# PKU-MARL/HARL

Hardware: AMD Instinct MI355X
Metric: transitions/sec through HAPPO update (MPE spread, 3 agents) (higher is better)
Workload: dtype f32

## Files before the change

### harl_amd/_lib.py

```python
from __future__ import annotations

import ctypes as C
import os
from typing import Dict, Optional

import torch

from .traffic import algorithmic_bytes, algorithmic_flops

_HERE = os.path.dirname(os.path.abspath(__file__))
LIB_PATH = os.path.join(_HERE, "lib", "libharl_%s.so" % (os.environ.get("HARL_LIB") or "hip"))

PS_STRIDE = 48
DHEAD_LD = 32
SLAB = 32

_vp, _i, _l, _f, _d = C.c_void_p, C.c_int, C.c_long, C.c_float, C.c_double

SIGNATURES = {
    "harl_gae_returns": [_vp] * 8 + [_i, _i, _f, _f, _i, _i, _i, _vp],
    "harl_masked_moments": [_vp, _vp, _l, _vp, _vp, _vp],
    "harl_dist_rows": [_vp, _l, _i, _i, _vp, _f, _f, _vp, _vp, _vp, _i, _i, _vp, _vp, _vp, _vp, _vp, _vp],
    "harl_moments_mean": [_vp, _vp, _vp],
    "harl_clock_probe": [_vp, _l, _vp],
    "harl_build_seq": [_vp, _i, _i, _i, _l, _vp, _vp, _i, _vp, _vp, _vp, _vp, _vp],
    "harl_adv_normalize": [_vp, _vp, _vp, _l, _vp],
    "harl_factor_update": [_vp, _vp, _vp, _l, _i, _i, _vp],
    "harl_sum_sumsq": [_vp, _vp, _l, _vp, _vp],
    "harl_valuenorm_apply": [_vp, _vp, _d, _d, _vp],
    "harl_gradnorm_clip_adam": [_vp, _vp, _vp, _vp, _l, _vp, _i, _f, _d, _d, _d, _f, _f, _d, _d, _vp, _vp],
    "harl_fold_linear": [_vp] * 6 + [_i, _i, _vp],
    "harl_unfold_linear_grads": [_vp, _vp, _i, _vp, _vp, _vp, _vp, _vp, _vp, _vp, _i, _i, _i, _vp],
    "harl_mlp_fwd_input": [_vp, _l, _vp, _l, _i, _vp, _vp, _i, _i, _vp, _vp, _vp, _vp, _vp, _vp, _vp],
    "harl_mlp_x0n_wide": [_vp, _l, _vp, _l, _i, _i, _vp, _vp, _vp, _vp],
    "harl_mlp_fwd_wide": [_vp, _l, _i, _vp, _i, _vp, _i, _vp, _vp, _vp, _vp, _vp],
    "harl_mlp_linear_wide": [_vp, _l, _i, _vp, _i, _vp, _i, _vp, _vp, _vp],
    "harl_act_ln_fwd": [_vp, _l, _i, _i, _vp, _vp, _vp, _vp],
    "harl_act_bwd": [_vp, _vp, _vp, _vp, _l, _i, _i, _vp],
    "harl_act_ln_tangent": [_vp, _vp, _vp, _vp, _vp, _l, _i, _i, _vp, _vp],
    "harl_mlp_tangent_wide": [_vp, _l, _i, _vp, _i, _vp, _i, _vp, _vp, _vp, _vp, _vp, _vp],
    "harl_mlp_fwd_fused2x": [_vp, _l, _vp, _i, _vp, _vp, _vp, _i, _i, _vp, _vp, _vp, _vp, _vp, _vp, _vp],
    "harl_mlp_fwd_fused2": [_vp, _l, _vp, _l, _i, _vp, _vp, _i, _vp, _vp, _i, _i, _vp, _vp, _vp, _vp, _vp, _vp, _vp, _vp,
                            _vp, _vp],
    "harl_mlp_fwd_hidden": [_vp, _l, _i, _i, _vp, _vp, _vp, _vp, _vp, _vp],
    "harl_mlp_bwd_dx": [_vp, _vp, _vp, _vp, _l, _i, _i, _vp, _vp, _vp, _i, _vp, _i, _vp],
    "harl_mlp_bwd_dx_dw": [_vp, _vp, _vp, _vp, _l, _i, _i, _vp, _vp, _vp, _i, _vp, _vp, _i, _i, _vp],
    "harl_mlp_dw_partials": [_vp, _i, _i, _i, _vp, _i, _l, _vp, _vp, _vp, _i, _l, _vp, _i, _vp],
    "harl_mlp_dw_partials_multi": [_i, _vp, _vp, _vp, _i, _i, _l, _i, _vp],
    "harl_mlp_dw_partials_multi_v": [_i, _vp, _vp, _vp, _i, _vp, _vp, _vp, _l, _i, _vp],
    "harl_gru_dw6": [_vp, _vp, _vp, _vp, _vp, _vp, _vp, _l, _i, _vp],
    "harl_mlp_fwd_trunk": [_vp, _l, _i, _vp, _i, _vp, _i, _vp, _i, _vp, _vp, _vp, _vp, _vp, _vp, _vp, _vp, _vp, _vp],
    "harl_mlp_bwd_trunk": [_l, _i, _i, _vp, _vp, _vp, _vp, _vp, _vp, _vp, _vp, _vp, _vp, _vp],
    "harl_reduce_partials": [_vp, _i, _l, _vp, _vp],
    "harl_reduce_partials_multi": [_vp, _vp, _i, _i, _l, _vp, _vp],
    "harl_adam_fold": [_vp, _vp, _vp, _vp, _l, _vp, _vp, _i, _vp, _vp, _vp, _i, _vp, _i, _f, _i, _i, _vp, _i, _f, _d, _d,
                       _d, _f, _f, _d, _d, _vp, _vp],
    "harl_pack_scalars_hilo": [_vp, _vp, _vp],
    "harl_reduce_pack_scalars": [_vp, _i, _vp, _vp, _vp],
    "harl_randperm_replay": [_vp, _l, _l, _vp, _vp, _vp],
    "harl_rng_advance": [_vp, _l, _l, _vp],
    "harl_rng_jump": [_vp, _l, _l, _vp],
    "harl_actor_head_logp": [_vp, _l, _i, _vp, _vp, _vp, _f, _f, _i, _i, _vp, _vp, _vp, _vp, _vp, _i, _vp, _l, _l, _vp],
    "harl_actor_head_loss": [_vp, _vp, _vp, _l, _i, _vp, _vp, _vp, _f, _f, _i, _i, _vp, _vp, _vp, _vp, _vp, _vp,
                             _vp, _vp, _d, _f, _i, _i, _l, _l, _vp, _vp, _vp, _vp, _vp, _i, _vp],
    "harl_critic_head_values": [_vp, _l, _i, _vp, _vp, _vp, _vp],
    "harl_critic_head_loss": [_vp, _vp, _vp, _l, _i, _vp, _vp, _vp, _vp, _vp, _vp, _f, _i, _i, _f, _l, _l, _vp, _vp, _vp,
                              _vp, _i, _vp],
    "harl_gru_fwd": [_vp] * 7 + [_i, _i, _l] + [_vp] * 8 + [_i, _vp, _vp],
    "harl_gru_bwd": [_vp] * 9 + [_i, _i, _l] + [_vp] * 8 + [_vp],
    "harl_fold_linear_tangent": [_vp] * 9 + [_i, _i, _vp],
    "harl_fold_table": [_vp, _vp, _vp, _i, _i, _vp],
    "harl_unfold_table": [_vp, _vp, _vp, _vp, _i, _i, _vp],
    "harl_fold_tangent_table": [_vp, _vp, _vp, _vp, _i, _i, _vp],
    "harl_mlp_tangent_input": [_vp, _l, _vp, _l, _i, _vp, _vp, _i, _i, _vp, _vp, _vp, _vp, _vp],
    "harl_gru_gates": [_vp, _vp, _i, _l, _vp, _vp, _vp, _i, _vp],
    "harl_gru_tangent": [_vp] * 15 + [_i, _i, _l, _vp, _vp],
    "harl_mlp_tangent_hidden": [_vp, _vp, _l, _i, _i, _vp, _vp, _vp, _vp, _vp, _vp, _vp, _vp],
    "harl_mlp_tangent_hidden2": [_vp, _vp, _l, _i, _i, _vp, _vp, _vp, _vp, _vp, _vp, _vp, _vp, _vp],
    "harl_actor_head_fvp": [_vp, _vp, _vp, _vp, _l, _i, _vp, _vp, _vp, _vp, _vp, _f, _f, _i, _i, _vp, _l, _l, _vp, _vp, _vp],
    "harl_trpo_kl_sum": [_vp, _vp, _vp, _vp, _f, _f, _l, _i, _i, _vp, _vp],
    "harl_update_supported": [_i, _i, _i, _i],
    "harl_update_fwd_actor": [_vp, _l, _i, _i] + [_vp] * 7 + [_f, _f, _i, _i] + [_vp] * 7 + [_d, _f, _i, _i] + [_vp] * 4 + [_i] + [_vp] * 4,
    "harl_update_logp": [_vp, _l, _i, _i] + [_vp] * 7 + [_f, _f, _i, _i] + [_vp] * 5 + [_i, _vp, _vp],
    "harl_update_last_actor": [_vp, _l, _i] + [_vp] * 5 + [_f, _f, _i, _i] + [_vp] * 8 + [_d, _f, _i, _i] + [_vp] * 4 + [_i, _vp],
    "harl_update_last_critic": [_vp, _l, _i] + [_vp] * 8 + [_f, _i, _i, _f] + [_vp] * 3 + [_i, _vp],
    "harl_update_fwd_critic": [_vp, _l, _i, _i] + [_vp] * 9 + [_f, _i, _i, _f] + [_vp] * 3 + [_i] + [_vp] * 4,
    "harl_update_values": [_vp, _l, _i, _i] + [_vp] * 7 + [_vp],
    "harl_update_bwd": [_vp, _vp, _l, _i, _i] + [_vp] * 5 + [_i, _vp],
    "harl_head_blocks": [_l],
    "harl_trpo_fvp_finish": [_vp, _vp, _vp, _vp, _l, _f, _f, _l, _i, _f, _f, _vp],
    "harl_trpo_cg_step": [_vp, _vp, _vp, _vp, _l, _vp, _vp, _vp],
    "harl_mlp_panel_fwd": [_vp, _l, _i, _vp, _i, _vp, _i, _vp, _vp, _vp, _vp],
    "harl_mlp_panel_bwd": [_vp, _vp, _vp, _vp, _l, _i, _i, _vp, _vp, _vp],
    "harl_head_dw_rows256": [_vp, _l, _i, _vp, _vp, _i, _vp],
    "harl_mlp_panel_tangent": [_vp, _vp, _l, _i, _vp, _vp, _i, _vp, _vp, _vp, _vp, _vp, _vp],
    "harl_reduce_scalars": [_vp, _i, _vp, _vp],
    "harl_mlp_linear": [_vp, _l, _i, _i, _vp, _vp, _vp, _vp],
    "harl_mlp_linear3": [_vp, _vp, _vp, _l, _i, _i, _vp, _vp, _vp, _vp, _vp, _vp, _vp, _vp, _vp, _vp],
    "harl_gru_cell_init": [_vp, _vp, _i, _l, _vp, _vp],
    "harl_gru_cell_fwd": [_vp] * 8 + [_i, _l] + [_vp] * 7 + [_vp],
    "harl_gru_cell_bwd": [_vp] * 10 + [_i, _l] + [_vp] * 5 + [_vp],
    "harl_rownorm": [_vp, _l, _i, _vp, _vp, _vp],
    "harl_gru_cell_tangent": [_vp] * 19 + [_i, _l] + [_vp] * 3,
    "harl_md_head_logp": [_vp, _i, _vp, _i, _vp, _vp, _l, _vp, _vp, _vp, _i, _vp, _i, _vp, _l, _l, _vp],
    "harl_md_head_loss": [_vp, _vp, _i, _vp, _i, _vp, _vp, _l, _vp, _vp, _vp, _i, _vp, _vp, _vp, _vp, _vp, _d, _f, _i, _i,
                          _l, _l, _vp, _vp, _i, _vp],
    "harl_trpo_begin": [_vp, _vp, _l, _i, _vp, _vp, _vp, _vp, _l, _vp, _vp, _vp, _vp],
    "harl_trpo_step": [_vp, _vp, _vp, _vp, _vp, _vp, _l, _f, _vp, _vp, _vp],
    "harl_trpo_ls_candidate": [_vp, _vp, _vp, _vp, _l, _vp],
    "harl_trpo_ls_test": [_vp, _vp, _d, _d, _d, _d, _vp, _vp],
    "harl_reduce_scalars_set": [_vp, _i, _vp, _vp],
    "harl_zero_bytes": [_vp, _l, _vp],
    "harl_comm_create": [_i, _i, _l, _i, _vp, _vp],
    "harl_comm_connect": [_vp, _vp],
    "harl_comm_allreduce": [_vp, _vp, _l, _i, _vp],
    "harl_comm_set_timeout": [_vp, _d],
    "harl_comm_status": [_vp],
    "harl_comm_destroy": [_vp],
    "harl_version": [],
}


class HipLibraryMissing(RuntimeError):
    pass


_lib: Optional[C.CDLL] = None


def load() -> C.CDLL:
    global _lib
    if _lib is not None:
        return _lib
    if not os.path.exists(LIB_PATH):
        raise HipLibraryMissing(
            f"{LIB_PATH} not found: build it with `python -m harl_amd._build` (hipcc, gfx950). "
            "harl_amd has no CPU fallback.")
    lib = C.CDLL(LIB_PATH)
    for name, argtypes in SIGNATURES.items():
        fn = getattr(lib, name)
        fn.argtypes = argtypes
        fn.restype = C.c_int
    lib.harl_last_error.argtypes = []
    lib.harl_last_error.restype = C.c_char_p
    _lib = lib
    return lib


def ptr(t: Optional[torch.Tensor]) -> Optional[int]:
    if t is None:
        return None
    assert t.is_contiguous(), "harl_amd kernels need contiguous tensors"
    return t.data_ptr()


_raw_stream = getattr(torch._C, "_cuda_getCurrentRawStream", None)
_raw_device = getattr(torch._C, "_cuda_getDevice", None)


def stream() -> int:
    if _raw_stream is not None and _raw_device is not None:
        return _raw_stream(_raw_device())
    return torch.cuda.current_stream().cuda_stream


_timing_on = False
_timing_events: dict = {}


_timing_tags = None


_event_pool: list = []


def reserve_timing_events(n: int) -> None:
    while len(_event_pool) < n:
        _event_pool.append(torch.cuda.Event(enable_timing=True))


def enable_kernel_timing(on: bool, tags=None) -> None:
    global _timing_on, _timing_tags
    _timing_on = bool(on)
    _timing_tags = set(tags) if tags else None
    if on:
        _timing_events.clear()

# ... 57 lines not shown
```

### harl_amd/csrc/wide.hip

```cpp
#include <type_traits>
#include <stdlib.h>
#include "common.h"
#include "split_mfma.h"
#include "fwd_epilogue.h"
#include "../../include/harl_hip.h"

using namespace harl;

namespace {

int bad(const char *m) {
  set_error(m);
  return -2;
}

__device__ __forceinline__ float wave_sum_dpp(float v) {
  auto dpp = [](float x, auto ctrl) {
    return __builtin_bit_cast(float, __builtin_amdgcn_update_dpp(0, __builtin_bit_cast(int, x), decltype(ctrl)::value, 0xf, 0xf, true));
  };
  v += dpp(v, std::integral_constant<int, 0xB1>{});
  v += dpp(v, std::integral_constant<int, 0x4E>{});
  v += dpp(v, std::integral_constant<int, 0x141>{});
  v += dpp(v, std::integral_constant<int, 0x140>{});
  const float r0 = __builtin_bit_cast(float, __builtin_amdgcn_readlane(__builtin_bit_cast(int, v), 0));
  const float r1 = __builtin_bit_cast(float, __builtin_amdgcn_readlane(__builtin_bit_cast(int, v), 16));
  const float r2 = __builtin_bit_cast(float, __builtin_amdgcn_readlane(__builtin_bit_cast(int, v), 32));
  const float r3 = __builtin_bit_cast(float, __builtin_amdgcn_readlane(__builtin_bit_cast(int, v), 48));
  return (r0 + r1) + (r2 + r3);
}

constexpr int XT_LD = 36;

template <int NC>
__global__ __launch_bounds__(WG_THREADS, NC <= 3 ? 2 : 1) void k_x0n_wide(const float *__restrict__ X, long ldx,
                                                                           const int64_t *__restrict__ idx, long M, int D,
                                                                           int use_ln0, float *__restrict__ x0n,
                                                                           float *__restrict__ mu0_out,
                                                                           float *__restrict__ rstd0_out, long n_slabs, int KP) {
  __shared__ __attribute__((aligned(16))) float tiles[WAVES_PER_WG][2][32 * XT_LD];
  const int lane = threadIdx.x & 63, wave = wave_id();
  const int i = lane & 31, h = lane >> 5;
  float *tw = &tiles[wave][0][0];
  for (long slab = (long)blockIdx.x * WAVES_PER_WG + wave; slab < n_slabs; slab += (long)gridDim.x * WAVES_PER_WG) {
    long rows[32];
    if (idx) {
#pragma unroll
      for (int r = 0; r < 32; ++r) {
        const long j = slab * SLAB + r;
        rows[r] = idx[j < M ? j : M - 1];
      }
    } else {
#pragma unroll
      for (int r = 0; r < 32; ++r) {
        const long j = slab * SLAB + r;
        rows[r] = j < M ? j : M - 1;
      }
    }
    int kc[NC];
#pragma unroll
    for (int c = 0; c < NC; ++c) kc[c] = 64 * c + lane < D ? 64 * c + lane : 0;
    float v[32][NC];
#pragma unroll
    for (int r = 0; r < 32; ++r) {
      const float *xr = X + rows[r] * ldx;
#pragma unroll
      for (int c = 0; c < NC; ++c) v[r][c] = xr[kc[c]];
    }
    const float invD = 1.0f / (float)D;
    float my_mean = 0.f, my_rstd = 1.f;
#pragma unroll
    for (int r = 0; r < 32; ++r) {
      float mean = 0.f, rstd = 1.f;
      if (use_ln0) {
        float s = 0.f;
#pragma unroll
        for (int c = 0; c < NC; ++c) s += (64 * c + lane < D) ? v[r][c] : 0.f;
        mean = wave_sum_dpp(s) * invD;
        float q = 0.f;
#pragma unroll
        for (int c = 0; c < NC; ++c) {
          const float d = v[r][c] - mean;
          q += (64 * c + lane < D) ? d * d : 0.f;
        }
        rstd = 1.0f / sqrtf(wave_sum_dpp(q) * invD + 1e-5f);
      }
#pragma unroll
      for (int c = 0; c < NC; ++c) {
        const int k = 64 * c + lane;
        v[r][c] = k < D ? (v[r][c] - mean) * rstd : ((k == KP - 1 && D < KP) ? 1.0f : 0.f);
      }
      if (lane == r) {
        my_mean = mean;
        my_rstd = rstd;
      }
    }
    if (lane < 32) {
      mu0_out[slab * SLAB + lane] = my_mean;
      rstd0_out[slab * SLAB + lane] = my_rstd;
    }
    f32x4 *op = reinterpret_cast<f32x4 *>(x0n + slab * (long)KP * SLAB) + lane;
#pragma unroll
    for (int c = 0; c < NC; ++c) {
      if (64 * c < KP) {
        float *tl = tw + h * (32 * XT_LD) + i * XT_LD;
#pragma unroll
        for (int r4 = 0; r4 < 8; ++r4)
          *reinterpret_cast<f32x4 *>(tl + 4 * r4) = f32x4{v[4 * r4][c], v[4 * r4 + 1][c], v[4 * r4 + 2][c], v[4 * r4 + 3][c]};
        asm volatile("s_waitcnt lgkmcnt(0)" ::: "memory");
        __builtin_amdgcn_wave_barrier();
#pragma unroll
        for (int t2 = 0; t2 < 2; ++t2) {
          if (64 * c + 32 * t2 < KP) {
            const float *ts = tw + t2 * (32 * XT_LD);
#pragma unroll
            for (int qq = 0; qq < 4; ++qq) {
              f32x4 o;
#pragma unroll
              for (int e = 0; e < 4; ++e) o[e] = ts[(8 * qq + 4 * h + e) * XT_LD + i];
              op[(4 * (2 * c + t2) + qq) * WAVE] = o;
            }
          }
        }
        asm volatile("s_waitcnt lgkmcnt(0)" ::: "memory");
        __builtin_amdgcn_wave_barrier();
      }
    }
  }
}

template <int KPV>
__global__ __launch_bounds__(WG_THREADS, 4) void k_x0n_contig(const float *__restrict__ X, long M, int D, int use_ln0,
                                                              float *__restrict__ x0n, float *__restrict__ mu0_out,
                                                              float *__restrict__ rstd0_out, long n_slabs) {
  __shared__ float rowsl[WAVES_PER_WG][32 * KPV + 32];
  const int lane = threadIdx.x & 63, wave = wave_id();
  const int i = lane & 31, h = lane >> 5;
  float *rw = &rowsl[wave][0];
  const int per = 32 * D;
  for (long slab = (long)blockIdx.x * WAVES_PER_WG + wave; slab < n_slabs; slab += (long)gridDim.x * WAVES_PER_WG) {
    const long base = slab * SLAB * (long)D, lim = M * (long)D;
#pragma unroll
    for (int u = 0; u < KPV / 2; ++u) {
      const int e = u * 64 + lane;
      if (e < per) rw[e] = base + e < lim ? X[base + e] : 0.f;
    }
    asm volatile("s_waitcnt vmcnt(0) lgkmcnt(0)" ::: "memory");
    __builtin_amdgcn_wave_barrier();
    const float *xr = rw + i * D;
    float mean = 0.f, rstd = 1.f;
    if (use_ln0) {
      float sm = 0.f;
      for (int k = 0; k < D; ++k) sm += xr[k];
      mean = sm / (float)D;
      float vs = 0.f;
      for (int k = 0; k < D; ++k) {
        const float d = xr[k] - mean;
        vs += d * d;
      }
      rstd = 1.0f / sqrtf(vs / (float)D + 1e-5f);
    }
    f32x4 *op = reinterpret_cast<f32x4 *>(x0n + slab * (long)KPV * SLAB) + lane;
#pragma unroll
    for (int q = 0; q < KPV / 8; ++q) {
      f32x4 o;
#pragma unroll
      for (int e = 0; e < 4; ++e) {
        const int f = 32 * (q >> 2) + 8 * (q & 3) + 4 * h + e;
        o[e] = f < D ? (xr[f < D ? f : 0] - mean) * rstd : ((f == KPV - 1 && D < KPV) ? 1.0f : 0.f);
      }
      op[q * WAVE] = o;
    }
    if (h == 0) {
      mu0_out[slab * SLAB + i] = mean;
      rstd0_out[slab * SLAB + i] = rstd;
    }
    asm volatile("s_waitcnt lgkmcnt(0)" ::: "memory");
    __builtin_amdgcn_wave_barrier();
  }
}

__global__ __launch_bounds__(WG_THREADS, 2) void k_x0n_narrow(const float *__restrict__ X, long ldx,
                                                              const int64_t *__restrict__ idx, long M, int D, int use_ln0,
                                                              float *__restrict__ x0n, float *__restrict__ mu0_out,
                                                              float *__restrict__ rstd0_out, long n_slabs) {
  __shared__ __attribute__((aligned(16))) float tiles[WAVES_PER_WG][32 * XT_LD];
  const int lane = threadIdx.x & 63, wave = wave_id();
  const int i = lane & 31, h = lane >> 5;
  float *tw = &tiles[wave][0];
  const int kc = i < D ? i : 0;
  for (long slab = (long)blockIdx.x * WAVES_PER_WG + wave; slab < n_slabs; slab += (long)gridDim.x * WAVES_PER_WG) {
    long rows[16];
    if (idx) {
#pragma unroll
      for (int u = 0; u < 16; ++u) {
        const long j = slab * SLAB + 2 * u + h;
        rows[u] = idx[j < M ? j : M - 1];
      }
    } else {
#pragma unroll
      for (int u = 0; u < 16; ++u) {
        const long j = slab * SLAB + 2 * u + h;
        rows[u] = j < M ? j : M - 1;
      }
    }
    float v[16];
#pragma unroll
    for (int u = 0; u < 16; ++u) v[u] = X[rows[u] * ldx + kc];
    const float invD = 1.0f / (float)D;
    float my_mean = 0.f, my_rstd = 1.f;
#pragma unroll
    for (int u = 0; u < 16; ++u) {
      float mean = 0.f, rstd = 1.f;
      if (use_ln0) {
        mean = half_reduce_sum(i < D ? v[u] : 0.f) * invD;
        const float d = v[u] - mean;
        rstd = 1.0f / sqrtf(half_reduce_sum(i < D ? d * d : 0.f) * invD + 1e-5f);
      }
      v[u] = i < D ? (v[u] - mean) * rstd : ((i == 31 && D < 32) ? 1.0f : 0.f);
      if (i == u) {
        my_mean = mean;
        my_rstd = rstd;
      }
    }
    if (i < 16) {
      mu0_out[slab * SLAB + 2 * i + h] = my_mean;
      rstd0_out[slab * SLAB + 2 * i + h] = my_rstd;
    }
#pragma unroll
    for (int u = 0; u < 16; ++u) tw[i * XT_LD + 2 * u + h] = v[u];
    asm volatile("s_waitcnt lgkmcnt(0)" ::: "memory");
    __builtin_amdgcn_wave_barrier();
    f32x4 *op = reinterpret_cast<f32x4 *>(x0n + slab * (long)32 * SLAB) + lane;
#pragma unroll
    for (int qq = 0; qq < 4; ++qq) {
      f32x4 o;
#pragma unroll
      for (int e = 0; e < 4; ++e) o[e] = tw[(8 * qq + 4 * h + e) * XT_LD + i];
      op[qq * WAVE] = o;
    }
    asm volatile("s_waitcnt lgkmcnt(0)" ::: "memory");
    __builtin_amdgcn_wave_barrier();
  }
}

__global__ __launch_bounds__(256) void k_split_image(const float *__restrict__ Wp, int H, int D, int KP,
                                                     u32x4 *__restrict__ img, const float *__restrict__ WpB = nullptr,
                                                     int DA = 0) {
  const int MT = H / 32, NJ = KP / 16, total = MT * NJ * 64;
  for (int e = blockIdx.x * blockDim.x + threadIdx.x; e < total; e += gridDim.x * blockDim.x) {
    const int ln = e & 63, j = (e >> 6) % NJ, t = (e >> 6) / NJ, m = 32 * t + (ln & 31), g = ln >> 5;
    unsigned p[3][4];
#pragma unroll
    for (int c = 0; c < 4; ++c) {
      const int f0 = feat_base(8 * j + 2 * c) + 4 * g, f1 = feat_base(8 * j + 2 * c + 1) + 4 * g;
      float w0, w1;
      if (WpB) {
        w0 = f0 < DA ? Wp[(long)m * DA + f0] : (f0 < D ? WpB[(long)m * (D - DA) + (f0 - DA)] : 0.f);
        w1 = f1 < DA ? Wp[(long)m * DA + f1] : (f1 < D ? WpB[(long)m * (D - DA) + (f1 - DA)] : 0.f);
      } else {
        w0 = f0 < D ? Wp[(long)m * D + f0] : 0.f;
        w1 = f1 < D ? Wp[(long)m * D + f1] : 0.f;
      }
      split3_rne(w0, w1, p[0][c], p[1][c], p[2][c]);
    }
#pragma unroll
    for (int term = 0; term < 3; ++term) img[(long)term * total + e] = u32x4{p[term][0], p[term][1], p[term][2], p[term][3]};
  }
}

template <int HO, int MODE, int NJL = 0>
__global__ __launch_bounds__(WG_THREADS, 1) void k_fwd_wide(const float *__restrict__ x0n, const u32x4 *__restrict__ img,
                                                            const float *__restrict__ bp, float *__restrict__ xout,
                                                            uint32_t *__restrict__ mask_out, float *__restrict__ rstd_out,
                                                            const float *__restrict__ xprimal,
                                                            const uint32_t *__restrict__ mask_in,
                                                            const float *__restrict__ rstd_in, long n_slabs, int KP,
                                                            const float *__restrict__ x0n_b = nullptr, int KPA = 0) {
  constexpr int MT = HO / 32;
  const int NJ = KP / 16, TS = MT * NJ * 64;
  const int KA = x0n_b ? KPA : KP, NJA = KA / 16, KB = KP - KA;
  const int lane = threadIdx.x & 63, wave = wave_id(), h = lane >> 5;
  const long n_pairs = (n_slabs + 1) / 2;
  const u32x4 *wl = img + lane;
  extern __shared__ __attribute__((aligned(16))) float lds_w[];
  const u32x4 *ll = reinterpret_cast<const u32x4 *>(lds_w) + lane;
  if constexpr (NJL > 0) {
    u32x4 *li = reinterpret_cast<u32x4 *>(lds_w);
    for (int e = threadIdx.x; e < 3 * MT * NJL * 64; e += WG_THREADS) {
      const int ln = e & 63, j = (e >> 6) % NJL, t = ((e >> 6) / NJL) % MT, term = (e >> 6) / (NJL * MT);
      li[e] = img[(long)term * TS + (t * NJ + j) * 64 + ln];
    }
    __syncthreads();
  }
  for (long pair = (long)blockIdx.x * WAVES_PER_WG + wave; pair < n_pairs; pair += (long)gridDim.x * WAVES_PER_WG) {
    const long s0 = 2 * pair, s1 = s0 + 1 < n_slabs ? s0 + 1 : s0;
    const f32x4 *xp0 = reinterpret_cast<const f32x4 *>(x0n + s0 * (long)KA * SLAB) + lane;
    const f32x4 *xp1 = reinterpret_cast<const f32x4 *>(x0n + s1 * (long)KA * SLAB) + lane;
    const f32x4 *xq0 = x0n_b ? reinterpret_cast<const f32x4 *>(x0n_b + s0 * (long)KB * SLAB) + lane : xp0;
    const f32x4 *xq1 = x0n_b ? reinterpret_cast<const f32x4 *>(x0n_b + s1 * (long)KB * SLAB) + lane : xp1;
    f32x16 acc0[MT], acc1[MT];
#pragma unroll
    for (int t = 0; t < MT; ++t)
#pragma unroll
      for (int r = 0; r < 16; ++r) acc0[t][r] = acc1[t][r] = bp[32 * t + (r & 3) + 8 * (r >> 2) + 4 * h];
    u32x4 an[3][MT];
    f32x4 bn[2][2];
    auto fetch = [&](int j) {
      if (NJL > 0 && j < NJL) {
#pragma unroll
        for (int term = 0; term < 3; ++term)
#pragma unroll
          for (int t = 0; t < MT; ++t) an[term][t] = ll[((term * MT + t) * NJL + j) * 64];
      } else {
#pragma unroll
        for (int term = 0; term < 3; ++term)
#pragma unroll
          for (int t = 0; t < MT; ++t) an[term][t] = wl[(long)term * TS + (t * NJ + j) * 64];
      }
      const f32x4 *b0 = j < NJA ? xp0 + (2 * j) * WAVE : xq0 + (2 * (j - NJA)) * WAVE;
      const f32x4 *b1 = j < NJA ? xp1 + (2 * j) * WAVE : xq1 + (2 * (j - NJA)) * WAVE;
      bn[0][0] = b0[0];
      bn[0][1] = b0[WAVE];
      bn[1][0] = b1[0];
      bn[1][1] = b1[WAVE];
    };
    fetch(0);
    for (int j = 0; j < NJ; ++j) {
      u32x4 a[3][MT];
#pragma unroll
      for (int term = 0; term < 3; ++term)
// ... 263 lines not shown
      vs = wave_sum32(vs);
      const float rstd = 1.0f / sqrtf(vs * (1.0f / H) + 1e-5f);
#pragma unroll
      for (int R = 0; R < NR; ++R) v[R] *= rstd;
      atl_store<H>(x2out, slab, lane, v);
#pragma unroll
      for (int w = 0; w < NW; ++w) mask2[(slab * NW + w) * WAVE + lane] = bits[w];
      if (lane < 32) rstd2[slab * SLAB + lane] = rstd;
    }
    PHASE(5);
  }
  PHASE_END(0);
}

constexpr size_t wide_sh_lds(int ho) { return (size_t)2 * 3 * (ho / 32) * WSH_PJ * 64 * 16; }
bool wide_shared(long n_slabs) {
  const char *e = getenv("HARL_WIDE_SHARED");
  return e && e[0] == '1' && n_slabs >= 512;
}

constexpr size_t wide_res_lds() { return (size_t)3 * 4 * 8 * 64 * 16; }
bool wide_resident(long n_slabs) {
  const char *e = getenv("HARL_WIDE_RESIDENT");
  return e && e[0] == '1' && n_slabs >= 512;
}

template <int MODE>
int launch_wide(const float *x0n, long M, int KP, const float *Wp, int D, const float *bp, int H, void *w_img, float *xout,
                uint32_t *mask_out, float *rstd_out, const float *xprimal, const uint32_t *mask_in, const float *rstd_in,
                hipStream_t s, const char *what) {
  if (M <= 0) return 0;
  if (H != 128 && H != 64) return bad("harl_mlp_*_wide: hidden width must be 64 or 128");
  if (KP % 32 != 0 || KP < D || KP > 512) return bad("harl_mlp_*_wide: KP must be a multiple of 32, >= D and <= 512");
  if (!w_img || !x0n) return bad("harl_mlp_*_wide: x0n and the weight-image scratch are required");
  const long n_slabs = n_slabs_of(M);
  const int total = (H / 32) * (KP / 16) * 64;
  hipLaunchKernelGGL(k_split_image, dim3((total + 255) / 256), dim3(256), 0, s, Wp, H, D, KP, reinterpret_cast<u32x4 *>(w_img));
  const long pairs = (n_slabs + 1) / 2, wgs = (pairs + WAVES_PER_WG - 1) / WAVES_PER_WG;
  const int grid = (int)(wgs < 256 ? (wgs < 1 ? 1 : wgs) : 256);
  if (wide_shared(n_slabs)) {
    if (H == 128) {
      allow_big_lds(k_fwd_wide_sh<128, MODE>, wide_sh_lds(128));
      hipLaunchKernelGGL((k_fwd_wide_sh<128, MODE>), dim3(grid), dim3(WG_THREADS), wide_sh_lds(128), s, x0n,
                         reinterpret_cast<const u32x4 *>(w_img), bp, xout, mask_out, rstd_out, xprimal, mask_in, rstd_in, n_slabs, KP);
    } else {
      allow_big_lds(k_fwd_wide_sh<64, MODE>, wide_sh_lds(64));
      hipLaunchKernelGGL((k_fwd_wide_sh<64, MODE>), dim3(grid), dim3(WG_THREADS), wide_sh_lds(64), s, x0n,
                         reinterpret_cast<const u32x4 *>(w_img), bp, xout, mask_out, rstd_out, xprimal, mask_in, rstd_in, n_slabs, KP);
    }
    return check_launch(what);
  }
  if (H == 128 && KP >= 256 && wide_resident(n_slabs)) {
    allow_big_lds(k_fwd_wide<128, MODE, 8>, wide_res_lds());
    hipLaunchKernelGGL((k_fwd_wide<128, MODE, 8>), dim3(grid), dim3(WG_THREADS), wide_res_lds(), s, x0n,
                       reinterpret_cast<const u32x4 *>(w_img), bp, xout, mask_out, rstd_out, xprimal, mask_in, rstd_in, n_slabs, KP);
  } else if (H == 128)
    hipLaunchKernelGGL((k_fwd_wide<128, MODE>), dim3(grid), dim3(WG_THREADS), 0, s, x0n, reinterpret_cast<const u32x4 *>(w_img),
                       bp, xout, mask_out, rstd_out, xprimal, mask_in, rstd_in, n_slabs, KP);
  else
    hipLaunchKernelGGL((k_fwd_wide<64, MODE>), dim3(grid), dim3(WG_THREADS), 0, s, x0n, reinterpret_cast<const u32x4 *>(w_img),
                       bp, xout, mask_out, rstd_out, xprimal, mask_in, rstd_in, n_slabs, KP);
  return check_launch(what);
}

}

void harl::launch_split_image(const float *Wp, int H, int D, int KP, void *img, hipStream_t stream) {
  const int total = (H / 32) * (KP / 16) * 64;
  hipLaunchKernelGGL(k_split_image, dim3((total + 255) / 256), dim3(256), 0, stream, Wp, H, D, KP, reinterpret_cast<u32x4 *>(img));
}

HARL_PHASE_ACCESSOR(wide)

extern "C" int harl_mlp_tangent_hidden2(const float *xin_dot, const float *xin, long M, int HI, int HO, const float *Wp,
                                        const float *Wdp, const float *bdp, void *w_img, const float *xprimal,
                                        const uint32_t *mask_in, const float *rstd_in, float *xout_dot, void *stream) {
  if (M <= 0) return 0;
  if ((HO != 128 && HO != 64) || (HI != 128 && HI != 64)) return bad("harl_mlp_tangent_hidden2: widths must be 64 or 128");
  if (!w_img || !xin_dot || !xin) return bad("harl_mlp_tangent_hidden2: inputs and the weight-image scratch are required");
  hipStream_t s = (hipStream_t)stream;
  const long n_slabs = n_slabs_of(M);
  const int KP = 2 * HI, total = (HO / 32) * (KP / 16) * 64;
  hipLaunchKernelGGL(k_split_image, dim3((total + 255) / 256), dim3(256), 0, s, Wp, HO, KP, KP, reinterpret_cast<u32x4 *>(w_img),
                     Wdp, HI);
  const long pairs = (n_slabs + 1) / 2, wgs = (pairs + WAVES_PER_WG - 1) / WAVES_PER_WG;
  const int grid = (int)(wgs < 256 ? (wgs < 1 ? 1 : wgs) : 256);
  if (wide_shared(n_slabs)) {
    if (HO == 128) {
      allow_big_lds(k_fwd_wide_sh<128, 1>, wide_sh_lds(128));
      hipLaunchKernelGGL((k_fwd_wide_sh<128, 1>), dim3(grid), dim3(WG_THREADS), wide_sh_lds(128), s, xin_dot,
                         reinterpret_cast<const u32x4 *>(w_img), bdp, xout_dot, nullptr, nullptr, xprimal, mask_in, rstd_in, n_slabs,
                         KP, xin, HI);
    } else {
      allow_big_lds(k_fwd_wide_sh<64, 1>, wide_sh_lds(64));
      hipLaunchKernelGGL((k_fwd_wide_sh<64, 1>), dim3(grid), dim3(WG_THREADS), wide_sh_lds(64), s, xin_dot,
                         reinterpret_cast<const u32x4 *>(w_img), bdp, xout_dot, nullptr, nullptr, xprimal, mask_in, rstd_in, n_slabs,
                         KP, xin, HI);
    }
    return check_launch("harl_mlp_tangent_hidden2");
  }
  if (HO == 128 && HI == 128 && wide_resident(n_slabs)) {
    allow_big_lds(k_fwd_wide<128, 1, 8>, wide_res_lds());
    hipLaunchKernelGGL((k_fwd_wide<128, 1, 8>), dim3(grid), dim3(WG_THREADS), wide_res_lds(), s, xin_dot,
                       reinterpret_cast<const u32x4 *>(w_img), bdp, xout_dot, nullptr, nullptr, xprimal, mask_in, rstd_in, n_slabs, KP,
                       xin, HI);
  } else if (HO == 128)
    hipLaunchKernelGGL((k_fwd_wide<128, 1>), dim3(grid), dim3(WG_THREADS), 0, s, xin_dot, reinterpret_cast<const u32x4 *>(w_img),
                       bdp, xout_dot, nullptr, nullptr, xprimal, mask_in, rstd_in, n_slabs, KP, xin, HI);
  else
    hipLaunchKernelGGL((k_fwd_wide<64, 1>), dim3(grid), dim3(WG_THREADS), 0, s, xin_dot, reinterpret_cast<const u32x4 *>(w_img),
                       bdp, xout_dot, nullptr, nullptr, xprimal, mask_in, rstd_in, n_slabs, KP, xin, HI);
  return check_launch("harl_mlp_tangent_hidden2");
}

extern "C" int harl_mlp_x0n_wide(const float *X, long ldx, const int64_t *idx, long M, int D, int use_ln0, float *x0n,
                                 float *mu0, float *rstd0, void *stream) {
  if (M <= 0) return 0;
  if (D < 1 || D > 512) return bad("harl_mlp_x0n_wide: 1 <= D <= 512");
  const long n_slabs = n_slabs_of(M);
  const int KP = ((D + 31) / 32) * 32, NC = (D + 63) / 64;
  const long wgs = (n_slabs + WAVES_PER_WG - 1) / WAVES_PER_WG;
  hipStream_t s = (hipStream_t)stream;
  if (D <= 32 && !idx && ldx == D) {
    const int grid = (int)(wgs < 1024 ? (wgs < 1 ? 1 : wgs) : 1024);
    hipLaunchKernelGGL(k_x0n_contig<32>, dim3(grid), dim3(WG_THREADS), 0, s, X, M, D, use_ln0, x0n, mu0, rstd0, n_slabs);
    return check_launch("harl_mlp_x0n_wide");
  }
  if (D <= 32) {
    const int grid = (int)(wgs < 512 ? (wgs < 1 ? 1 : wgs) : 512);
    hipLaunchKernelGGL(k_x0n_narrow, dim3(grid), dim3(WG_THREADS), 0, s, X, ldx, idx, M, D, use_ln0, x0n, mu0, rstd0, n_slabs);
    return check_launch("harl_mlp_x0n_wide");
  }
#define LX(NCv)                                                                                                         \
  {                                                                                                                     \
    const long cap = 256L * (NCv <= 3 ? 2 : 1);                                                                         \
    const int grid = (int)(wgs < cap ? (wgs < 1 ? 1 : wgs) : cap);                                                      \
    hipLaunchKernelGGL((k_x0n_wide<NCv>), dim3(grid), dim3(WG_THREADS), 0, s, X, ldx, idx, M, D, use_ln0, x0n, mu0, rstd0, \
                       n_slabs, KP);                                                                                    \
  }
  switch (NC) {
    case 1: LX(1) break;
    case 2: LX(2) break;
    case 3: LX(3) break;
    case 4: LX(4) break;
    case 5: LX(5) break;
    case 6: LX(6) break;
    case 7: LX(7) break;
    default: LX(8) break;
  }
#undef LX
  return check_launch("harl_mlp_x0n_wide");
}

extern "C" int harl_mlp_fwd_wide(const float *x0n, long M, int KP, const float *Wp, int D, const float *bp, int H,
                                 void *w_img, float *xout, uint32_t *relu_mask, float *rstd, void *stream) {
  return launch_wide<0>(x0n, M, KP, Wp, D, bp, H, w_img, xout, relu_mask, rstd, nullptr, nullptr, nullptr,
                        (hipStream_t)stream, "harl_mlp_fwd_wide");
}

extern "C" int harl_mlp_linear_wide(const float *x0n, long M, int KP, const float *Wp, int D, const float *bp, int H,
                                    void *w_img, float *zout, void *stream) {
  return launch_wide<2>(x0n, M, KP, Wp, D, bp, H, w_img, zout, nullptr, nullptr, nullptr, nullptr, nullptr,
                        (hipStream_t)stream, "harl_mlp_linear_wide");
}

extern "C" int harl_mlp_tangent_wide(const float *x0n, long M, int KP, const float *Wdp, int D, const float *bdp, int H,
                                     void *w_img, const float *x1, const uint32_t *mask1, const float *rstd1, float *x1dot,
                                     void *stream) {
  return launch_wide<1>(x0n, M, KP, Wdp, D, bdp, H, w_img, x1dot, nullptr, nullptr, x1, mask1, rstd1,
                        (hipStream_t)stream, "harl_mlp_tangent_wide");
}

extern "C" int harl_mlp_fwd_fused2x(const float *x0n, long M, const float *W1p, int D, const float *b1p, const float *W2p,
                                    const float *b2p, int H, int store1, float *x1out, uint32_t *mask1, float *rstd1,
                                    float *x2out, uint32_t *mask2, float *rstd2, void *stream) {
  if (M <= 0) return 0;
  if (D < 1 || D > 64) return bad("harl_mlp_fwd_fused2x: input width must be <= 64");
  if (H != 128 && H != 64) return bad("harl_mlp_fwd_fused2x: hidden width must be 64 or 128");
  const long n_slabs = n_slabs_of(M);
  const int kp0 = D <= 32 ? 32 : 64;
  const size_t shm = split_image_bytes(H, kp0) + split_image_bytes(H, H) + 2 * (size_t)H * sizeof(float);
  const long wgs = (n_slabs + F2X_WAVES - 1) / F2X_WAVES;
  const int grid = (int)(wgs < 256 ? (wgs < 1 ? 1 : wgs) : 256);
  hipStream_t s = (hipStream_t)stream;
#define LF(Hv, Kv)                                                                                                       \
  {                                                                                                                      \
    allow_big_lds(k_fwd_fused2x<Hv, Kv>, shm);                                                                           \
    hipLaunchKernelGGL((k_fwd_fused2x<Hv, Kv>), dim3(grid), dim3(64 * F2X_WAVES), shm, s, x0n, W1p, D, b1p, W2p, b2p, store1, \
                       x1out, mask1, rstd1, x2out, mask2, rstd2, n_slabs);                                                \
  }
  if (H == 128) {
    if (kp0 == 32) LF(128, 32) else LF(128, 64)
  } else {
    if (kp0 == 32) LF(64, 32) else LF(64, 64)
  }
#undef LF
  return check_launch("harl_mlp_fwd_fused2x");
}
```

### harl_amd/dropin.py

```python
from __future__ import annotations

import os
import runpy
import sys
import types
from typing import Optional

_INSTALLED = False


def stub_optional_modules() -> None:
    def missing(name):
        try:
            __import__(name)
            return False
        except ImportError:
            return True

    if missing("absl"):
        absl, flags = types.ModuleType("absl"), types.ModuleType("absl.flags")
        flags.FLAGS = lambda argv: argv
        absl.flags = flags
        sys.modules["absl"], sys.modules["absl.flags"] = absl, flags
    if missing("setproctitle"):
        sp = types.ModuleType("setproctitle")
        sp.setproctitle = lambda s: None
        sys.modules["setproctitle"] = sp
    if missing("tensorboardX"):
        tb = types.ModuleType("tensorboardX")

        class SummaryWriter:
            def __init__(self, *a, **k):
                self.scalars = {}

            def add_scalars(self, main_tag, tag_scalar_dict, global_step=None):
                for k, v in tag_scalar_dict.items():
                    self.scalars.setdefault(f"{main_tag}/{k}", []).append((global_step, float(v)))

            def export_scalars_to_json(self, path):
                import json
                with open(path, "w", encoding="utf-8") as f:
                    json.dump(self.scalars, f)

            def close(self):
                pass

        tb.SummaryWriter = SummaryWriter
        sys.modules["tensorboardX"] = tb


def _runner_class(base_cls, ours):
    import torch

    class Runner(base_cls):
        __doc__ = f"harl_amd drop-in: {base_cls.__module__}.{base_cls.__name__} + device-resident {ours.__name__} methods"

        _init_update_state = ours._init_update_state
        _ensure_update_state = ours._ensure_update_state
        _critic_first_ok = getattr(ours, "_critic_first_ok", None)
        _fp_normalised_advantages = ours._fp_normalised_advantages
        _check_comms = ours._check_comms
        warmup = ours.warmup
        insert = ours.insert
        compute = ours.compute
        train = ours.train
        after_update = ours.after_update

        def __init__(self, *a, **k):
            super().__init__(*a, **k)
            if not self.algo_args["render"]["use_render"]:
                from .dist import Comm
                self.comm = Comm()
                self._critic_comm = self.comm.second_group()
                self._init_update_state()

        @torch.no_grad()
        def collect(self, step):
            values, actions, logp, rnn, rnn_c = ours.collect(self, step)
            return values, actions.cpu().numpy(), logp, rnn, rnn_c

    Runner.__name__ = ours.__name__
    Runner.__qualname__ = ours.__name__
    return Runner


def install(reference_root: Optional[str] = None, stubs: bool = True) -> dict:
    global _INSTALLED
    if reference_root and reference_root not in sys.path:
        sys.path.insert(0, reference_root)
    if stubs:
        stub_optional_modules()
    import harl.algorithms.actors as ref_actors
    import harl.runners as ref_runners
    import harl.runners.on_policy_base_runner as base

    from . import buffers, runner, valuenorm
    from .happo import HAA2C, HAPPO
    from .hatrpo import HATRPO
    from .mappo import MAPPO
    from .v_critic import VCritic

    ours_algos = {"happo": HAPPO, "hatrpo": HATRPO, "haa2c": HAA2C, "mappo": MAPPO}
    ref_actors.ALGO_REGISTRY.update(ours_algos)
    base.ALGO_REGISTRY = ref_actors.ALGO_REGISTRY
    base.VCritic = VCritic
    base.ValueNorm = valuenorm.ValueNorm
    base.OnPolicyActorBuffer = buffers.OnPolicyActorBuffer
    base.OnPolicyCriticBufferEP = buffers.OnPolicyCriticBufferEP
    base.OnPolicyCriticBufferFP = buffers.OnPolicyCriticBufferFP
    ha = _runner_class(base.OnPolicyBaseRunner, runner.OnPolicyHARunner)
    ma = _runner_class(base.OnPolicyBaseRunner, runner.OnPolicyMARunner)
    installed = {"happo": ha, "hatrpo": ha, "haa2c": ha, "mappo": ma}
    ref_runners.RUNNER_REGISTRY.update(installed)
    _INSTALLED = True
    return installed


def main(argv=None) -> None:
    argv = list(sys.argv[1:] if argv is None else argv)
    ref = os.environ.get("HARL_REFERENCE")
    if "--reference" in argv:
        i = argv.index("--reference")
        ref = argv[i + 1]
        del argv[i:i + 2]
    if "--" in argv:
        argv.remove("--")
    if not ref or not os.path.exists(os.path.join(ref, "examples", "train.py")):
        raise SystemExit("harl_amd.dropin: --reference /path/to/HARL (or HARL_REFERENCE) must contain examples/train.py")
    install(ref)
    sys.argv = [os.path.join(ref, "examples", "train.py")] + argv
    runpy.run_path(sys.argv[0], run_name="__main__")


if __name__ == "__main__":
    main()
```

### harl_amd/nets.py

```python
from __future__ import annotations

import math
import os
from typing import Dict, List, Optional, Sequence, Tuple

import torch
import torch.nn as nn

from . import _lib
from ._lib import DHEAD_LD, PS_STRIDE, SLAB, call, ptr, stream

SUPPORTED_WIDTHS = (64, 128, 256)
ACT_IDS = {"relu": 0, "leaky_relu": 1, "tanh": 2, "sigmoid": 3, "selu": 4}


_FUSED_UPDATE_MODES = ("hybrid", "logp", "1", "actor", "0")


def _fused_update_mode() -> str:
    mode = os.environ.get("HARL_FUSED_UPDATE", "hybrid")
    if mode not in _FUSED_UPDATE_MODES:
        raise ValueError(f"HARL_FUSED_UPDATE={mode!r}: expected one of {_FUSED_UPDATE_MODES}")
    return mode


BWD_FUSED_MIN_ROWS = 400_000


def _bwd_fused_mode(M: int = 0) -> str:
    m = os.environ.get("HARL_BWD_FUSED", "auto")
    if m not in ("0", "1", "nofill", "auto"):
        raise ValueError(f"HARL_BWD_FUSED={m!r}: expected auto, 0, 1 or nofill")
    if m == "auto":
        return "1" if M >= BWD_FUSED_MIN_ROWS else "0"
    return m


def _bwd_streams() -> bool:
    return os.environ.get("HARL_BWD_STREAMS", "0") == "1"


def _space_shape(space) -> Tuple[int, ...]:
    name = space.__class__.__name__
    if name == "Box":
        return tuple(space.shape)
    if name == "list":
        return tuple(space)
    raise NotImplementedError(f"observation space {name}")


class _Node(nn.Module):
    """Empty container used to reproduce the reference's dotted parameter names."""


def _register(root: nn.Module, dotted: str, p: nn.Parameter) -> None:
    parts = dotted.split(".")
    mod = root
    for name in parts[:-1]:
        if name not in mod._modules:
            mod.add_module(name, _Node())
        mod = mod._modules[name]
    mod.register_parameter(parts[-1], p)


class _FlatNet(nn.Module):

    def __init__(self, args: dict, in_dim: int, device: torch.device):
        super().__init__()
        _lib.require_gpu(device)
        self.device_ = device
        self.hidden_sizes = list(args["hidden_sizes"])
        self.use_feature_normalization = bool(args["use_feature_normalization"])
        self.activation_func = args.get("activation_func", "relu")
        if self.activation_func not in ACT_IDS:
            raise NotImplementedError(f"activation_func {self.activation_func!r}: supported are {sorted(ACT_IDS)} (the functions "
                                      "torch.nn.init.calculate_gain knows, as in the reference's MLPLayer)")
        self.act_id = ACT_IDS[self.activation_func]
        self.recurrent = bool(args.get("use_recurrent_policy", False) or args.get("use_naive_recurrent_policy", False))
        self.recurrent_n = int(args.get("recurrent_n", 1))
        hl = self.hidden_sizes[-1]
        self.gru_wide = self.recurrent and ((hl == 128 and os.environ.get("HARL_GRU128", "1") != "0")
                                            or (hl in (64, 128) and self.recurrent_n > 1))
        if self.recurrent and hl == 64 and os.environ.get("HARL_GRU_COMPOSED") == "1":
            self.gru_wide = True
        if self.recurrent and self.recurrent_n < 1:
            raise ValueError("recurrent_n must be >= 1")
        if self.recurrent and not self.gru_wide and (hl != 64 or self.recurrent_n != 1):
            raise NotImplementedError("GRU kernels: hidden width 64 (fused; composed for recurrent_n > 1) or 128 (composed)")
        for h in self.hidden_sizes:
            if h not in SUPPORTED_WIDTHS:
                raise NotImplementedError(f"hidden width {h}: kernels are instantiated for {SUPPORTED_WIDTHS}")
        self.panel = 256 in self.hidden_sizes
        if self.panel and (any(h != 256 for h in self.hidden_sizes) or self.recurrent or in_dim > 512):
            raise NotImplementedError("hidden width 256: all layers must be 256 wide, feed-forward, inputs <= 512")
        if self.act_id and (self.recurrent or self.panel or in_dim > 512):
            raise NotImplementedError("activation functions other than relu: feed-forward MLPs of width 64 / 128 with inputs <= 512")
        self.in_dim = in_dim
        self.wide = 32 < in_dim <= 512
        self._x0n_key = None
        self.md = False
        self._md_sp: List[int] = []
        self._cpu_params: List[Tuple[str, torch.Tensor]] = []
        self._build_trunk_params(args)

    def _build_trunk_params(self, args: dict) -> None:
        init = getattr(nn.init, args["initialization_method"])
        gain = nn.init.calculate_gain(self.activation_func)
        d = self.in_dim
        if self.use_feature_normalization:
            self._cpu_params += [("base.feature_norm.weight", torch.ones(d)), ("base.feature_norm.bias", torch.zeros(d))]
        for i, h in enumerate(self.hidden_sizes):
            lin = nn.Linear(d, h)
            init(lin.weight.data, gain=gain)
            nn.init.constant_(lin.bias.data, 0)
            self._cpu_params += [(f"base.mlp.fc.{3*i}.weight", lin.weight.data), (f"base.mlp.fc.{3*i}.bias", lin.bias.data),
                                 (f"base.mlp.fc.{3*i+2}.weight", torch.ones(h)), (f"base.mlp.fc.{3*i+2}.bias", torch.zeros(h))]
            d = h
        if self.recurrent:
            gru = nn.GRU(d, d, num_layers=self.recurrent_n)
            for name, param in gru.named_parameters():
                if "bias" in name:
                    nn.init.constant_(param, 0)
                elif "weight" in name:
                    init(param)
            sd = dict(gru.named_parameters())
            for l in range(self.recurrent_n):
                self._cpu_params += [(f"rnn.rnn.{k}", sd[k].data) for k in
                                     (f"weight_ih_l{l}", f"weight_hh_l{l}", f"bias_ih_l{l}", f"bias_hh_l{l}")]
            self._cpu_params += [("rnn.norm.weight", torch.ones(d)), ("rnn.norm.bias", torch.zeros(d))]

    def _finalize_params(self) -> None:
        dev = self.device_
        total = sum(t.numel() for _, t in self._cpu_params)
        self.flat_param = torch.empty(total, dtype=torch.float32, device=dev)
        self.flat_grad = torch.zeros(total, dtype=torch.float32, device=dev)
        self.offsets: Dict[str, Tuple[int, Tuple[int, ...]]] = {}
        off = 0
        hidden = getattr(self, "_hidden_blocks", ())
        for name, t in self._cpu_params:
            n = t.numel()
            view = self.flat_param[off:off + n].view(t.shape)
            view.copy_(t.to(dev))
            if name not in hidden:
                p = nn.Parameter(view, requires_grad=True)
                p.grad = self.flat_grad[off:off + n].view(t.shape)
                _register(self, name, p)
            self.offsets[name] = (off, tuple(t.shape))
            off += n
        for name, base, lo, hi in getattr(self, "_alias_params", ()):
            boff, bshape = self.offsets[base]
            rowlen = math.prod(bshape[1:])
            o, shape = boff + lo * rowlen, (hi - lo,) + tuple(bshape[1:])
            n = math.prod(shape)
            p = nn.Parameter(self.flat_param[o:o + n].view(shape), requires_grad=True)
            p.grad = self.flat_grad[o:o + n].view(shape)
            _register(self, name, p)
            self.offsets[name] = (o, shape)
        self.n_params = total
        del self._cpu_params
        self._packs: List[Tuple[torch.Tensor, torch.Tensor]] = []
        self._max_rows = 0

    def flat_reference(self) -> torch.Tensor:
        return torch.cat([p.detach().reshape(-1) for p in self.parameters()])

    def pview(self, name: str) -> torch.Tensor:
        off, shape = self.offsets[name]
        return self.flat_param[off:off + math.prod(shape)].view(shape)

    def gview(self, name: str) -> torch.Tensor:
        off, shape = self.offsets[name]
        return self.flat_grad[off:off + math.prod(shape)].view(shape)

    def _layers(self) -> List[Tuple[str, str, Optional[str], Optional[str], int, int]]:
        out = []
        d = self.in_dim
        g = ("base.feature_norm.weight", "base.feature_norm.bias") if self.use_feature_normalization else (None, None)
        for i, h in enumerate(self.hidden_sizes):
            out.append((f"base.mlp.fc.{3*i}.weight", f"base.mlp.fc.{3*i}.bias", g[0], g[1], h, d))
            g = (f"base.mlp.fc.{3*i+2}.weight", f"base.mlp.fc.{3*i+2}.bias")
            d = h
        if self.recurrent:
            g = ("rnn.norm.weight", "rnn.norm.bias")
        for hw, hb, hdim in self._head_layers():
            out.append((hw, hb, g[0], g[1], hdim, d))
        return out

    def _head_layers(self) -> List[Tuple[str, str, int]]:
        return [self._head_names()]

    def _entries(self) -> List[Tuple[int, int, int, int, int, int]]:
        off = lambda n: self.offsets[n][0] if n else -1
        layers = self._layers()
        nh = len(self._head_layers())
        ents = [(off(w), off(b), off(g), off(be), o, k) for (w, b, g, be, o, k) in layers[:-nh]]
        if self.recurrent:
            H = self.hidden_sizes[-1]
            i = len(self.hidden_sizes) - 1
            for l in range(self.recurrent_n):
                g, be = (off(f"base.mlp.fc.{3*i+2}.weight"), off(f"base.mlp.fc.{3*i+2}.bias")) if l == 0 else (-1, -1)
                for gate in range(3):
                    ents.append((off(f"rnn.rnn.weight_ih_l{l}") + gate * H * H, off(f"rnn.rnn.bias_ih_l{l}") + gate * H, g, be, H, H))
                for gate in range(3):
                    ents.append((off(f"rnn.rnn.weight_hh_l{l}") + gate * H * H, off(f"rnn.rnn.bias_hh_l{l}") + gate * H, -1, -1, H, H))
        for (w, b, g, be, o, k) in layers[-nh:]:
            ents.append((off(w), off(b), off(g), off(be), o, k))
        return ents

    def _head_names(self) -> Tuple[str, str, int]:
        raise NotImplementedError

    def _build_tables(self) -> None:
        ents = self._entries()
        dev = self.device_
        L = len(self.hidden_sizes)
        rows, pack_off, dwp_off = [], 0, 0
        pack_slots = []
        self._dwp_offs, self._elems = [], []
        if self.recurrent:
            H = self.hidden_sizes[-1]
        for ei, (wo, bo, go, beo, o, k) in enumerate(ents):
            gru_i = ei - L if (self.recurrent and L <= ei < L + 6 * self.recurrent_n) else -1
            if gru_i >= 0:
                layer, within = divmod(gru_i, 6)
                mat, gate = divmod(within, 3)
                base = self._gru_pack_base + (2 * layer + mat) * (3 * H * H + 3 * H)
                pw, pb = base + gate * H * H, base + 3 * H * H + gate * H
            else:
                if self.recurrent and ei == L:
                    pass
                orows = self._md_sp[ei - (len(ents) - len(self._md_sp))] if (self.md and ei >= len(ents) - len(self._md_sp)) else o
                pw, pb = pack_off, pack_off + orows * k
                pack_off += orows * k + orows
                if self.recurrent and ei == L - 1:
                    self._gru_pack_base = pack_off
                    pack_off += 2 * self.recurrent_n * (3 * H * H + 3 * H)
            kp, op = ((k + 31) // 32) * 32, ((o + 31) // 32) * 32
            if self.md and ei >= len(ents) - len(self._md_sp):
                op = self._md_sp[ei - (len(ents) - len(self._md_sp))]
            elems = op * kp + op
            rows.append([wo, bo, go, beo, o, k, pw, pb, dwp_off, kp, op, 0])
            pack_slots.append((pw, pb, o, k))
            self._dwp_offs.append(dwp_off)
            self._elems.append(elems)
            dwp_off += elems
        self._table_rows = rows
        self.n_entries = len(rows)
        self.pack_arena = torch.zeros(pack_off, dtype=torch.float32, device=dev)
        self.dwp_msg = torch.zeros(dwp_off + 4 * PS_STRIDE, dtype=torch.float32, device=dev)
        self.dwp = self.dwp_msg[:dwp_off]
        self.total_dwp = dwp_off
        self._pack_slots = pack_slots
        views = [(self.pack_arena[pw:pw + o * k], self.pack_arena[pb:pb + o]) for (pw, pb, o, k) in pack_slots]
        self._packs = views[:L] + [views[-1]]
        nh = len(self._head_layers())
        self._head_packs = views[-nh:]
        if self.recurrent:
            n = 3 * H * H
            self.gru_packs = []
            for l in range(self.recurrent_n):
                b0 = self._gru_pack_base + 2 * l * (n + 3 * H)
                self.gru_packs.append(dict(Wih=self.pack_arena[b0:b0 + n], bih=self.pack_arena[b0 + n:b0 + n + 3 * H],
                                           Whh=self.pack_arena[b0 + n + 3 * H:b0 + 2 * n + 3 * H],
                                           bhh=self.pack_arena[b0 + 2 * n + 3 * H:b0 + 2 * n + 6 * H]))
            self.gru_pack = self.gru_packs[0]
        covered = sum(o * k + o for (_, _, _, _, o, k) in ents)
        covered += sum(k for go, k in {(go, k) for (_, _, go, _, _, k) in ents if go >= 0}) * 2
        if isinstance(self, StochasticPolicy) and not self.discrete:
            covered += self.act_dim
        assert covered == self.n_params, f"layer table covers {covered} of {self.n_params} parameters"
        self.table = None

    def fold(self) -> None:
        if not self._packs:
            self._build_tables()
        ver = self.flat_param._version
        if getattr(self, "_fold_version", None) == ver and os.environ.get("HARL_ALWAYS_FOLD", "0") != "1":
            return
        s = stream()
        fp, pa = self.flat_param, self.pack_arena
        if self.table is not None and os.environ.get("HARL_FOLD_TABLE", "1") != "0":
            call("harl_fold_table", ptr(fp), ptr(pa), ptr(self.table), self.n_entries, sum(r[4] for r in self._table_rows), s)
            self._fold_version = ver
            return
        for (wo, bo, go, beo, o, k), (pw, pb, _, _) in zip(self._entries(), self._pack_slots):
            call("harl_fold_linear", ptr(fp[wo:]), ptr(fp[bo:]), ptr(fp[go:]) if go >= 0 else None,
                 ptr(fp[beo:]) if beo >= 0 else None, ptr(pa[pw:]), ptr(pa[pb:]), o, k, s)
        self._fold_version = ver

    def _ensure_ws(self, M: int) -> None:
        if M <= self._max_rows:
            return
        dev = self.device_
        n_slabs = (M + SLAB - 1) // SLAB
        mp = n_slabs * SLAB
        f32, u32 = torch.float32, torch.int32
        self.xh = [torch.empty(mp * h, dtype=f32, device=dev) for h in self.hidden_sizes]
        self.rmask = [torch.empty(n_slabs * max(h // 64, 1) * 64, dtype=u32, device=dev) for h in self.hidden_sizes]
        self.rstd = [torch.empty(mp, dtype=f32, device=dev) for _ in self.hidden_sizes]
        self.mu0 = torch.empty(mp, dtype=f32, device=dev)
        self.rstd0 = torch.empty(mp, dtype=f32, device=dev)
        self.kp0 = ((self.in_dim + 31) // 32) * 32
        self.wide = 32 < self.in_dim <= 512
        self._x0n_key = None
        self.x0n = torch.empty(mp * self.kp0, dtype=f32, device=dev) if (self.in_dim <= 64 or self.wide) else None
        self.w1img = (torch.empty(3 * self.hidden_sizes[0] * self.kp0 // 2, dtype=f32, device=dev)
                      if (self.wide or self.act_id) else None)
        hmax = max(self.hidden_sizes)
        if self.act_id:
            self.zraw = torch.empty(mp * hmax, dtype=f32, device=dev)
            self.amean = [torch.empty(mp, dtype=f32, device=dev) for _ in self.hidden_sizes]
            self.ones_mask = torch.full((n_slabs * 64 * 2,), -1, dtype=u32, device=dev)
        self.dz = [torch.empty(mp * hmax, dtype=f32, device=dev) for _ in range(3 if len(self.hidden_sizes) == 3 and self.trunk_fused() else 2)]
        self._trunk_cache = {}
        self.wide_head = (not self.md) and self._layers()[-1][4] > 32
        self.dhead = torch.zeros(mp * (64 if self.wide_head else DHEAD_LD), dtype=f32, device=dev)
        self.md_z = [torch.zeros(mp * sp, dtype=f32, device=dev) for sp in self._md_sp]
        n_iter = (n_slabs + 1) // 2
        nwg_env = os.environ.get("HARL_NWG")
        nwg_cap = int(nwg_env) if nwg_env else max(256, min(512, n_slabs // 10))
        if (not nwg_env and _bwd_fused_mode(M) == "1" and len(self.hidden_sizes) >= 2 and all(h == 128 for h in self.hidden_sizes)
                and ((self.in_dim + 31) // 32) * 32 == 32 and not (self.recurrent or self.md or self.act_id or self.panel)):
            nwg_cap = 256
        self.n_wg = max(1, min(nwg_cap, n_iter))
        part_off, rows = 0, [list(r) for r in self._table_rows]
        self._part_offs = []
        for r, elems in zip(rows, self._elems):
            r[11] = part_off
            self._part_offs.append(part_off)
            part_off += self.n_wg * elems
        self.part = torch.empty(part_off, dtype=f32, device=dev)
        self.table = torch.tensor(rows, dtype=torch.int32, device=dev).reshape(-1).contiguous()
        if self.recurrent:
            H = self.hidden_sizes[-1]
            a = lambda: torch.empty(mp * H, dtype=f32, device=dev)
            self.rnn_y, self.rnn_rstd = a(), torch.empty(mp, dtype=f32, device=dev)
            self.rnn_saved_l = [[a() for _ in range(5)] for _ in range(self.recurrent_n)]
            self.rnn_dgate_l = [[a() for _ in range(4)] for _ in range(self.recurrent_n)]
            self.rnn_saved, self.rnn_dgate = self.rnn_saved_l[0], self.rnn_dgate_l[0]
            self.rnn_ones = torch.full((n_slabs * 64 * ((H // 2 + 31) // 32),), -1, dtype=u32, device=dev)
            self.rnn_gi = torch.empty(3 * mp * H, dtype=f32, device=dev)
            if self.gru_wide:
                from . import gru_wide
                gru_wide.ensure_ws(self, mp)
        self.n_head_blocks = max(_lib.load().harl_head_blocks(M), self.n_wg)
        self.part_scalars = torch.zeros(self.n_head_blocks * PS_STRIDE, dtype=f32, device=dev)
        self.scalars = torch.zeros(PS_STRIDE, dtype=torch.float64, device=dev)
        self._max_rows = M

    def feat(self):
        if self.recurrent:
            return self.rnn_y, self.rnn_ones, self.rnn_rstd, self.hidden_sizes[-1]
        if self.act_id:
            return self.xh[-1], self.ones_mask, self.rstd[-1], self.hidden_sizes[-1]
        return self.xh[-1], self.rmask[-1], self.rstd[-1], self.hidden_sizes[-1]

    def forward_rnn(self, seq: dict, save: bool, gates_done: bool = False) -> None:
        if self.gru_wide:
            from . import gru_wide
            return gru_wide.forward(self, seq, save)
        gp = self.gru_pack
        sv = self.rnn_saved
        call("harl_gru_fwd", ptr(self.xh[-1]), ptr(seq["mask_rows"]), ptr(seq["h0"]), ptr(gp["Wih"]), ptr(gp["bih"]),
             ptr(gp["Whh"]), ptr(gp["bhh"]), self.hidden_sizes[-1], seq["L"], seq["m_pad"], ptr(self.rnn_y),
             ptr(self.rnn_rstd), ptr(sv[0]), ptr(sv[1]), ptr(sv[2]), ptr(sv[3]), ptr(sv[4]), ptr(seq.get("h_last")),
             int(save) | (2 if gates_done else 0), ptr(self.rnn_gi), stream(), tag="gru_fwd")

    def trunk_fused(self) -> bool:
        hs = self.hidden_sizes
        return (os.environ.get("HARL_TRUNK_FUSED", "1") != "0" and self.wide and not self.act_id and not self.panel
                and 2 <= len(hs) <= 3 and all(h == 64 for h in hs))

    def _trunk_ptrs(self, save: bool, gates: bool):
        key = (save, gates, self._max_rows)
        hit = self._trunk_cache.get(key)
        if hit is None:
            import ctypes as C
            L = len(self.hidden_sizes)
            keep = [save or (l == L - 1 and not gates) for l in range(L)]
            vp = lambda ts: (C.c_void_p * len(ts))(*[ptr(t) for t in ts])
            hit = self._trunk_cache[key] = (
                vp([self._packs[l][0] for l in range(1, L)]), vp([self._packs[l][1] for l in range(1, L)]),
                vp([self.xh[l] if keep[l] else None for l in range(L)]), vp([self.rmask[l] if keep[l] else None for l in range(L)]),
                vp([self.rstd[l] if keep[l] else None for l in range(L)]))
        return hit

    def _x0n_image(self, X: torch.Tensor, M: int, s, idx: Optional[torch.Tensor] = None) -> None:
        key = ((X.data_ptr(), X._version, tuple(X.shape), M) if idx is None
               else (X.data_ptr(), X._version, tuple(X.shape), M, idx.data_ptr(), idx._version, idx.numel()))
        if key != self._x0n_key:
            call("harl_mlp_x0n_wide", ptr(X), X.shape[1], ptr(idx), M, self.in_dim, int(self.use_feature_normalization),
                 ptr(self.x0n), ptr(self.mu0), ptr(self.rstd0), s, tag="x0n_wide")
            self._x0n_key, self._x0n_src = key, (X, idx)

    def invalidate_caches(self) -> None:
        self._x0n_key = None
        self._x0n_src = None
        self._fold_version = None

    def forward_trunk(self, X: torch.Tensor, idx: Optional[torch.Tensor], M: int, for_backward: bool = True,
                      seq: Optional[dict] = None, upto: Optional[int] = None) -> None:
        assert X.dim() == 2 and X.shape[1] == self.in_dim and X.is_contiguous()
        rnn_save = for_backward
        if self.recurrent:
            assert seq is not None and seq["L"] * seq["m_pad"] == M, "recurrent nets need the sequence layout"
            for_backward = True
        self._ensure_ws(M)
        s = stream()
        hs = self.hidden_sizes
        first_hidden = 1
        if self.act_id:
            self._x0n_image(X, M, s, idx)
            for l, h in enumerate(hs):
                Wp, bp = self._packs[l]
                if l == 0:
                    call("harl_mlp_linear_wide", ptr(self.x0n), M, self.kp0, ptr(Wp), self.in_dim, ptr(bp), h, ptr(self.w1img),
                         ptr(self.zraw), s, tag="linear_wide")
                else:
                    call("harl_mlp_linear", ptr(self.xh[l - 1]), M, hs[l - 1], h, ptr(Wp), ptr(bp), ptr(self.zraw), s, tag="linear")
                call("harl_act_ln_fwd", ptr(self.zraw), M, h, self.act_id, ptr(self.xh[l]), ptr(self.amean[l]), ptr(self.rstd[l]),
                     s, tag="act_ln_fwd")
            return
        if self.panel:
            self._x0n_image(X, M, s, idx)
            for l in range(len(hs)):
                Wp, bp = self._packs[l]
                xin, kp, d = (self.x0n, self.kp0, self.in_dim) if l == 0 else (self.xh[l - 1], 256, 256)
                call("harl_mlp_panel_fwd", ptr(xin), M, kp, ptr(Wp), d, ptr(bp), 256, ptr(self.xh[l]), ptr(self.rmask[l]),
                     ptr(self.rstd[l]), s, tag="fwd_panel")
            return
        if upto is None and self.trunk_fused():
            gates = self.recurrent and not self.gru_wide
            Wp, bp = self._packs[0]
            self._x0n_image(X, M, s, idx)
            pW, pb, pX, pM, pR = self._trunk_ptrs(bool(rnn_save), gates)
            gp = self.gru_pack if gates else None
            call("harl_mlp_fwd_trunk", ptr(self.x0n), M, self.kp0, ptr(Wp), self.in_dim, ptr(bp), 64, ptr(self.w1img),
                 len(hs) - 1, pW, pb, pX, pM, pR, ptr(gp["Wih"]) if gates else None, ptr(gp["bih"]) if gates else None,
                 ptr(gp["bhh"]) if gates else None, ptr(self.rnn_gi) if gates else None, s, tag="fwd_trunk")
            if self.recurrent:
                self.forward_rnn(seq, save=rnn_save, gates_done=gates)
            return
        if len(hs) >= 2 and hs[0] == hs[1] and self.in_dim <= 64 and idx is None:
            (W1, b1), (W2, b2) = self._packs[0], self._packs[1]
            self._x0n_image(X, M, s)
            call("harl_mlp_fwd_fused2x", ptr(self.x0n), M, ptr(W1), self.in_dim, ptr(b1), ptr(W2), ptr(b2), hs[0],
                 int(for_backward), ptr(self.xh[0]), ptr(self.rmask[0]), ptr(self.rstd[0]), ptr(self.xh[1]),
                 ptr(self.rmask[1]), ptr(self.rstd[1]), s, tag="fwd_fused2" if self.kp0 == 32 else "fwd_fused2_k64")
            first_hidden = 2
        elif len(hs) >= 2 and hs[0] == hs[1] and self.in_dim <= 32:
            (W1, b1), (W2, b2) = self._packs[0], self._packs[1]
            self._x0n_key = None
            call("harl_mlp_fwd_fused2", ptr(X), X.shape[1], ptr(idx), M, self.in_dim, ptr(W1), ptr(b1),
                 int(self.use_feature_normalization), ptr(W2), ptr(b2), hs[0], int(for_backward), ptr(self.xh[0]),
                 ptr(self.rmask[0]), ptr(self.rstd[0]), ptr(self.mu0), ptr(self.rstd0), ptr(self.xh[1]),
                 ptr(self.rmask[1]), ptr(self.rstd[1]), ptr(self.x0n) if for_backward else None, s, tag="fwd_fused2")
            first_hidden = 2
        elif self.wide:
            Wp, bp = self._packs[0]
            self._x0n_image(X, M, s, idx)
            call("harl_mlp_fwd_wide", ptr(self.x0n), M, self.kp0, ptr(Wp), self.in_dim, ptr(bp), hs[0], ptr(self.w1img),
                 ptr(self.xh[0]), ptr(self.rmask[0]), ptr(self.rstd[0]), s, tag="fwd_wide")
        else:
            Wp, bp = self._packs[0]
            self._x0n_key = None
            call("harl_mlp_fwd_input", ptr(X), X.shape[1], ptr(idx), M, self.in_dim, ptr(Wp), ptr(bp),
                 int(self.use_feature_normalization), hs[0], ptr(self.xh[0]), ptr(self.rmask[0]), ptr(self.rstd[0]),
                 ptr(self.mu0), ptr(self.rstd0), ptr(self.x0n) if for_backward else None, s, tag="fwd_input")
        assert upto is None or upto >= first_hidden
        for l in range(first_hidden, len(hs) if upto is None else upto):
            Wp, bp = self._packs[l]
            call("harl_mlp_fwd_hidden", ptr(self.xh[l - 1]), M, hs[l - 1], hs[l],
                 ptr(Wp), ptr(bp), ptr(self.xh[l]), ptr(self.rmask[l]), ptr(self.rstd[l]), s, tag="fwd_hidden")
        if self.recurrent:
            self.forward_rnn(seq, save=rnn_save)

    def fused_update_ok(self, idx: Optional[torch.Tensor], seq: Optional[dict] = None, train: bool = True) -> bool:
        hs = self.hidden_sizes
        mode = _fused_update_mode()
        if self.act_id:
            return False
        if mode == "0" or (train and mode == "logp") or (train and mode == "actor" and isinstance(self, VNet)):
            return False
        if not (not self.recurrent and not self.md and idx is None and seq is None
                and len(hs) == 2 and hs[0] == hs[1] and hs[0] in (64, 128) and self.in_dim <= 64 and self._layers()[-1][4] <= 8):
            return False
        kind = 0 if not train else (2 if isinstance(self, VNet) else 1)
        return bool(_lib.load().harl_update_supported(self.in_dim, hs[0], self._layers()[-1][4], kind))

    def fused_last_ok(self, idx: Optional[torch.Tensor], seq: Optional[dict] = None) -> bool:
        hs = self.hidden_sizes
        if _fused_update_mode() != "hybrid" or self.act_id or self.recurrent or self.md or self.panel:
            return False
        if seq is not None or len(hs) < 2 or hs[-1] != hs[-2] or hs[-1] not in (64, 128) or self._layers()[-1][4] > 8:
            return False
        two_fused = hs[0] == hs[1] and ((self.in_dim <= 64 and idx is None) or self.in_dim <= 32)
        return len(hs) >= (3 if two_fused else 2) and bool(_lib.load().harl_update_supported(0, hs[-1], self._layers()[-1][4], 2 if isinstance(self, VNet) else 1))

    def fused_hybrid(self) -> bool:
        return _fused_update_mode() == "hybrid"

    def hybrid_outputs(self):
        if not self.fused_hybrid():
            return (None, None, None)
        return (ptr(self.xh[0]), ptr(self.rmask[0]), ptr(self.rstd[0]))

    def backward_after_fused(self, X: torch.Tensor, M: int) -> None:
        if self.fused_hybrid():
            self.backward_trunk(X, None, M, head_dw_done=True)
        else:
            self.backward_fused(M)

    def fused_args(self, X: torch.Tensor, M: int):
        self._ensure_ws(M)
        self._x0n_image(X, M, stream())
        (W1, b1), (W2, b2), (Wh, bh) = self._packs[0], self._packs[1], self._packs[-1]
        return (ptr(self.x0n), M, self.in_dim, self.hidden_sizes[0], ptr(W1), ptr(b1), ptr(W2), ptr(b2), ptr(Wh), ptr(bh))

    def _bwd_side(self):
        if getattr(self, "_bwd_side_stream", None) is None:
            self._bwd_side_stream = torch.cuda.Stream(device=self.device_)
            self._bwd_ev = [torch.cuda.Event(), torch.cuda.Event()]
        return self._bwd_side_stream

    def _combine_partials(self, s) -> None:
        call("harl_reduce_partials_multi", ptr(self.part), ptr(self.table), self.n_entries, self.n_wg, self.total_dwp,
             ptr(self.dwp), s, tag="reduce_partials")

    def backward_fused(self, M: int) -> None:
        s = stream()
        (W1, b1), (W2, _) = self._packs[0], self._packs[1]
        po = self._part_offs
        call("harl_update_bwd", ptr(self.x0n), ptr(self.dz[0]), M, self.in_dim, self.hidden_sizes[0], ptr(W1), ptr(b1),
             ptr(W2), ptr(self.part[po[0]:]), ptr(self.part[po[1]:]), self.n_wg, s, tag="update_bwd")
        self._combine_partials(s)

    def backward_trunk(self, X: torch.Tensor, idx: Optional[torch.Tensor], M: int, seq: Optional[dict] = None,
                       head_dw_done: bool = False) -> None:
        s = stream()
        L = len(self.hidden_sizes)
        nwg = self.n_wg
        po = self._part_offs
        hdim = self._layers()[-1][4]
        fx, _, _, fh = self.feat()
        if self.md:
            self.md_backward(M)
        elif not head_dw_done:
            if self.wide_head:
                call("harl_mlp_dw_partials", ptr(self.dhead), 0, 0, 64, ptr(fx), 0, 0, None, None, None, fh, M,
                     ptr(self.part[po[-1]:]), nwg, s, tag="dw_head")
            elif self.panel:
                call("harl_head_dw_rows256", ptr(self.dhead), M, hdim, ptr(fx), ptr(self.part[po[-1]:]), nwg, s, tag="dw_head")
            else:
                call("harl_mlp_dw_partials", ptr(self.dhead), 1, DHEAD_LD, hdim, ptr(fx), 0, 0, None, None, None, fh, M,
                     ptr(self.part[po[-1]:]), nwg, s, tag="dw_head")
        if self.trunk_fused() and not self.gru_wide:
            return self._backward_trunk_fused(M, seq, s)
        cur = 0
        if self.recurrent:
            gp, sv, dg = self.gru_pack, self.rnn_saved, self.rnn_dgate
            H = self.hidden_sizes[-1]
            if self.gru_wide:
                from . import gru_wide
                gru_wide.backward(self, seq)
            else:
                call("harl_gru_bwd", ptr(self.dz[0]), ptr(seq["mask_rows"]), ptr(gp["Wih"]), ptr(gp["Whh"]), ptr(sv[0]),
                     ptr(sv[1]), ptr(sv[2]), ptr(sv[3]), ptr(sv[4]), H, seq["L"], seq["m_pad"], ptr(self.xh[-1]),
                     ptr(self.rmask[-1]), ptr(self.rstd[-1]), ptr(dg[0]), ptr(dg[1]), ptr(dg[2]), ptr(dg[3]), ptr(self.dz[1]), s,
                     tag="gru_bwd")
            import ctypes as C
            for gl in range(self.recurrent_n):
                dg_, sv_ = self.rnn_dgate_l[gl], self.rnn_saved_l[gl]
                xin = self.xh[-1] if gl == 0 else self.rnn_hraw_l[gl - 1]
                a6 = (C.c_void_p * 6)(*[ptr(t) for t in (dg_[0], dg_[1], dg_[2], dg_[0], dg_[1], dg_[3])])
                b6 = (C.c_void_p * 6)(*([ptr(xin)] * 3 + [ptr(sv_[0])] * 3))
                p6 = (C.c_void_p * 6)(*[ptr(self.part[po[L + 6 * gl + k]:]) for k in range(6)])
                call("harl_mlp_dw_partials_multi", 6, a6, b6, p6, H, H, M, nwg, s, tag="dw_gru")
            cur = 1
        if self.panel:
            for l in range(L - 1, -1, -1):
                b_in, k_in = (self.x0n, self.kp0) if l == 0 else (self.xh[l - 1], 256)
                call("harl_mlp_dw_partials", ptr(self.dz[cur]), 0, 0, 256, ptr(b_in), 0, 0, None, None, None, k_in, M,
                     ptr(self.part[po[l]:]), nwg, s, tag="dw_hidden" if l else "dw_input")
                if l > 0:
                    Wp, _ = self._packs[l]
                    call("harl_mlp_panel_bwd", ptr(self.dz[cur]), ptr(self.xh[l - 1]), ptr(self.rmask[l - 1]),
                         ptr(self.rstd[l - 1]), M, 256, 256, ptr(Wp), ptr(self.dz[1 - cur]), s, tag="bwd_panel")
                    cur = 1 - cur
            self._combine_partials(s)
            return
        if self.act_id:
            hs = self.hidden_sizes
            call("harl_act_bwd", ptr(self.dz[cur]), ptr(self.xh[L - 1]), ptr(self.amean[L - 1]), ptr(self.rstd[L - 1]), M, hs[L - 1],
                 self.act_id, s, tag="act_bwd")
            for l in range(L - 1, 0, -1):
                ho, hi = hs[l], hs[l - 1]
                call("harl_mlp_dw_partials", ptr(self.dz[cur]), 0, 0, ho, ptr(self.xh[l - 1]), 0, 0, None, None, None, hi, M,
                     ptr(self.part[po[l]:]), nwg, s, tag="dw_hidden")
                Wp, _ = self._packs[l]
                call("harl_mlp_bwd_dx", ptr(self.dz[cur]), ptr(self.xh[l - 1]), ptr(self.ones_mask), ptr(self.rstd[l - 1]), M, ho,
                     hi, ptr(Wp), ptr(self.dz[1 - cur]), None, 0, None, 0, s, tag="bwd_dx")
                cur = 1 - cur
                call("harl_act_bwd", ptr(self.dz[cur]), ptr(self.xh[l - 1]), ptr(self.amean[l - 1]), ptr(self.rstd[l - 1]), M, hi,
                     self.act_id, s, tag="act_bwd")
            call("harl_mlp_dw_partials", ptr(self.dz[cur]), 0, 0, hs[0], ptr(self.x0n), 0, 0, None, None, None, self.kp0, M,
                 ptr(self.part[po[0]:]), nwg, s, tag="dw_input")
            self._combine_partials(s)
            return
        fuse_dw1 = L >= 2 and self.x0n is not None and self.in_dim < self.kp0 and self.kp0 <= 64
        bwd_mode = _bwd_fused_mode(M)
        side_pending = False
        if (bwd_mode != "0" and fuse_dw1 and self.kp0 == 64 and L >= 2 and self.hidden_sizes[0] == 128 and self.hidden_sizes[1] == 128
                and os.environ.get("HARL_BWD_K64", "0") == "1"):
            fuse_dw1 = False
        for l in range(L - 1, 0, -1):
            ho, hi = self.hidden_sizes[l], self.hidden_sizes[l - 1]
            Wp, _ = self._packs[l]
            dw1_here = l == 1 and fuse_dw1
# ... 9 lines not shown
            if side_pending and not (l == 1 and fuse_dw1):
                torch.cuda.current_stream(self.device_).wait_event(self._bwd_ev[1])
            if two:
                main_s, side_s, e0 = torch.cuda.current_stream(self.device_), self._bwd_side(), self._bwd_ev[0]
                e0.record(main_s)
            else:
                call("harl_mlp_dw_partials", ptr(self.dz[cur]), 0, 0, ho, ptr(self.xh[l - 1]), 0, 0, None, None, None, hi, M,
                     ptr(self.part[po[l]:]), nwg, s, tag="dw_hidden")
            if l == 1 and fuse_dw1:
                call("harl_mlp_bwd_dx", ptr(self.dz[cur]), ptr(self.xh[0]), ptr(self.rmask[0]), ptr(self.rstd[0]), M, ho, hi,
                     ptr(Wp), None, ptr(self.x0n), self.kp0, ptr(self.part[po[0]:]), nwg, s, tag="bwd_dx_dw1")
            else:
                call("harl_mlp_bwd_dx", ptr(self.dz[cur]), ptr(self.xh[l - 1]), ptr(self.rmask[l - 1]),
                     ptr(self.rstd[l - 1]), M, ho, hi, ptr(Wp), ptr(self.dz[1 - cur]), None, 0, None, 0, s, tag="bwd_dx")
            if two:
                side_s.wait_event(e0)
                with torch.cuda.stream(side_s):
                    call("harl_mlp_dw_partials", ptr(self.dz[cur]), 0, 0, ho, ptr(self.xh[l - 1]), 0, 0, None, None, None, hi, M,
                         ptr(self.part[po[l]:]), nwg, side_s.cuda_stream, tag="dw_hidden")
                self._bwd_ev[1].record(side_s)
                side_pending = True
            cur = 1 - cur
        h0 = self.hidden_sizes[0]
        use_ln = self.use_feature_normalization
        if fuse_dw1:
            pass
        elif self.x0n is not None:
            call("harl_mlp_dw_partials", ptr(self.dz[cur]), 0, 0, h0, ptr(self.x0n), 0, 0, None, None, None, self.kp0, M,
                 ptr(self.part[po[0]:]), nwg, s, tag="dw_input")
        else:
            call("harl_mlp_dw_partials", ptr(self.dz[cur]), 0, 0, h0, ptr(X), 1, X.shape[1], ptr(idx),
                 ptr(self.mu0) if use_ln else None, ptr(self.rstd0) if use_ln else None, self.in_dim, M,
                 ptr(self.part[po[0]:]), nwg, s, tag="dw_input")
        if side_pending:
            e1 = self._bwd_ev[1]
            e1.record(self._bwd_side())
            torch.cuda.current_stream(self.device_).wait_event(e1)
        self._combine_partials(s)

    def _backward_trunk_fused(self, M: int, seq: Optional[dict], s) -> None:
        import ctypes as C
        L, po, nwg = len(self.hidden_sizes), self._part_offs, self.n_wg
        spare = [self.dz[2]] if L == 3 else []
        if self.recurrent:
            gp, sv, dg = self.gru_pack, self.rnn_saved, self.rnn_dgate
            call("harl_gru_bwd", ptr(self.dz[0]), ptr(seq["mask_rows"]), ptr(gp["Wih"]), ptr(gp["Whh"]), ptr(sv[0]),
                 ptr(sv[1]), ptr(sv[2]), ptr(sv[3]), ptr(sv[4]), 64, seq["L"], seq["m_pad"], ptr(self.xh[-1]),
                 ptr(self.rmask[-1]), ptr(self.rstd[-1]), ptr(dg[0]), ptr(dg[1]), ptr(dg[2]), ptr(dg[3]), None, s, tag="gru_bwd")
            dzs = [self.dz[1], self.dz[0]] + spare
        else:
            dzs = [self.dz[0], self.dz[1]] + spare
        args = self._trunk_cache.get("bwd")
        if args is None:
            vp = lambda ts: (C.c_void_p * len(ts))(*[ptr(t) for t in ts])
            top_down = range(L - 1, -1, -1)
            a, b, part, K, t0, nt = [], [], [], [], [], []

            def add(aa, bb, l, k, t, n):
                a.append(aa), b.append(bb), part.append(self.part[po[l]:]), K.append(k), t0.append(t), nt.append(n)
            if self.recurrent:
                for k, (aa, bb) in enumerate(zip((dg[0], dg[1], dg[2], dg[0], dg[1], dg[3]), [self.xh[-1]] * 3 + [sv[0]] * 3)):
                    add(aa, bb, L + k, 64, 0, 2)
            for j, l in enumerate(range(L - 1, 0, -1)):
                add(dzs[j], self.xh[l - 1], l, 64, 0, 2)
            for t in range(0, self.kp0 // 32, 4):
                add(dzs[L - 1], self.x0n, 0, self.kp0, t, min(4, self.kp0 // 32 - t))
            def pack(lo, hi):
                n = hi - lo
                ci = lambda v: (C.c_int * n)(*v[lo:hi])
                return (n, vp(a[lo:hi]), vp(b[lo:hi]), vp(part[lo:hi]), ci(K), ci(t0), ci(nt))
            ng = 6 if self.recurrent else 0
            args = self._trunk_cache["bwd"] = (
                vp([self._packs[l][0] for l in range(L - 1, 0, -1)]), vp([self.xh[l] for l in top_down]),
                vp([self.rmask[l] for l in top_down]), vp([self.rstd[l] for l in top_down]),
                vp([dzs[0] if self.recurrent else None] + dzs[1:]), pack(0, len(a)), pack(0, ng) if ng else None, pack(ng, len(a)))
        pW, pX, pM, pR, pD, dw_all, dw_gates, dw_mlp = args
        two = (self.recurrent and self.device_.type == "cuda" and os.environ.get("HARL_TRUNK_DW_STREAM", "0") == "1")
        if two:
            main_s, side_s, (e0, e1) = torch.cuda.current_stream(self.device_), self._bwd_side(), self._bwd_ev
            e0.record(main_s)
            side_s.wait_event(e0)
            with torch.cuda.stream(side_s):
                call("harl_mlp_dw_partials_multi_v", dw_gates[0], *dw_gates[1:4], 64, *dw_gates[4:], M, nwg, side_s.cuda_stream,
                     tag="dw_gru")
                e1.record(side_s)
        if self.recurrent:
            call("harl_mlp_bwd_trunk", M, 64, L - 1, ptr(gp["Wih"]), ptr(dg[0]), ptr(dg[1]), ptr(dg[2]), None, pW, pX, pM, pR, pD, s,
                 tag="bwd_trunk")
        else:
            call("harl_mlp_bwd_trunk", M, 64, L - 1, None, None, None, None, ptr(self.dz[0]), pW, pX, pM, pR, pD, s, tag="bwd_trunk")
        g6 = os.environ.get("HARL_GRU_DW6", "auto")
        gru6 = self.recurrent and not two and (g6 == "1" or (g6 == "auto" and M >= 160000))
        if gru6:
            call("harl_gru_dw6", ptr(dg[0]), ptr(dg[1]), ptr(dg[2]), ptr(dg[3]), ptr(self.xh[-1]), ptr(sv[0]), dw_gates[3], M, nwg, s,
                 tag="dw_gru")
        dw = dw_mlp if (two or gru6) else dw_all
        call("harl_mlp_dw_partials_multi_v", dw[0], *dw[1:4], 64, *dw[4:], M, nwg, s, tag="dw_trunk")
        if two:
            main_s.wait_event(e1)
        self._combine_partials(s)

    def md_logits(self, M: int) -> None:
        fx, _, _, fh = self.feat()
        s = stream()
        for (Wp, bp), z, sp in zip(self._head_packs, self.md_z, self._md_sp):
            call("harl_mlp_linear", ptr(fx), M, fh, sp, ptr(Wp), ptr(bp), ptr(z), s, tag="md_linear")

    def md_layout(self):
        import ctypes as C
        G, K = len(self._md_sp), len(self.nvec)
        zs = (C.c_void_p * G)(*[z.data_ptr() for z in self.md_z])
        return (zs, G, (C.c_int * G)(*self._md_sp), K, (C.c_int * K)(*self.nvec), (C.c_int * K)(*self._md_head_group))

    def md_backward(self, M: int) -> None:
        fx, fmask, frstd, fh = self.feat()
        s = stream()
        nh = len(self._md_sp)
        po = self._part_offs[-nh:]
        for g, ((Wp, _), dzg, sp) in enumerate(zip(self._head_packs, self.md_z, self._md_sp)):
            call("harl_mlp_dw_partials", ptr(dzg), 0, 0, sp, ptr(fx), 0, 0, None, None, None, fh, M,
                 ptr(self.part[po[g]:]), self.n_wg, s, tag="dw_head")
            call("harl_mlp_bwd_dx", ptr(dzg), ptr(fx), ptr(fmask), ptr(frstd), M, sp, fh, ptr(Wp),
                 ptr(self.dz[0 if g == 0 else 1]), None, 0, None, 0, s, tag="bwd_dx")
            if g > 0:
                n = ((M + SLAB - 1) // SLAB) * SLAB * fh
                self.dz[0][:n].add_(self.dz[1][:n])

    def unfold_grads(self) -> None:
        s = stream()
        fp, fg = self.flat_param, self.flat_grad
        if self.table is not None and os.environ.get("HARL_UNFOLD_TABLE", "1") != "0":
            call("harl_unfold_table", ptr(fp), ptr(fg), ptr(self.dwp), ptr(self.table), self.n_entries,
                 sum(r[5] for r in self._table_rows), s)
            return
        seen = set()
        for (wo, bo, go, beo, o, k), off, trow in zip(self._entries(), self._dwp_offs, self._table_rows):
            kp, op = trow[9], trow[10]
            dW = self.dwp[off:off + op * kp]
            db = self.dwp[off + op * kp:off + op * kp + op]
            acc = int(go in seen)
            if go >= 0:
                seen.add(go)
            call("harl_unfold_linear_grads", ptr(dW), ptr(db), kp, ptr(fp[wo:]), ptr(fp[go:]) if go >= 0 else None,
                 ptr(fp[beo:]) if beo >= 0 else None, ptr(fg[wo:]), ptr(fg[bo:]), ptr(fg[go:]) if go >= 0 else None,
                 ptr(fg[beo:]) if beo >= 0 else None, o, k, acc, s)

    def load_state_dict(self, state_dict, strict: bool = True, assign: bool = False):
        out = super().load_state_dict(state_dict, strict=strict, assign=False)
        self._fold_version = None
        self.fold()
        return out


class StochasticPolicy(_FlatNet):

    def __init__(self, args: dict, obs_space, action_space, device: torch.device):
        obs_shape = _space_shape(obs_space)
        if len(obs_shape) != 1:
            raise NotImplementedError("image observations (CNNBase) are outside the accelerated path")
        super().__init__(args, obs_shape[0], device)
        self.action_type = action_space.__class__.__name__
        self.std_x_coef = float(args["std_x_coef"])
        self.std_y_coef = float(args["std_y_coef"])
        init = getattr(nn.init, args["initialization_method"])
        d = self.hidden_sizes[-1]
        if self.action_type == "Discrete":
            self.discrete, self.act_dim, self.act_w = True, int(action_space.n), 1
            lin = nn.Linear(d, self.act_dim)
            init(lin.weight.data, gain=args["gain"])
            nn.init.constant_(lin.bias.data, 0)
            self._cpu_params += [("act.action_out.linear.weight", lin.weight.data), ("act.action_out.linear.bias", lin.bias.data)]
        elif self.action_type == "Box":
            self.discrete, self.act_dim = False, int(action_space.shape[0])
            self.act_w = self.act_dim
            lin = nn.Linear(d, self.act_dim)
            init(lin.weight.data, gain=args["gain"])
            nn.init.constant_(lin.bias.data, 0)
            self._cpu_params += [("act.action_out.log_std", torch.ones(self.act_dim) * self.std_x_coef),
                                 ("act.action_out.fc_mean.weight", lin.weight.data), ("act.action_out.fc_mean.bias", lin.bias.data)]
        elif self.action_type == "MultiDiscrete":
            self._init_multidiscrete(args, action_space, init, d)
        else:
            raise NotImplementedError(f"action space {self.action_type}")
        if not self.md and (self.act_dim > 64 or (self.act_dim > 32 and not self.discrete)):
            raise NotImplementedError("action heads wider than 32 (Categorical: 64) are not instantiated")
        self.wide_head = (not self.md) and self.act_dim > 32
        self._finalize_params()
        self.fold()

    def _init_multidiscrete(self, args: dict, action_space, init, d: int) -> None:
        nvec = [int(n) for n in action_space.nvec]
        if self.panel:
            raise NotImplementedError("MultiDiscrete heads on 256-wide layers")
        if len(nvec) > 8 or max(nvec) > 128:
            raise NotImplementedError("MultiDiscrete: at most 8 heads of at most 128 actions each")
        if self.act_id:
            raise NotImplementedError("MultiDiscrete heads with an activation other than relu are not implemented")
        self.md, self.discrete = True, True
        self.nvec, self.n_heads = nvec, len(nvec)
        self.act_dim = sum(nvec)
        self.act_w = 1
        groups: List[List[int]] = [[]]
        for k, n in enumerate(nvec):
            if sum(nvec[j] for j in groups[-1]) + n > 128:
                groups.append([])
            groups[-1].append(k)
        if len(groups) > 4:
            raise NotImplementedError("MultiDiscrete: more than 4 groups of 128 logits")
        self._md_groups = groups
        self._md_head_group = [g for g, ks in enumerate(groups) for _ in ks]
        self._md_sp = [64 if sum(nvec[k] for k in ks) <= 64 else 128 for ks in groups]
        lins = []
        for n in nvec:
            lin = nn.Linear(d, n)
            init(lin.weight.data, gain=args["gain"])
            nn.init.constant_(lin.bias.data, 0)
            lins.append(lin)
        hidden, alias = [], []
        for g, ks in enumerate(groups):
            self._cpu_params += [(f"__md{g}.weight", torch.cat([lins[k].weight.data for k in ks], 0)),
                                 (f"__md{g}.bias", torch.cat([lins[k].bias.data for k in ks], 0))]
            hidden += [f"__md{g}.weight", f"__md{g}.bias"]
        for g, ks in enumerate(groups):
            lo = 0
            for k in ks:
                alias.append((f"act.action_outs.{k}.linear.weight", f"__md{g}.weight", lo, lo + nvec[k]))
                alias.append((f"act.action_outs.{k}.linear.bias", f"__md{g}.bias", lo, lo + nvec[k]))
                lo += nvec[k]
        self._hidden_blocks, self._alias_params = tuple(hidden), alias

    def _head_layers(self):
        if self.md:
            return [(f"__md{g}.weight", f"__md{g}.bias", sum(self.nvec[k] for k in ks)) for g, ks in enumerate(self._md_groups)]
        return [self._head_names()]

    def _head_names(self):
        if self.discrete:
            return "act.action_out.linear.weight", "act.action_out.linear.bias", self.act_dim
        return "act.action_out.fc_mean.weight", "act.action_out.fc_mean.bias", self.act_dim

    def log_std(self) -> Optional[torch.Tensor]:
        return None if self.discrete else self.pview("act.action_out.log_std")


class VNet(_FlatNet):

    def __init__(self, args: dict, cent_obs_space, device: torch.device):
        shape = _space_shape(cent_obs_space)
        if len(shape) != 1:
            raise NotImplementedError("image observations (CNNBase) are outside the accelerated path")
        super().__init__(args, shape[0], device)
        init = getattr(nn.init, args["initialization_method"])
        lin = nn.Linear(self.hidden_sizes[-1], 1)
        init(lin.weight.data, gain=1)
        nn.init.constant_(lin.bias.data, 0)
        self._cpu_params += [("v_out.weight", lin.weight.data), ("v_out.bias", lin.bias.data)]
        self._finalize_params()
        self.fold()

    def _head_names(self):
        return "v_out.weight", "v_out.bias", 1


def consume_policy_init_rng(args: dict, obs_space, action_space) -> None:
    from .buffers import rng_sync
    rng_sync()
    init = getattr(nn.init, args["initialization_method"])
    gain = nn.init.calculate_gain(args.get("activation_func", "relu"))

    def draw(lin, g):
        if args["initialization_method"] == "orthogonal_":
            w = lin.weight.data
            w.new_empty((w.size(0), w.numel() // w.size(0))).normal_(0, 1)
        else:
            init(lin.weight.data, gain=g)

    d = _space_shape(obs_space)[0]
    for h in args["hidden_sizes"]:
        draw(nn.Linear(d, h), gain)
        d = h
    if args.get("use_recurrent_policy") or args.get("use_naive_recurrent_policy"):
        gru = nn.GRU(d, d, num_layers=args.get("recurrent_n", 1))
        for pn, prm in gru.named_parameters():
            if "weight" in pn:
                if args["initialization_method"] == "orthogonal_":
                    prm.data.new_empty((prm.size(0), prm.numel() // prm.size(0))).normal_(0, 1)
                else:
                    init(prm.data)
    kind = action_space.__class__.__name__
    if kind == "MultiDiscrete":
        for n in action_space.nvec:
            draw(nn.Linear(d, int(n)), args["gain"])
        return
    n_out = int(action_space.n) if kind == "Discrete" else int(action_space.shape[0])
    draw(nn.Linear(d, n_out), args["gain"])


_FIRST_RING: dict = {}


def _upload_first_rows(first_rows: torch.Tensor, dev) -> torch.Tensor:
    if first_rows.is_cuda:
        return first_rows
    n = first_rows.numel()
    ring = _FIRST_RING.get(dev)
    if ring is None or ring["cap"] < n:
# ... 102 lines not shown
```

### harl_amd/runner.py

```python
from __future__ import annotations

import os
from typing import List, Optional

import torch

from . import _lib
from .buffers import OnPolicyActorBuffer, OnPolicyCriticBufferEP, OnPolicyCriticBufferFP, rng_sync
from ._lib import call, ptr, stream
from .dist import Comm, shard_columns
from .happo import HAA2C, HAPPO
from .hatrpo import HATRPO
from .mappo import MAPPO
from .v_critic import VCritic
from .valuenorm import ValueNorm

ALGO_REGISTRY = {"happo": HAPPO, "hatrpo": HATRPO, "haa2c": HAA2C, "mappo": MAPPO}


class OnPolicyHARunner:
    CRITIC_STREAM_MAX_ROWS = 150_000

    def __init__(self, args: dict, algo_args: dict, env_args: Optional[dict] = None, *, obs_spaces=None,
                 share_obs_space=None, act_spaces=None, device: Optional[torch.device] = None,
                 comm: Optional[Comm] = None, envs=None, logger=None, eval_envs=None, save_dir: Optional[str] = None):
        self.envs, self.logger, self.eval_envs, self.save_dir = envs, logger, eval_envs, save_dir
        if envs is not None and obs_spaces is None:
            obs_spaces, act_spaces = list(envs.observation_space), list(envs.action_space)
            share_obs_space = envs.share_observation_space[0]
        if obs_spaces is None or share_obs_space is None or act_spaces is None:
            raise ValueError("OnPolicyHARunner needs obs_spaces / share_obs_space / act_spaces (no env creation here)")
        self.args = args
        self.algo_args = algo_args
        self.env_args = env_args
        self.device = torch.device(device if device is not None else "cuda:0")
        _lib.require_gpu(self.device)
        self.comm = comm if comm is not None else Comm()
        algo = args.get("algo", "happo")
        if algo not in ALGO_REGISTRY:
            raise NotImplementedError(f"algo {algo}: this round implements {sorted(ALGO_REGISTRY)}")
        self.num_agents = len(obs_spaces)
        self.state_type = (env_args or {}).get("state_type", "EP")
        if self.state_type not in ("EP", "FP"):
            raise ValueError(f"state_type {self.state_type}")
        self.share_param = bool(algo_args["algo"].get("share_param", False))
        if self.share_param and algo != "mappo":
            raise NotImplementedError("share_param is a MAPPO feature (HAPPO/HATRPO/HAA2C need per-agent actors)")
        self.fixed_order = algo_args["algo"].get("fixed_order", True)
        self.action_aggregation = algo_args["algo"]["action_aggregation"]
        if self.share_param and self.comm.world_size > 1 and (algo_args["model"].get("use_recurrent_policy")
                                                             or algo_args["model"].get("use_naive_recurrent_policy")):
            raise NotImplementedError("share_param with recurrent policies under data parallelism is not implemented")

        n_global = algo_args["train"]["n_rollout_threads"]
        lo, hi = shard_columns(n_global, self.comm.rank, self.comm.world_size)
        self.n_global, self.col_lo, self.col_hi = n_global, lo, hi
        train_local = dict(algo_args["train"])
        train_local["n_rollout_threads"] = hi - lo
        margs = {**algo_args["model"], **algo_args["algo"]}
        self.actor: List[HAPPO] = []
        for a in range(self.num_agents):
            if self.share_param and a > 0:
                self.actor.append(self.actor[0])
            else:
                self.actor.append(ALGO_REGISTRY[algo](margs, obs_spaces[a], act_spaces[a], device=self.device))
        self.actor_buffer = [OnPolicyActorBuffer({**train_local, **algo_args["model"]}, obs_spaces[a], act_spaces[a],
                                                 device=self.device) for a in range(self.num_agents)]
        self.critic = VCritic(margs, share_obs_space, device=self.device)
        cb_args = {**train_local, **algo_args["model"], **algo_args["algo"]}
        if self.state_type == "EP":
            self.critic_buffer = OnPolicyCriticBufferEP(cb_args, share_obs_space, device=self.device)
        else:
            self.critic_buffer = OnPolicyCriticBufferFP(cb_args, share_obs_space, self.num_agents, device=self.device)
        self.value_normalizer = ValueNorm(1, device=self.device) if algo_args["train"]["use_valuenorm"] else None
        self._critic_comm = self.comm.second_group()
        self._init_update_state(n_global)
        if algo_args["train"].get("model_dir") is not None:
            self.restore(algo_args["train"]["model_dir"])

    def _init_update_state(self, n_global: Optional[int] = None, comm: Optional[Comm] = None) -> None:
        if not hasattr(self, "comm") or self.comm is None:
            self.comm = comm if comm is not None else Comm()
        if n_global is None:
            n_global = self.algo_args["train"]["n_rollout_threads"]
        if not hasattr(self, "col_lo"):
            self.n_global = n_global
            self.col_lo, self.col_hi = shard_columns(n_global, self.comm.rank, self.comm.world_size)
        shard = (self.n_global, self.col_lo, self.col_hi) if self.comm.enabled else None
        for x in list(self.actor) + [self.critic]:
            x.comm, x.shard = self.comm, shard
        self.critic.comm = getattr(self, "_critic_comm", None) or self.comm
        self._logp_old = None
        self._counts_host = None
        self._update_state_ready = True

    def _ensure_update_state(self) -> None:
        if not getattr(self, "_update_state_ready", False):
            self._init_update_state()

    def _check_comms(self) -> None:
        self.comm.check()
        if self.critic.comm is not self.comm:
            self.critic.comm.check()

    @torch.no_grad()
    def compute(self):
        self._ensure_update_state()
        cb = self.critic_buffer
        if self.state_type == "EP":
            next_value, _ = self.critic.get_values(cb.share_obs[-1], cb.rnn_states_critic[-1], cb.masks[-1])
        else:
            so = cb.share_obs[-1]
            rows = so.shape[0] * so.shape[1]
            next_value, _ = self.critic.get_values(so.reshape(rows, -1), cb.rnn_states_critic[-1].reshape(rows, 1, -1),
                                                   cb.masks[-1].reshape(rows, 1))
        cb.compute_returns(next_value, self.value_normalizer)

    @torch.no_grad()
    def train(self):
        self._ensure_update_state()
        T = self.algo_args["train"]["episode_length"]
        N = self.col_hi - self.col_lo
        B = T * N
        dev = self.device
        actor_train_infos = []
        for x in self.actor:
            x.actor.invalidate_caches()
        factor = torch.ones(T, N, 1, dtype=torch.float32, device=dev)
        advantages = self.critic_buffer.advantages
        if self.state_type == "FP":
            advantages = self._fp_normalised_advantages(advantages)
        if self.fixed_order:
            agent_order = list(range(self.num_agents))
        else:
            rng_sync()
            agent_order = [int(a) for a in torch.randperm(self.num_agents).numpy()]
        fast = [hasattr(a, "masked_moments") for a in self.actor]
        mom_all = torch.zeros(self.num_agents, 3, dtype=torch.float64, device=dev)
        for a in range(self.num_agents):
            if fast[a]:
                adv_a = advantages if self.state_type == "EP" else advantages[:, :, a].contiguous()
                self.actor[a].masked_moments(self.actor_buffer[a], adv_a, mom_all[a])
        self.comm.all_reduce_sum(mom_all)
        if self._counts_host is None or self._counts_host.numel() != self.num_agents:
            self._counts_host = torch.empty(self.num_agents, dtype=torch.float64, pin_memory=torch.cuda.is_available())
        self._counts_host.copy_(mom_all[:, 2], non_blocking=True)
        ev = torch.cuda.Event()
        ev.record()
        cinfo, critic_done = None, None
        if self._critic_first_ok(fast):
            cs_mode = os.environ.get("HARL_CRITIC_STREAM", "auto")
            if (dev.type == "cuda" and (not self.comm.enabled or self.critic.comm is not self.comm)
                    and cs_mode != "0" and (cs_mode == "1" or B <= self.CRITIC_STREAM_MAX_ROWS)):
                if getattr(self, "_critic_stream", None) is None:
                    self._critic_stream = torch.cuda.Stream(device=dev)
                main_s = torch.cuda.current_stream(dev)
                self._critic_stream.wait_stream(main_s)
                with torch.cuda.stream(self._critic_stream):
                    cinfo = self.critic.train(self.critic_buffer, self.value_normalizer, _defer=True)
                    critic_done = torch.cuda.Event()
                    critic_done.record(self._critic_stream)
            else:
                cinfo = self.critic.train(self.critic_buffer, self.value_normalizer, _defer=True)
        ev.synchronize()
        counts = self._counts_host.tolist()
        rng_after = None
        if (cinfo is None and dev.type == "cuda" and all(hasattr(a, "rng_footprint") for a in self.actor)
                and (not self.comm.enabled or self.critic.comm is not self.comm)
                and os.environ.get("HARL_CRITIC_STREAM", "1") != "0" and os.environ.get("HARL_CRITIC_EARLY", "1") != "0"):
            from .buffers import consume_randperm
            rng_sync()
            rng_start = torch.get_rng_state()
            for a in agent_order:
                if counts[a] > 0.0:
                    for n in self.actor[a].rng_footprint(self.actor_buffer[a]):
                        consume_randperm(n)
            rng_sync()
            if getattr(self, "_critic_stream", None) is None:
                self._critic_stream = torch.cuda.Stream(device=dev)
            self._critic_stream.wait_stream(torch.cuda.current_stream(dev))
            staggered = dict(gen=self.critic._train_epochs(self.critic_buffer, self.value_normalizer), state=torch.get_rng_state(),
                             left=self.critic.critic_epoch)
            torch.set_rng_state(rng_start)

            def critic_epoch(after_event=None, _st=staggered):
                if _st["left"] <= 0:
                    return
                rng_sync()
                actor_state = torch.get_rng_state()
                torch.set_rng_state(_st["state"])
                if after_event is not None:
                    self._critic_stream.wait_event(after_event)
                with torch.cuda.stream(self._critic_stream):
                    next(_st["gen"])
                _st["left"] -= 1
                rng_sync()
                _st["state"] = torch.get_rng_state()
                torch.set_rng_state(actor_state)
            rng_after = staggered
        old_all, old_ev = {}, {}
        side_agents = [a for a in agent_order
                       if not (fast[a] and self.actor[a].fuses_old_logp() and counts[a] > 0.0) and os.environ.get("HARL_SIDE_STREAM", "1") != "0"]
        def enqueue_old_logp(a):
            act_a, buf_a = self.actor[a], self.actor_buffer[a]
            with torch.cuda.stream(self._side_stream):
                act_a.actor.fold()
                kw_a = dict(rnn_states=buf_a.rnn_states[0], masks=buf_a.flat("masks")) if act_a.actor.recurrent else {}
                act_a._logp_pass(buf_a.flat("obs"), buf_a.flat("actions"),
                                 None if buf_a.available_actions is None else buf_a.flat("available_actions"), B, old_all[a], **kw_a)
                old_ev[a] = torch.cuda.Event()
                old_ev[a].record(self._side_stream)

        side_lazy = os.environ.get("HARL_SIDE_AHEAD", "1") != "0"
        side_pending = []
        if side_agents:
            if getattr(self, "_side_stream", None) is None:
                self._side_stream = torch.cuda.Stream(device=dev)
            main = torch.cuda.current_stream(dev)
            self._side_stream.wait_stream(main)
            for a in side_agents:
                act_a, buf_a = self.actor[a], self.actor_buffer[a]
                old_all[a] = torch.empty(B, act_a.actor.act_w, dtype=torch.float32, device=dev)
            side_pending = list(side_agents)
            for a in (side_pending[:1] if side_lazy else list(side_pending)):
                enqueue_old_logp(a)
                side_pending.remove(a)
        pending = []
        post_ok = dev.type == "cuda" and os.environ.get("HARL_POST_STREAM", "1") != "0"
        factor_ev, keep_alive, prev_overlapped = None, [], False
        for pos, agent_id in enumerate(agent_order):
            buf, actor = self.actor_buffer[agent_id], self.actor[agent_id]
            if agent_id in old_ev:
                torch.cuda.current_stream(dev).wait_event(old_ev[agent_id])
            buf.update_factor(factor)
            if prev_overlapped:
                keep_alive.append(self._logp_old)
                self._logp_old = None
            obs, actions = buf.flat("obs"), buf.flat("actions")
            avail = None if buf.available_actions is None else buf.flat("available_actions")
            if self._logp_old is None or self._logp_old.shape != (B, actor.actor.act_w):
                self._logp_old = torch.empty(B, actor.actor.act_w, dtype=torch.float32, device=dev)
            actor.actor.fold()
            rnn_kw = dict(rnn_states=buf.rnn_states[0], masks=buf.flat("masks")) if actor.actor.recurrent else {}
            adv_a = advantages if self.state_type == "EP" else advantages[:, :, agent_id].contiguous()
            kw = dict(_pre=(mom_all[agent_id], counts[agent_id]), _defer=True) if fast[agent_id] else {}
            fused_old = fast[agent_id] and actor.fuses_old_logp() and counts[agent_id] > 0.0
            if fused_old:
                kw["_old_logp_out"] = self._logp_old
            elif agent_id in old_all:
                self._logp_old = old_all.pop(agent_id)
            else:
                actor._logp_pass(obs, actions, avail, B, self._logp_old, **rnn_kw)
            if factor_ev is not None and hasattr(actor, "_factor_ready"):
                actor._factor_ready = factor_ev
            info = actor.train(buf, adv_a, self.state_type, **kw)
            if side_pending:
                enqueue_old_logp(side_pending.pop(0))
            if rng_after is not None and rng_after["left"] > 0:
                ev_a = torch.cuda.Event()
                ev_a.record(torch.cuda.current_stream(dev))
                critic_epoch(ev_a)
            if factor_ev is not None:
                if hasattr(actor, "_factor_ready"):
                    actor._factor_ready = None
                torch.cuda.current_stream(dev).wait_event(factor_ev)
                factor_ev = None
            pending.append((len(actor_train_infos), info, actor._INFO_KEYS) if torch.is_tensor(info) else None)
            actor_train_infos.append(info)
            nxt = agent_order[pos + 1] if pos + 1 < len(agent_order) else None
            prev_overlapped = bool(post_ok and nxt is not None and actor.actor.recurrent and hasattr(self.actor[nxt], "_factor_ready"))
            if prev_overlapped:
                if getattr(self, "_post_stream", None) is None:
                    self._post_stream = torch.cuda.Stream(device=dev)
                ps = self._post_stream
                ps.wait_stream(torch.cuda.current_stream(dev))
                keep_alive += [factor, self._logp_old]
                with torch.cuda.stream(ps):
                    new_factor = factor.clone()
                    actor._logp_pass(obs, actions, avail, B, None, old_logp=self._logp_old, factor=new_factor.reshape(B), **rnn_kw)
                    factor_ev = torch.cuda.Event()
                    factor_ev.record(ps)
                factor = new_factor
                continue
            new_factor = factor.clone()
            actor._logp_pass(obs, actions, avail, B, None, old_logp=self._logp_old, factor=new_factor.reshape(B), **rnn_kw)
            factor = new_factor
        if keep_alive:
            torch.cuda.current_stream(dev).wait_stream(self._post_stream)
            keep_alive.clear()
        if rng_after is not None:
            while rng_after["left"] > 0:
                critic_epoch(None)
            for _ in rng_after["gen"]:
                pass
            with torch.cuda.stream(self._critic_stream):
                cinfo = self.critic._train_result(True)
                critic_done = torch.cuda.Event()
                critic_done.record(self._critic_stream)
        if cinfo is None:
            cinfo = self.critic.train(self.critic_buffer, self.value_normalizer, _defer=True)
        if critic_done is not None:
            torch.cuda.current_stream(dev).wait_event(critic_done)
        rng_sync()
        if rng_after is not None:
            torch.set_rng_state(rng_after["state"])
        dev_infos = [p[1] for p in pending if p is not None] + [cinfo]
        flat = torch.cat([t.reshape(-1) for t in dev_infos]).cpu().tolist()
        self._check_comms()
        off = 0
        for p in pending:
            if p is not None:
                i, _, keys = p
                actor_train_infos[i] = dict(zip(keys, flat[off:off + len(keys)]))
                off += len(keys)
        critic_train_info = {"value_loss": flat[off], "critic_grad_norm": flat[off + 1]}
        return actor_train_infos, critic_train_info

    def _critic_first_ok(self, fast) -> bool:
        if not all(fast) or os.environ.get("HARL_CRITIC_FIRST", "1") == "0":
            return False
        c = self.critic
        if c.critic_num_mini_batch != 1 or c.use_recurrent_policy or c.use_naive_recurrent_policy:
            return False
        return all(hasattr(a, "fuses_old_logp") and a.fuses_old_logp() for a in self.actor)

    def after_update(self):
        for b in self.actor_buffer:
            b.after_update()
        self.critic_buffer.after_update()

    def _fp_normalised_advantages(self, advantages):
        dev = self.device
        active = torch.stack([b.active_masks[:-1] for b in self.actor_buffer], dim=2).contiguous()
        mom = torch.zeros(3, dtype=torch.float64, device=dev)
        n = advantages.numel()
        call("harl_masked_moments", ptr(advantages), ptr(active), n, ptr(mom), _lib.scratch("mm"), stream())
        self.comm.all_reduce_sum(mom)
        adv_n = torch.empty_like(advantages)
        call("harl_adv_normalize", ptr(advantages), ptr(mom), ptr(adv_n), n, stream())
        return adv_n

    def warmup(self):
        obs, share_obs, available_actions = self.envs.reset()
        obs = torch.as_tensor(obs, dtype=torch.float32).to(self.device)
        for a in range(self.num_agents):
            self.actor_buffer[a].obs[0].copy_(obs[:, a])
            if self.actor_buffer[a].available_actions is not None:
                av = torch.as_tensor(available_actions, dtype=torch.float32).to(self.device)
                self.actor_buffer[a].available_actions[0].copy_(av[:, a])
        so = torch.as_tensor(share_obs, dtype=torch.float32).to(self.device)
        self.critic_buffer.share_obs[0].copy_(so[:, 0] if self.state_type == "EP" else so)

    @torch.no_grad()
    def collect(self, step: int):
        acts, logps, rnns = [], [], []
        for a in range(self.num_agents):
            b = self.actor_buffer[a]
            action, logp, rnn = self.actor[a].get_actions(
                b.obs[step], b.rnn_states[step], b.masks[step],
                b.available_actions[step] if b.available_actions is not None else None)
            acts.append(action)
            logps.append(logp)
            rnns.append(rnn.reshape(rnn.shape[0], b.recurrent_n, -1))
        actions, action_log_probs, rnn_states = torch.stack(acts, 1), torch.stack(logps, 1), torch.stack(rnns, 1)
        cb = self.critic_buffer
        if self.state_type == "EP":
            values, rnn_c = self.critic.get_values(cb.share_obs[step], cb.rnn_states_critic[step], cb.masks[step])
            rnn_c = rnn_c.reshape(values.shape[0], cb.recurrent_n, -1)
        else:
            so = cb.share_obs[step]
            N, A = so.shape[:2]
            values, rnn_c = self.critic.get_values(so.reshape(N * A, -1), cb.rnn_states_critic[step].reshape(N * A, 1, -1),
                                                   cb.masks[step].reshape(N * A, 1))
            values, rnn_c = values.reshape(N, A, 1), rnn_c.reshape(N, A, cb.recurrent_n, -1)
        return values, actions, action_log_probs, rnn_states, rnn_c

    @torch.no_grad()
    def insert(self, data):
        (obs, share_obs, rewards, dones, infos, available_actions, values, actions, action_log_probs, rnn_states,
         rnn_states_critic) = data
        dev, A = self.device, self.num_agents
        up = lambda x: torch.as_tensor(x, dtype=torch.float32).to(dev)
        dones = torch.as_tensor(dones).to(dev).bool()
        N = dones.shape[0]
        dones_env = dones.all(dim=1)
        keep = (~dones_env).to(torch.float32)
        rnn_states = rnn_states * keep.view(N, 1, 1, 1)
        rnn_states_critic = rnn_states_critic * (keep.view(N, 1, 1) if self.state_type == "EP" else keep.view(N, 1, 1, 1))
        masks = keep.view(N, 1, 1).expand(N, A, 1)
        active_masks = torch.where(dones & ~dones_env.view(N, 1), 0.0, 1.0).view(N, A, 1)
        if self.state_type == "EP":
            bad = [[0.0] if info[0].get("bad_transition", False) is True else [1.0] for info in infos]
        else:
            bad = [[[0.0] if info[a].get("bad_transition", False) is True else [1.0] for a in range(A)] for info in infos]
        bad_masks = torch.tensor(bad, dtype=torch.float32, device=dev)
        obs, rewards, share_obs = up(obs), up(rewards), up(share_obs)
        avail = None if (available_actions is None or available_actions[0] is None) else up(available_actions)
        for a in range(A):
            self.actor_buffer[a].insert(obs[:, a], rnn_states[:, a], actions[:, a], action_log_probs[:, a], masks[:, a],
                                        active_masks[:, a], None if avail is None else avail[:, a])
        if self.state_type == "EP":
            self.critic_buffer.insert(share_obs[:, 0], rnn_states_critic, values, rewards[:, 0], masks[:, 0], bad_masks)
        else:
            self.critic_buffer.insert(share_obs, rnn_states_critic, values, rewards, masks, bad_masks)

    def run(self, num_episodes: Optional[int] = None):
        if self.envs is None:
            raise RuntimeError("run() needs a vectorised environment (envs=...)")
        tr = self.algo_args["train"]
        T = tr["episode_length"]
        episodes = num_episodes if num_episodes is not None else int(tr["num_env_steps"]) // T // tr["n_rollout_threads"]
        self.warmup()
        if self.logger is not None:
            self.logger.init(episodes)
        history = []
        for episode in range(1, episodes + 1):
            if tr.get("use_linear_lr_decay", False):
                for a in self.actor:
                    a.lr_decay(episode, episodes)
                self.critic.lr_decay(episode, episodes)
            if self.logger is not None:
                self.logger.episode_init(episode)
            self.prep_rollout()
            for step in range(T):
                values, actions, logp, rnn, rnn_c = self.collect(step)
                obs, share_obs, rewards, dones, infos, avail = self.envs.step(actions.cpu().numpy())
                data = (obs, share_obs, rewards, dones, infos, avail, values, actions, logp, rnn, rnn_c)
                if self.logger is not None:
                    self.logger.per_step(data)
                self.insert(data)
            self.compute()
            self.prep_training()
            infos_a, info_c = self.train()
            history.append((infos_a, info_c, self.critic_buffer.get_mean_rewards()))
            if self.logger is not None and episode % tr.get("log_interval", 1) == 0:
                self.logger.episode_log(infos_a, info_c, self.actor_buffer, self.critic_buffer)
            if episode % tr.get("eval_interval", 25) == 0:
                if self.algo_args.get("eval", {}).get("use_eval", False) and self.eval_envs is not None:
                    self.prep_rollout()
                    self.eval()
                if getattr(self, "save_dir", None):
                    self.save(self.save_dir)
            self.after_update()
        return history

    @torch.no_grad()
    def eval(self):
        import numpy as np
        ev = self.algo_args["eval"]
        n_thr, A = ev["n_eval_rollout_threads"], self.num_agents
        lg = self.logger
        if lg is not None:
            lg.eval_init()
        obs, _share, avail = self.eval_envs.reset()
        H = self.algo_args["model"]["hidden_sizes"][-1]
        rn = self.algo_args["model"]["recurrent_n"]
        rnn = torch.zeros(n_thr, A, rn, H, dtype=torch.float32, device=self.device)
        masks = torch.ones(n_thr, A, 1, dtype=torch.float32, device=self.device)
        done_eps, ep_rewards, cur = 0, [], np.zeros(n_thr)
        while True:
            acts = []
            obs_d = torch.as_tensor(np.asarray(obs), dtype=torch.float32).to(self.device)
            av_d = None if (avail is None or avail[0] is None) else torch.as_tensor(np.asarray(avail), dtype=torch.float32).to(self.device)
            for a in range(A):
                act, r_ = self.actor[a].act(obs_d[:, a], rnn[:, a], masks[:, a], None if av_d is None else av_d[:, a],
                                            deterministic=True)
                rnn[:, a] = r_.reshape(n_thr, rn, H)
                acts.append(act)
            actions = torch.stack(acts, 1).cpu().numpy()
# ... 147 lines not shown
```

### harl_amd/traffic.py

```python
from __future__ import annotations

from typing import Callable, Dict, Optional, Sequence


def _act(H: int) -> float:
    return 4.0 * H + H / 8.0 + 4.0


def _kp(D: int) -> int:
    return 32 * ((int(D) + 31) // 32)


def _fwd_fused2x(a: Sequence) -> float:
    M, D, H, store1 = a[1], a[3], a[7], a[8]
    return M * (4.0 * _kp(D) + (_act(H) if store1 else 0.0) + _act(H))


def _fwd_fused2(a: Sequence) -> float:
    M, D, H, store1, x0n = a[3], a[4], a[10], a[11], a[20]
    return M * (4.0 * D + (8.0 if a[2] else 0.0) + (_act(H) if store1 else 0.0) + _act(H) + 8.0 + (4.0 * _kp(D) if x0n else 0.0))


def _fwd_hidden(a: Sequence) -> float:
    return a[1] * (4.0 * a[2] + _act(a[3]))


def _fwd_wide(a: Sequence) -> float:
    return a[1] * (4.0 * a[2] + _act(a[6]))


def _fwd_input(a: Sequence) -> float:
    return a[3] * (4.0 * a[4] + (8.0 if a[2] else 0.0) + _act(a[8]) + 8.0 + (4.0 * _kp(a[4]) if a[14] else 0.0))


def _x0n_wide(a: Sequence) -> float:
    return a[3] * (4.0 * a[4] + (8.0 if a[2] else 0.0) + 4.0 * _kp(a[4]) + 8.0)


def _tangent_wide(a: Sequence) -> float:
    return a[1] * (4.0 * a[2] + _act(a[6]) + 4.0 * a[6])


def _bwd_dx(a: Sequence) -> float:
    M, HO, HI = a[4], a[5], a[6]
    return M * (4.0 * HO + _act(HI) + (4.0 * HI if a[8] else 0.0) + (4.0 * a[10] if a[9] else 0.0))


def _bwd_dx_dw(a: Sequence) -> float:
    M, HO, HI = a[4], a[5], a[6]
    return M * (4.0 * HO + _act(HI) + (4.0 * HI if a[8] else 0.0) + (4.0 * a[10] if a[9] else 0.0))


def _dw_partials(a: Sequence) -> float:
    lda, HO, K, M = a[2], a[3], a[10], a[11]
    return M * (4.0 * (lda if a[1] else HO) + 4.0 * K)


def _dw_partials_multi(a: Sequence) -> float:
    n, HO, K, M = a[0], a[4], a[5], a[6]
    return n * M * (4.0 * HO + 4.0 * K)


def _gru_fwd(a: Sequence) -> float:
    H, L, m_pad, save = a[7], a[8], a[9], a[18]
    xin = 3 * 4.0 * H if (save & 2) else 4.0 * H
    return L * m_pad * (xin + 4.0 + 4.0 * H + 4.0 + (5 * 4.0 * H if (save & 1) else 0.0))


def _gru_bwd(a: Sequence) -> float:
    H, L, m_pad = a[9], a[10], a[11]
    if not a[19]:
        return L * m_pad * (6 * 4.0 * H + 4.0 + 4 * 4.0 * H)
    return L * m_pad * (6 * 4.0 * H + 4.0 + _act(H) + 4 * 4.0 * H + 4.0 * H)


def _nonnull(arr) -> int:
    return sum(1 for p in arr if p)


def _fwd_trunk(a: Sequence) -> float:
    M, KP, H = a[1], a[2], a[6]
    return M * (4.0 * KP + _nonnull(a[11]) * _act(H) + (3 * 4.0 * H if a[17] else 0.0))


def _bwd_trunk(a: Sequence) -> float:
    M, H, nh = a[0], a[1], a[2]
    top = (3 * 4.0 * H + _act(H) + 4.0 * H) if a[3] else 4.0 * H
    return M * (top + nh * (_act(H) + 4.0 * H))


def _dw_partials_multi_v(a: Sequence) -> float:
    n, HO, M = a[0], a[4], a[8]
    return M * sum(4.0 * HO + 4.0 * 32 * a[7][k] for k in range(n))


def _head_rows(discrete: int, act_dim: int, avail) -> float:
    w = 1 if discrete else act_dim
    return 4.0 * w + 4.0 * w + (4.0 * act_dim if avail else 0.0)


def _actor_head_loss(a: Sequence) -> float:
    M, H, disc, ad = a[3], a[4], a[10], a[11]
    w = 1 if disc else ad
    return M * (_act(H) + _head_rows(disc, ad, a[14]) + 4.0 + (4.0 if a[18] else 0.0) + (4.0 if a[19] else 0.0)
                + (4.0 * w if a[26] else 0.0) + 4.0 * H + (4.0 * 32 if (a[28] and not a[30]) else 0.0))


def _actor_head_logp(a: Sequence) -> float:
    M, H, disc, ad = a[1], a[2], a[8], a[9]
    w = 1 if disc else ad
    return M * (4.0 * H + 4.0 * w + (4.0 * ad if a[11] else 0.0) + (4.0 * w if a[12] else 0.0) + (4.0 * w if a[13] else 0.0)
                + (8.0 if a[14] else 0.0) + (4.0 * ad if a[16] else 0.0))


def _critic_head_loss(a: Sequence) -> float:
    return a[3] * (_act(a[4]) + 8.0 + 4.0 * a[4])


def _update_fwd_actor(a: Sequence) -> float:
    M, D, H, disc, ad = a[1], a[2], a[3], a[13], a[14]
    w = 1 if disc else ad
    return M * (4.0 * _kp(D) + _head_rows(disc, ad, a[16]) + 4.0 + (4.0 if a[20] else 0.0) + (4.0 if a[21] else 0.0)
                + (4.0 * w if a[26] else 0.0) + 4.0 * H + (_act(H) if a[31] else 0.0))


def _update_logp(a: Sequence) -> float:
    M, D, disc, ad = a[1], a[2], a[13], a[14]
    w = 1 if disc else ad
    return M * (4.0 * _kp(D) + 4.0 * w + (4.0 * ad if a[16] else 0.0) + (4.0 * w if a[17] else 0.0) + (4.0 * w if a[18] else 0.0)
                + (8.0 if a[19] else 0.0) + (4.0 * ad if a[21] else 0.0))


def _update_fwd_critic(a: Sequence) -> float:
    return a[1] * (4.0 * _kp(a[2]) + 8.0 + 4.0 * a[3] + (_act(a[3]) if a[21] else 0.0))


def _update_last_actor(a: Sequence) -> float:
    M, H, disc, ad = a[1], a[2], a[10], a[11]
    w = 1 if disc else ad
    return M * (4.0 * H + _head_rows(disc, ad, a[14]) + 4.0 + (4.0 if a[18] else 0.0) + (4.0 if a[19] else 0.0)
                + (4.0 * w if a[24] else 0.0) + 4.0 * H)


def _update_last_critic(a: Sequence) -> float:
    return a[1] * (4.0 * a[2] + 8.0 + 4.0 * a[2])


def _update_values(a: Sequence) -> float:
    return a[1] * (4.0 * _kp(a[2]) + 4.0)


def _update_bwd(a: Sequence) -> float:
    return a[2] * (4.0 * _kp(a[3]) + 4.0 * a[4])


def _panel_fwd(a: Sequence) -> float:
    return a[1] * (4.0 * a[2] + _act(a[6]))


def _panel_bwd(a: Sequence) -> float:
    return a[4] * (4.0 * a[5] + _act(a[6]) + 4.0 * a[6])


def _tangent_hidden(a: Sequence) -> float:
    return a[2] * (2 * 4.0 * a[3] + _act(a[4]) + 4.0 * a[4])


def _gae(a: Sequence) -> float:
    T, n = a[8], a[9]
    return 4.0 * n * (T + 3 * (T + 1) + (T + 1) + T)


ALGORITHMIC_BYTES: Dict[str, Callable[[Sequence], float]] = {
    "harl_mlp_fwd_fused2x": _fwd_fused2x,
    "harl_mlp_fwd_fused2": _fwd_fused2,
    "harl_mlp_fwd_hidden": _fwd_hidden,
    "harl_mlp_fwd_wide": _fwd_wide,
    "harl_mlp_fwd_input": _fwd_input,
    "harl_mlp_x0n_wide": _x0n_wide,
    "harl_mlp_tangent_wide": _tangent_wide,
    "harl_mlp_bwd_dx": _bwd_dx,
    "harl_mlp_bwd_dx_dw": _bwd_dx_dw,
    "harl_mlp_dw_partials": _dw_partials,
    "harl_mlp_dw_partials_multi": _dw_partials_multi,
    "harl_mlp_dw_partials_multi_v": _dw_partials_multi_v,
    "harl_gru_dw6": lambda a: a[7] * 6 * 4.0 * 64,
    "harl_mlp_fwd_trunk": _fwd_trunk,
    "harl_mlp_bwd_trunk": _bwd_trunk,
    "harl_gru_fwd": _gru_fwd,
    "harl_gru_bwd": _gru_bwd,
    "harl_actor_head_loss": _actor_head_loss,
    "harl_actor_head_logp": _actor_head_logp,
    "harl_critic_head_loss": _critic_head_loss,
    "harl_update_fwd_actor": _update_fwd_actor,
    "harl_update_logp": _update_logp,
    "harl_update_fwd_critic": _update_fwd_critic,
    "harl_update_values": _update_values,
    "harl_update_last_actor": _update_last_actor,
    "harl_update_last_critic": _update_last_critic,
    "harl_update_bwd": _update_bwd,
    "harl_gae_returns": _gae,
    "harl_mlp_panel_fwd": _panel_fwd,
    "harl_mlp_panel_bwd": _panel_bwd,
    "harl_mlp_tangent_hidden": _tangent_hidden,
    "harl_mlp_tangent_hidden2": _tangent_hidden,
}


def algorithmic_bytes(name: str, args: Sequence) -> Optional[float]:
    f = ALGORITHMIC_BYTES.get(name)
    return None if f is None else float(f(args))


def _f_fused2x(a):
    return 2.0 * a[1] * (a[3] * a[7] + a[7] * a[7])


def _f_fused2(a):
    return 2.0 * a[3] * (a[4] * a[10] + a[10] * a[10])


def _f_update_fwd_actor(a):
    M, D, H, ad = a[1], a[2], a[3], a[14]
    return 2.0 * M * (D * H + H * H + 3 * ad * H)


def _f_update_logp(a):
    M, D, H, ad = a[1], a[2], a[3], a[14]
    return 2.0 * M * (D * H + H * H + ad * H)


def _f_update_fwd_critic(a):
    M, D, H = a[1], a[2], a[3]
    return 2.0 * M * (D * H + H * H + 3 * H)


def _f_update_values(a):
    M, D, H = a[1], a[2], a[3]
    return 2.0 * M * (D * H + H * H + H)


def _f_update_last_actor(a):
    return 2.0 * a[1] * (a[2] * a[2] + 3 * a[11] * a[2])


def _f_update_last_critic(a):
    return 2.0 * a[1] * (a[2] * a[2] + 3 * a[2])


def _f_update_bwd(a):
    M, D, H = a[2], a[3], a[4]
    return 2.0 * M * (2 * D * H + 2 * H * H + D * H)


def _f_bwd_dx(a):
    M, HO, HI = a[4], a[5], a[6]
    return 2.0 * M * (HO * HI + (HI * a[10] if a[9] else 0))


def _f_bwd_dx_dw(a):
    M, HO, HI = a[4], a[5], a[6]
    return 2.0 * M * (2 * HO * HI + (HI * a[10] if a[9] else 0))


def _f_dw(a):
    return 2.0 * a[11] * a[3] * a[10]


def _f_dw_multi(a):
    return 2.0 * a[0] * a[6] * a[4] * a[5]


def _f_gru_fwd(a):
    H, L, m_pad = a[7], a[8], a[9]
    return 2.0 * L * m_pad * (3 if (a[18] & 2) else 6) * H * H


def _f_gru_bwd(a):
    H, L, m_pad = a[9], a[10], a[11]
    return 2.0 * L * m_pad * (6 if a[19] else 3) * H * H


def _f_fwd_trunk(a):
    M, D, H, nh = a[1], a[4], a[6], a[8]
    return 2.0 * M * (D * H + nh * H * H + (3 * H * H if a[17] else 0))


def _f_bwd_trunk(a):
    M, H, nh = a[0], a[1], a[2]
    return 2.0 * M * ((3 * H * H if a[3] else 0) + nh * H * H)


def _f_head(a_M, a_H, ad, train):
    return 2.0 * a_M * ad * a_H * (3 if train else 1)


ALGORITHMIC_FLOPS: Dict[str, Callable[[Sequence], float]] = {
    "harl_mlp_fwd_fused2x": _f_fused2x,
    "harl_mlp_fwd_fused2": _f_fused2,
    "harl_mlp_fwd_hidden": lambda a: 2.0 * a[1] * a[2] * a[3],
    "harl_mlp_linear": lambda a: 2.0 * a[1] * a[2] * a[3],
    "harl_mlp_linear3": lambda a: 3 * 2.0 * a[3] * a[4] * a[5],
    "harl_mlp_fwd_wide": lambda a: 2.0 * a[1] * a[4] * a[6],
    "harl_mlp_linear_wide": lambda a: 2.0 * a[1] * a[4] * a[6],
    "harl_mlp_fwd_input": lambda a: 2.0 * a[3] * a[4] * a[8],
    "harl_mlp_tangent_wide": lambda a: 2.0 * a[1] * a[4] * a[6],
    "harl_mlp_tangent_hidden": lambda a: 2.0 * 2 * a[2] * a[3] * a[4],
    "harl_mlp_tangent_hidden2": lambda a: 2.0 * 2 * a[2] * a[3] * a[4],
    "harl_mlp_bwd_dx": _f_bwd_dx,
    "harl_mlp_bwd_dx_dw": _f_bwd_dx_dw,
    "harl_mlp_dw_partials": _f_dw,
    "harl_mlp_dw_partials_multi": _f_dw_multi,
    "harl_mlp_dw_partials_multi_v": lambda a: 2.0 * a[8] * a[4] * 32 * sum(a[7][k] for k in range(a[0])),
    "harl_gru_dw6": lambda a: 2.0 * a[7] * 6 * 64 * 64,
    "harl_mlp_fwd_trunk": _f_fwd_trunk,
    "harl_mlp_bwd_trunk": _f_bwd_trunk,
    "harl_mlp_panel_fwd": lambda a: 2.0 * a[1] * a[4] * a[6],
    "harl_mlp_panel_bwd": lambda a: 2.0 * a[4] * a[5] * a[6],
    "harl_gru_fwd": _f_gru_fwd,
    "harl_gru_bwd": _f_gru_bwd,
    "harl_actor_head_loss": lambda a: _f_head(a[3], a[4], a[11], True) - (2.0 * a[3] * a[11] * a[4] if not a[30] else 0.0),
    "harl_actor_head_logp": lambda a: _f_head(a[1], a[2], a[9], False),
    "harl_actor_head_fvp": lambda a: 0.0,
    "harl_critic_head_loss": lambda a: _f_head(a[3], a[4], 1, True),
    "harl_update_fwd_actor": _f_update_fwd_actor,
    "harl_update_logp": _f_update_logp,
    "harl_update_fwd_critic": _f_update_fwd_critic,
    "harl_update_values": _f_update_values,
    "harl_update_last_actor": _f_update_last_actor,
    "harl_update_last_critic": _f_update_last_critic,
    "harl_update_bwd": _f_update_bwd,
}
# ... 11 lines not shown
```

### harl_amd/v_critic.py

```python
from __future__ import annotations

import os
from typing import Optional

import torch

from . import _lib
from ._lib import PS_STRIDE, call, ptr, stream
from .buffers import OnPolicyCriticBufferEP, consume_randperm, minibatch_indices, rng_sync
from .dist import Comm, local_minibatch_rows
from .nets import FusedAdam, VNet, build_seq
from .valuenorm import ValueNorm, _as_dev


class VCritic:
    def __init__(self, args, cent_obs_space, device=torch.device("cuda:0")):
        self.args = args
        self.device = torch.device(device)
        _lib.require_gpu(self.device)
        self.tpdv = dict(dtype=torch.float32, device=self.device)
        self.clip_param = args["clip_param"]
        self.critic_epoch = args["critic_epoch"]
        self.critic_num_mini_batch = args["critic_num_mini_batch"]
        self.data_chunk_length = args["data_chunk_length"]
        self.value_loss_coef = args["value_loss_coef"]
        self.max_grad_norm = args["max_grad_norm"]
        self.huber_delta = args["huber_delta"]
        self.use_recurrent_policy = args["use_recurrent_policy"]
        self.use_naive_recurrent_policy = args["use_naive_recurrent_policy"]
        self.use_max_grad_norm = args["use_max_grad_norm"]
        self.use_clipped_value_loss = args["use_clipped_value_loss"]
        self.use_huber_loss = args["use_huber_loss"]
        self.use_policy_active_masks = args["use_policy_active_masks"]
        self.critic_lr = args["critic_lr"]
        self.opti_eps = args["opti_eps"]
        self.weight_decay = args["weight_decay"]
        self.share_obs_space = cent_obs_space
        self.critic = VNet(args, cent_obs_space, self.device)
        self.critic_optimizer = FusedAdam(self.critic, self.critic_lr, self.opti_eps, self.weight_decay)
        self.comm = Comm()
        self.shard = None
        self._info = torch.zeros(2, dtype=torch.float64, device=self.device)
        self._grad_tap = None
        self._trace = None
        self._state_tap = None

    def lr_decay(self, episode, episodes):
        lr = self.critic_lr - (self.critic_lr * ((episode - 1) / float(episodes)))
        for g in self.critic_optimizer.param_groups:
            g["lr"] = lr

    def get_values(self, cent_obs, rnn_states_critic, masks):
        x = _as_dev(cent_obs, self.device)
        x = x.reshape(x.shape[0], -1)
        M = x.shape[0]
        net = self.critic
        net.fold()
        Wp, bp = net._packs[-1]
        out = torch.empty(M, 1, **self.tpdv)
        if net.fused_update_ok(None, train=False):
            call("harl_update_values", *net.fused_args(x, M), ptr(out), stream(), tag="update_values")
            return out, (None if rnn_states_critic is None else _as_dev(rnn_states_critic, self.device))
        if not net.recurrent:
            net.forward_trunk(x, None, M, for_backward=False)
            call("harl_critic_head_values", ptr(net.xh[-1]), M, net.hidden_sizes[-1], ptr(Wp), ptr(bp), ptr(out), stream())
            return out, (None if rnn_states_critic is None else _as_dev(rnn_states_critic, self.device))
        H = net.hidden_sizes[-1]
        h0 = _as_dev(rnn_states_critic, self.device)
        m = h0.shape[0]
        HS = H * net.recurrent_n
        seq = build_seq(self.device, M // m, m, HS, h0=h0.reshape(m, HS), masks_src=_as_dev(masks, self.device),
                        want_h_last=True)
        Mp = seq["L"] * seq["m_pad"]
        net.forward_trunk(x, seq["idx"], Mp, for_backward=False, seq=seq)
        fx, _, _, fh = net.feat()
        outp = out if seq["idx"] is None else torch.empty(Mp, 1, **self.tpdv)
        call("harl_critic_head_values", ptr(fx), Mp, fh, ptr(Wp), ptr(bp), ptr(outp), stream())
        if seq["idx"] is not None:
            out.copy_(outp.reshape(seq["L"], seq["m_pad"], 1)[:, :m].reshape(M, 1))
        return out, seq["h_last"][:m].reshape(m, net.recurrent_n, H).clone()

    def _update_core(self, share_obs, idx, m, m_global, value_preds, returns, vn: Optional[ValueNorm], seq=None):
        net = self.critic
        s = stream()
        if vn is not None:
            vidx = seq["valid_idx"] if seq is not None else idx
            vn.update(returns, vidx, count=m_global, reduce_fn=self.comm.all_reduce_sum if self.comm.enabled else None,
                      local_count=(seq["L"] * seq["m"] if seq is not None else m))
        net._ensure_ws(max(m, 1))
        sc = net.scalars
        self._forward_backward(net, share_obs, idx, m, value_preds, returns, vn, seq, s)
        nblk = net.n_wg if m > 0 else 0
        ps_kw = dict(part_scalars=net.part_scalars, n_scalar_blocks=nblk)
        if self.comm.enabled:
            if m <= 0:
                net.dwp.zero_()
            hilo = net.dwp_msg[net.total_dwp:]
            call("harl_reduce_pack_scalars", ptr(net.part_scalars), nblk, ptr(sc), ptr(hilo), s)
            self.comm.all_reduce_message(net.dwp_msg)
            ps_kw = dict(scalars_hilo=hilo)
        scale = float(self.value_loss_coef) / float(m_global)
        if self._state_tap is not None:
            o = self.critic_optimizer
            self._state_tap.append((net.flat_param.clone(), o.exp_avg.clone(), o.exp_avg_sq.clone(), o.step_count))
        self.critic_optimizer.step(1, scale, self.use_max_grad_norm, self.max_grad_norm, self._info, **ps_kw)
        if self._trace is not None:
            self._trace.append(self._info.clone())
        if self._grad_tap is not None:
            self._grad_tap(net.flat_grad * scale, sc.clone())

    def _forward_backward(self, net, share_obs, idx, m, value_preds, returns, vn, seq, s) -> None:
        if m > 0 and net.fused_update_ok(idx, seq):
            call("harl_update_fwd_critic", *net.fused_args(share_obs, m), ptr(value_preds), ptr(returns),
                 ptr(vn.stats) if vn is not None else None, float(self.clip_param), int(self.use_clipped_value_loss),
                 int(self.use_huber_loss), float(self.huber_delta), ptr(net.dz[0]), ptr(net.part_scalars),
                 ptr(net.part[net._part_offs[-1]:]), net.n_wg, *net.hybrid_outputs(), s, tag="update_fwd_critic")
            net.backward_after_fused(share_obs, m)
        elif m > 0 and net.fused_last_ok(idx, seq):
            L = len(net.hidden_sizes)
            net.forward_trunk(share_obs, idx, m, upto=L - 1)
            (Wl, bl), (Wh, bh) = net._packs[L - 1], net._packs[-1]
            call("harl_update_last_critic", ptr(net.xh[L - 2]), m, net.hidden_sizes[-1], ptr(Wl), ptr(bl), ptr(Wh), ptr(bh),
                 ptr(idx), ptr(value_preds), ptr(returns), ptr(vn.stats) if vn is not None else None, float(self.clip_param),
                 int(self.use_clipped_value_loss), int(self.use_huber_loss), float(self.huber_delta), ptr(net.dz[0]),
                 ptr(net.part_scalars), ptr(net.part[net._part_offs[-1]:]), net.n_wg, s, tag="update_last_critic")
            net.backward_trunk(share_obs, idx, m, head_dw_done=True)
        elif m > 0:
            net.forward_trunk(share_obs, idx, m, seq=seq)
            Wp, bp = net._packs[-1]
            fx, fmask, frstd, fh = net.feat()
            mv, mp = (seq["m"], seq["m_pad"]) if seq is not None else (0, 0)
            call("harl_critic_head_loss", ptr(fx), ptr(fmask), ptr(frstd), m, fh,
                 ptr(Wp), ptr(bp), ptr(idx), ptr(value_preds), ptr(returns), ptr(vn.stats) if vn is not None else None,
                 float(self.clip_param), int(self.use_clipped_value_loss), int(self.use_huber_loss), float(self.huber_delta),
                 mv, mp, ptr(net.dz[0]), ptr(net.dhead), ptr(net.part_scalars), ptr(net.part[net._part_offs[-1]:]),
                 net.n_wg, s, tag="critic_head_loss")
            net.backward_trunk(share_obs, idx, m, seq=seq, head_dw_done=True)

    def update(self, sample, value_normalizer=None):
        share_obs, _rnn, value_preds, returns, _masks = sample
        dev = self.device
        x = _as_dev(share_obs, dev)
        m = x.shape[0]
        before = self._info.clone()
        self.critic.fold()
        if self.critic.recurrent:
            HS = self.critic.hidden_sizes[-1] * self.critic.recurrent_n
            h0 = _as_dev(_rnn, dev)
            seq = build_seq(dev, m // h0.shape[0], h0.shape[0], HS, h0=h0.reshape(-1, HS), masks_src=_as_dev(_masks, dev))
            self._update_core(x.reshape(m, -1), seq["idx"], seq["L"] * seq["m_pad"], m, _as_dev(value_preds, dev).reshape(m),
                              _as_dev(returns, dev).reshape(m), value_normalizer, seq=seq)
            d = self._info - before
            return d[0], d[1]
        self._update_core(x.reshape(m, -1), None, m, m, _as_dev(value_preds, dev).reshape(m),
                          _as_dev(returns, dev).reshape(m), value_normalizer)
        d = self._info - before
        return d[0], d[1]

    def train(self, critic_buffer: OnPolicyCriticBufferEP, value_normalizer: Optional[ValueNorm] = None, _defer=False):
        for _ in self._train_epochs(critic_buffer, value_normalizer):
            pass
        return self._train_result(_defer)

    def _train_result(self, _defer: bool):
        n_upd = self.critic_epoch * self.critic_num_mini_batch
        if _defer:
            return self._info / n_upd
        rng_sync()
        vals = (self._info / n_upd).cpu().tolist()
        return {"value_loss": vals[0], "critic_grad_norm": vals[1]}

    def _train_epochs(self, critic_buffer: OnPolicyCriticBufferEP, value_normalizer: Optional[ValueNorm] = None):
        buf = critic_buffer
        T, N = buf.rewards.shape[:2]
        A = getattr(buf, "num_agents", None)
        B = T * N * (A or 1)
        dev = self.device
        self._info.zero_()
        self.critic.invalidate_caches()
        buf.__dict__.pop("_seq_cache", None)
        self.critic.fold()
        share_obs = buf.flat("share_obs")
        value_preds = buf.flat("value_preds").reshape(B)
        returns = buf.flat("returns").reshape(B)
        n_global = self.shard[0] * T * (A or 1) if self.shard else B
        for _ in range(self.critic_epoch):
            if self.use_recurrent_policy or self.use_naive_recurrent_policy:
                for seq in buf.recurrent_batches(self.critic_num_mini_batch, self.data_chunk_length,
                                                 naive=not self.use_recurrent_policy, shard=self.shard):
                    if seq.get("empty"):
                        self._update_core(share_obs, None, 0, seq["L"] * seq["m_global"], value_preds, returns,
                                          value_normalizer)
                        continue
                    self._update_core(share_obs, seq["idx"], seq["L"] * seq["m_pad"], seq["L"] * seq["m_global"],
                                      value_preds, returns, value_normalizer, seq=seq)
                yield
                continue
            if self.critic_num_mini_batch == 1:
                consume_randperm(n_global)
                self._update_core(share_obs, None, B, n_global, value_preds, returns, value_normalizer)
                yield
                continue
            sampler = minibatch_indices(n_global, self.critic_num_mini_batch, dev)
            for ind in sampler:
                m_global = ind.numel()
                if self.shard:
                    ind = local_minibatch_rows(ind, self.shard[0], self.shard[1], self.shard[2], agents=A or 1)
                self._update_core(share_obs, ind.to(dev), ind.numel(), m_global, value_preds, returns, value_normalizer)
            yield

    def prep_training(self):
        self.critic.train()
        self.critic.invalidate_caches()

    def prep_rollout(self):
        self.critic.eval()
        self.critic.invalidate_caches()
```

### include/harl_hip.h

```cpp
#ifndef HARL_HIP_H
#define HARL_HIP_H

#include <stdint.h>

#ifdef __cplusplus
extern "C" {
#endif

#define HARL_PS_STRIDE 48
#define HARL_DHEAD_LD 32
#define HARL_MD_MAX_HEADS 8
#define HARL_MD_MAX_GROUPS 4
#define HARL_MM_SCRATCH_BYTES 24640
#define HARL_CG_SCRATCH_BYTES 1088

int harl_version(void);
const char *harl_last_error(void);

int harl_gae_returns(const float *rewards, float *value_preds, const float *masks, const float *bad_masks,
                     const float *next_value, const float *vn_stats, float *returns, float *advantages,
                     int T, int ncols, float gamma, float gamma_lambda, int use_gae,
                     int use_proper_time_limits, int fp_order, void *stream);

int harl_masked_moments(const float *x, const float *active, long n, double *out3, void *scratch, void *stream);

int harl_dist_rows(const float *head, long M, int act_dim, int kind, const float *log_std, float std_x_coef, float std_y_coef,
                   const float *noise, float *actions, const int *head_off, int n_heads, int sum_heads, float *logp,
                   float *probs, float *argmax_out, float *ent_rows, float *sigma_out, void *stream);
int harl_moments_mean(const double *moments3, float *mean_out, void *stream);
int harl_build_seq(const int64_t *first, int m, int m_pad, int L, long stride, const float *masks_src, const float *h0_src,
                   int H, int64_t *idx, int64_t *valid_idx, float *mask_rows, float *h0, void *stream);
int harl_clock_probe(long long *cycles_ticks, long ticks, void *stream);
int harl_adv_normalize(const float *adv, const double *moments3, float *adv_out, long n, void *stream);

int harl_factor_update(float *factor, const float *new_logp, const float *old_logp, long n, int act_dim,
                       int agg_mean, void *stream);

int harl_sum_sumsq(const float *x, const int64_t *idx, long m, double *sums2, void *stream);
int harl_valuenorm_apply(float *vn_stats, const double *sums2, double count, double beta, void *stream);

int harl_gradnorm_clip_adam(float *param, float *grad, float *exp_avg, float *exp_avg_sq, long n,
                            const float *grad_scale, int use_clip, float max_norm, double lr, double beta1,
                            double beta2, float eps, float weight_decay, double bias_correction1,
                            double bias_correction2, double *info_out, void *stream);

int harl_fold_linear(const float *W, const float *b, const float *gamma, const float *beta, float *Wp,
                     float *bp, int out_dim, int in_dim, void *stream);
int harl_unfold_linear_grads(const float *dWp, const float *dbp, int ldp, const float *W, const float *gamma,
                             const float *beta, float *dW, float *db, float *dgamma, float *dbeta,
                             int out_dim, int in_dim, int accumulate, void *stream);

int harl_mlp_fwd_input(const float *X, long ldx, const int64_t *idx, long M, int D, const float *Wp,
                       const float *bp, int use_ln0, int H, float *xout, uint32_t *relu_mask, float *rstd,
                       float *mu0, float *rstd0, float *x0n, void *stream);
int harl_mlp_x0n_wide(const float *X, long ldx, const int64_t *idx, long M, int D, int use_ln0, float *x0n, float *mu0,
                      float *rstd0, void *stream);
int harl_mlp_fwd_wide(const float *x0n, long M, int KP, const float *Wp, int D, const float *bp, int H, void *w_img,
                      float *xout, uint32_t *relu_mask, float *rstd, void *stream);
int harl_mlp_panel_fwd(const float *xin, long M, int KP, const float *Wp, int D, const float *bp, int HO, float *xout,
                       uint32_t *relu_mask, float *rstd, void *stream);
int harl_head_dw_rows256(const float *dhead, long M, int act_dim, const float *xhat, float *part, int n_wg, void *stream);
int harl_mlp_panel_tangent(const float *xin_dot, const float *xin, long M, int KP, const float *Wp, const float *Wdp, int D,
                           const float *bdp, const float *xprimal, const uint32_t *mask_in, const float *rstd_in,
                           float *xout_dot, void *stream);
int harl_mlp_panel_bwd(const float *dz, const float *xprev, const uint32_t *relu_mask_prev, const float *rstd_prev, long M,
                       int HO, int HI, const float *Wp, float *dz_prev, void *stream);
int harl_mlp_fwd_fused2x(const float *x0n, long M, const float *W1p, int D, const float *b1p, const float *W2p,
                         const float *b2p, int H, int store1, float *x1out, uint32_t *mask1, float *rstd1, float *x2out,
                         uint32_t *mask2, float *rstd2, void *stream);
int harl_mlp_fwd_fused2(const float *X, long ldx, const int64_t *idx, long M, int D, const float *W1p,
                        const float *b1p, int use_ln0, const float *W2p, const float *b2p, int H, int store1,
                        float *x1out, uint32_t *mask1, float *rstd1, float *mu0, float *rstd0, float *x2out,
                        uint32_t *mask2, float *rstd2, float *x0n, void *stream);
int harl_mlp_fwd_hidden(const float *xin, long M, int HI, int HO, const float *Wp, const float *bp,
                        float *xout, uint32_t *relu_mask, float *rstd, void *stream);
int harl_mlp_bwd_dx(const float *dz, const float *xprev, const uint32_t *relu_mask_prev, const float *rstd_prev,
                    long M, int HO, int HI, const float *Wp, float *dz_prev, const float *x0n, int kp0, float *dw_part,
                    int n_wg, void *stream);
int harl_mlp_bwd_dx_dw(const float *dz, const float *xprev, const uint32_t *relu_mask_prev, const float *rstd_prev,
                       long M, int HO, int HI, const float *Wp, float *dz_prev, const float *x0n, int kp0, float *dw1_part,
                       float *dw2_part, int n_wg, int fill, void *stream);
int harl_mlp_dw_partials(const float *a, int a_kind, int lda, int HO, const float *b, int b_kind, long ldx,
                         const int64_t *idx, const float *mu0, const float *rstd0, int K, long M, float *part,
                         int n_wg, void *stream);
int harl_mlp_dw_partials_multi(int n, const float *const *a, const float *const *b, float *const *part, int HO, int K,
                               long M, int n_wg, void *stream);
int harl_mlp_dw_partials_multi_v(int n, const float *const *a, const float *const *b, float *const *part, int HO, const int *K,
                                 const int *tile0, const int *nt, long M, int n_wg, void *stream);
int harl_gru_dw6(const float *dr, const float *dz, const float *dn, const float *dhn, const float *xhat, const float *hpm,
                 float *const *part, long M, int n_wg, void *stream);
int harl_mlp_fwd_trunk(const float *x0n, long M, int KP, const float *W1p, int D, const float *b1p, int H, void *w_img,
                       int n_hidden, const float *const *Wp, const float *const *bp, float *const *xout,
                       uint32_t *const *relu_mask, float *const *rstd, const float *Wih, const float *bih, const float *bhh,
                       float *gi_ws, void *stream);
int harl_mlp_bwd_trunk(long M, int H, int n_hidden, const float *Wih, const float *dr, const float *dzg, const float *dn,
                       const float *dz_in, const float *const *Wp, const float *const *xh, const uint32_t *const *relu_mask,
                       const float *const *rstd, float *const *dz_out, void *stream);
int harl_reduce_partials(const float *part, int n_wg, long elems, float *out, void *stream);

#define HARL_TABLE_STRIDE 12
int harl_reduce_partials_multi(const float *part, const int *table, int n_layers, int n_wg, long total_elems,
                               float *dwp, void *stream);
int harl_fold_table(const float *param, float *packs, const int *table, int n_layers, int total_rows, void *stream);
int harl_unfold_table(const float *param, float *grad, const float *dwp, const int *table, int n_layers, int total_cols,
                      void *stream);
int harl_fold_tangent_table(const float *param, const float *vec, float *pack_d, const int *table, int n_layers,
                            int total_rows, void *stream);
int harl_pack_scalars_hilo(const double *scalars, float *hilo, void *stream);
int harl_reduce_pack_scalars(const float *part_scalars, int n_blocks, double *scalars, float *hilo, void *stream);
int harl_adam_fold(float *param, float *grad, float *exp_avg, float *exp_avg_sq, long n, const float *dwp,
                   const int *table, int n_layers, float *packs, double *scalars, const float *part_scalars,
                   int n_scalar_blocks, const float *scalars_hilo, int mode, float const_scale, int logstd_off,
                   int act_dim, double *info,
                   int use_clip, float max_norm, double lr, double beta1, double beta2, float eps, float weight_decay,
                   double bias_correction1, double bias_correction2, void *ws, void *stream);

int harl_actor_head_logp(const float *xL, long M, int H, const float *Whp, const float *bhp,
                         const float *log_std, float std_x_coef, float std_y_coef, int discrete, int act_dim,
                         const float *actions, const float *avail, float *logp_out, const float *old_logp,
                         float *factor, int agg_mean, float *head_out, long m_valid, long m_pad, void *stream);
int harl_actor_head_loss(const float *xL, const uint32_t *relu_mask, const float *rstd, long M, int H,
                         const float *Whp, const float *bhp, const float *log_std, float std_x_coef,
                         float std_y_coef, int discrete, int act_dim, const int64_t *idx, const float *actions,
                         const float *avail, const float *old_logp, const float *adv, const double *adv_moments,
                         const float *factor, const float *active, double clip_param, float entropy_coef,
                         int agg_mean, int trpo, long m_valid, long m_pad, float *logp_out, float *dzL, float *dhead,
                         float *part_scalars, float *dw_part, int n_wg, void *stream);
int harl_critic_head_values(const float *xL, long M, int H, const float *Whp, const float *bhp, float *values,
                            void *stream);
int harl_critic_head_loss(const float *xL, const uint32_t *relu_mask, const float *rstd, long M, int H,
                          const float *Whp, const float *bhp, const int64_t *idx, const float *value_preds,
                          const float *returns, const float *vn_stats, float clip_param, int use_clipped,
                          int use_huber, float huber_delta, long m_valid, long m_pad, float *dzL, float *dhead,
                          float *part_scalars, float *dw_part, int n_wg, void *stream);
int harl_fold_linear_tangent(const float *W, const float *gamma, const float *beta, const float *Wd, const float *bd,
                             const float *gammad, const float *betad, float *Wpd, float *bpd, int out_dim, int in_dim,
                             void *stream);
int harl_mlp_tangent_input(const float *X, long ldx, const int64_t *idx, long M, int D, const float *Wdp,
                           const float *bdp, int use_ln0, int H, const float *x1, const uint32_t *mask1,
                           const float *rstd1, float *x1dot, void *stream);
int harl_mlp_linear_wide(const float *x0n, long M, int KP, const float *Wp, int D, const float *bp, int H, void *w_img,
                         float *zout, void *stream);
int harl_act_ln_fwd(const float *z, long M, int H, int act, float *xhat, float *mean, float *rstd, void *stream);
int harl_act_bwd(float *dz, const float *xhat, const float *mean, const float *rstd, long M, int H, int act, void *stream);
int harl_act_ln_tangent(const float *zd1, const float *zd2, const float *xhat, const float *mean, const float *rstd, long M,
                        int H, int act, float *xhat_dot, void *stream);
int harl_mlp_tangent_wide(const float *x0n, long M, int KP, const float *Wdp, int D, const float *bdp, int H, void *w_img,
                          const float *x1, const uint32_t *mask1, const float *rstd1, float *x1dot, void *stream);
int harl_gru_gates(const float *xin, const float *W, int H, long n_slabs, float *out_r, float *out_z, float *out_n,
                   int acc_mask, void *stream);
int harl_gru_tangent(const float *g_r, const float *g_z, const float *g_nx, const float *g_nh, const float *mask_rows,
                     const float *Whh, const float *bihd, const float *bhhd, const float *hpm, const float *r,
                     const float *z, const float *n, const float *hn, const float *y, const float *rstd_y, int H, int L,
                     long m_pad, float *ydot, void *stream);
int harl_mlp_tangent_hidden(const float *xin_dot, const float *xin, long M, int HI, int HO, const float *Wp,
                            const float *Wdp, const float *bdp, const float *xprimal, const uint32_t *mask_in,
                            const float *rstd_in, float *xout_dot, void *stream);
int harl_mlp_tangent_hidden2(const float *xin_dot, const float *xin, long M, int HI, int HO, const float *Wp,
                             const float *Wdp, const float *bdp, void *w_img, const float *xprimal,
                             const uint32_t *mask_in, const float *rstd_in, float *xout_dot, void *stream);
int harl_actor_head_fvp(const float *xL, const float *xLdot, const uint32_t *relu_mask, const float *rstd, long M, int H,
                        const float *Whp, const float *bhp, const float *Whdp, const float *bhdp, const float *log_std,
                        float std_x_coef, float std_y_coef, int discrete, int act_dim, const float *avail, long m_valid,
                        long m_pad, float *dzL, float *dhead, void *stream);
int harl_trpo_fvp_finish(const float *grad, const float *vec, const float *log_std, float *out, long n, float m_global,
                         float damping, long logstd_off, int act_dim, float std_x_coef, float std_y_coef, void *stream);
int harl_trpo_cg_step(float *x, float *r, float *p, const float *avp, long n, float *state, void *scratch, void *stream);
#define HARL_TRPO_STATE 16
int harl_trpo_begin(const float *grad_sum, const double *scalars, long logstd_off, int act_dim, float *g, float *x, float *r,
                    float *p, long n, float *cg_state, double *st, void *scratch, void *stream);
int harl_trpo_step(const float *x, const float *fx, const float *g, const float *theta, float *theta_save, float *full_step,
                   long n, float kl_threshold, double *st, void *scratch, void *stream);
int harl_trpo_ls_candidate(const float *theta_save, const float *full_step, const double *st, float *theta, long n, void *stream);
int harl_trpo_ls_test(const double *scalars, double *kl_sum, double m_global, double kl_threshold, double accept_ratio,
                      double backtrack_coeff, double *st, void *stream);
int harl_reduce_scalars_set(const float *part_scalars, int n_blocks, double *scalars, void *stream);
int harl_zero_bytes(void *p, long bytes, void *stream);
int harl_trpo_kl_sum(const float *head_old, const float *head_new, const float *log_std_old, const float *log_std_new,
                     float std_x_coef, float std_y_coef, long M, int act_dim, int discrete, double *out_sum,
                     void *stream);

int harl_mlp_linear(const float *xin, long M, int HI, int HO, const float *Wp, const float *bp, float *xout, void *stream);
int harl_mlp_linear3(const float *x0, const float *x1, const float *x2, long M, int HI, int HO, const float *W0, const float *W1,
                     const float *W2, const float *b0, const float *b1, const float *b2, float *o0, float *o1, float *o2,
                     void *stream);
int harl_md_head_logp(const float *const *z, int n_groups, const int *sp, int n_heads, const int *nvec,
                      const int *head_group, long M, const float *actions, float *logp_out, const float *old_logp,
                      int old_w, float *factor, int agg_mean, float *head_out, long m_valid, long m_pad, void *stream);
int harl_md_head_loss(const float *const *z, float *const *dz, int n_groups, const int *sp, int n_heads, const int *nvec,
                      const int *head_group, long M, const int64_t *idx, const float *actions, const float *old_logp,
                      int old_w, const float *adv, const double *adv_moments, const float *factor, const float *active,
                      const float *ent_scale, double clip_param, float entropy_coef, int agg_mean, int mode, long m_valid,
                      long m_pad, float *logp_out, float *part_scalars, int n_blocks, void *stream);

int harl_update_supported(int D, int H, int act_dim, int kind);
int harl_update_fwd_actor(const float *x0n, long M, int D, int H, const float *W1p, const float *b1p, const float *W2p,
                          const float *b2p, const float *Whp, const float *bhp, const float *log_std, float std_x_coef,
                          float std_y_coef, int discrete, int act_dim, const float *actions, const float *avail,
                          const float *old_logp, const float *adv, const double *adv_moments, const float *factor,
                          const float *active, double clip_param, float entropy_coef, int agg_mean, int trpo,
                          float *logp_out, float *dz2, float *part_scalars, float *dw_part_head, int n_part_rows,
                          float *xh1, uint32_t *rmask1, float *rstd1, void *stream);
int harl_update_logp(const float *x0n, long M, int D, int H, const float *W1p, const float *b1p, const float *W2p,
                     const float *b2p, const float *Whp, const float *bhp, const float *log_std, float std_x_coef,
                     float std_y_coef, int discrete, int act_dim, const float *actions, const float *avail,
                     float *logp_out, const float *old_logp, float *factor, int agg_mean, float *head_out, void *stream);
int harl_update_fwd_critic(const float *x0n, long M, int D, int H, const float *W1p, const float *b1p, const float *W2p,
                           const float *b2p, const float *Whp, const float *bhp, const float *value_preds,
                           const float *returns, const float *vn_stats, float clip_param, int use_clipped, int use_huber,
                           float huber_delta, float *dz2, float *part_scalars, float *dw_part_head, int n_part_rows,
                           float *xh1, uint32_t *rmask1, float *rstd1, void *stream);
// ... 57 lines not shown
```

Before: 53.07 million.

## Batch input-normalization images for all actors and critic in one side-stream launch

Adds a multi-problem kernel that computes the normalized input image (x0n, mean, rstd) for every actor and the critic in a single grouped launch. The launch runs on a dedicated side stream before training, and an event makes later consumers wait only when they actually use the cached image. The aim is to remove per-network launch overhead and to overlap image construction with other work. In exchange it adds event and cache-key bookkeeping, and any place that overwrites the image buffer must wait on the side-stream event first.

```diff
diff --git a/harl_amd/_lib.py b/harl_amd/_lib.py
--- a/harl_amd/_lib.py
+++ b/harl_amd/_lib.py
@@ -33,6 +33,7 @@
     "harl_unfold_linear_grads": [_vp, _vp, _i, _vp, _vp, _vp, _vp, _vp, _vp, _vp, _i, _i, _i, _vp],
     "harl_mlp_fwd_input": [_vp, _l, _vp, _l, _i, _vp, _vp, _i, _i, _vp, _vp, _vp, _vp, _vp, _vp, _vp],
     "harl_mlp_x0n_wide": [_vp, _l, _vp, _l, _i, _i, _vp, _vp, _vp, _vp],
+    "harl_x0n_multi": [_i] + [_vp] * 10,
     "harl_mlp_fwd_wide": [_vp, _l, _i, _vp, _i, _vp, _i, _vp, _vp, _vp, _vp, _vp],
     "harl_mlp_linear_wide": [_vp, _l, _i, _vp, _i, _vp, _i, _vp, _vp, _vp],
     "harl_act_ln_fwd": [_vp, _l, _i, _i, _vp, _vp, _vp, _vp],
diff --git a/harl_amd/csrc/wide.hip b/harl_amd/csrc/wide.hip
--- a/harl_amd/csrc/wide.hip
+++ b/harl_amd/csrc/wide.hip
@@ -32,6 +32,99 @@
 constexpr int XT_LD = 36;
 
 template <int NC>
+__device__ __forceinline__ void x0n_wide_slab(float *tw, const float *__restrict__ X, long ldx,
+                                              const int64_t *__restrict__ idx, long M, int D, int use_ln0,
+                                              float *__restrict__ x0n, float *__restrict__ mu0_out,
+                                              float *__restrict__ rstd0_out, long slab, int KP, int lane) {
+  const int i = lane & 31, h = lane >> 5;
+  {
+    long rows[32];
+    if (idx) {
+#pragma unroll
+      for (int r = 0; r < 32; ++r) {
+        const long j = slab * SLAB + r;
+        rows[r] = idx[j < M ? j : M - 1];
+      }
+    } else {
+#pragma unroll
+      for (int r = 0; r < 32; ++r) {
+        const long j = slab * SLAB + r;
+        rows[r] = j < M ? j : M - 1;
+      }
+    }
+    int kc[NC];
+#pragma unroll
+    for (int c = 0; c < NC; ++c) kc[c] = 64 * c + lane < D ? 64 * c + lane : 0;
+    float v[32][NC];
+#pragma unroll
+    for (int r = 0; r < 32; ++r) {
+      const float *xr = X + rows[r] * ldx;
+#pragma unroll
+      for (int c = 0; c < NC; ++c) v[r][c] = xr[kc[c]];
+    }
+    const float invD = 1.0f / (float)D;
+    float my_mean = 0.f, my_rstd = 1.f;
+#pragma unroll
+    for (int r = 0; r < 32; ++r) {
+      float mean = 0.f, rstd = 1.f;
+      if (use_ln0) {
+        float s = 0.f;
+#pragma unroll
+        for (int c = 0; c < NC; ++c) s += (64 * c + lane < D) ? v[r][c] : 0.f;
+        mean = wave_sum_dpp(s) * invD;
+        float q = 0.f;
+#pragma unroll
+        for (int c = 0; c < NC; ++c) {
+          const float d = v[r][c] - mean;
+          q += (64 * c + lane < D) ? d * d : 0.f;
+        }
+        rstd = 1.0f / sqrtf(wave_sum_dpp(q) * invD + 1e-5f);
+      }
+#pragma unroll
+      for (int c = 0; c < NC; ++c) {
+        const int k = 64 * c + lane;
+        v[r][c] = k < D ? (v[r][c] - mean) * rstd : ((k == KP - 1 && D < KP) ? 1.0f : 0.f);
+      }
+      if (lane == r) {
+        my_mean = mean;
+        my_rstd = rstd;
+      }
+    }
+    if (lane < 32) {
+      mu0_out[slab * SLAB + lane] = my_mean;
+      rstd0_out[slab * SLAB + lane] = my_rstd;
+    }
+    f32x4 *op = reinterpret_cast<f32x4 *>(x0n + slab * (long)KP * SLAB) + lane;
+#pragma unroll
+    for (int c = 0; c < NC; ++c) {
+      if (64 * c < KP) {
+        float *tl = tw + h * (32 * XT_LD) + i * XT_LD;
+#pragma unroll
+        for (int r4 = 0; r4 < 8; ++r4)
+          *reinterpret_cast<f32x4 *>(tl + 4 * r4) = f32x4{v[4 * r4][c], v[4 * r4 + 1][c], v[4 * r4 + 2][c], v[4 * r4 + 3][c]};
+        asm volatile("s_waitcnt lgkmcnt(0)" ::: "memory");
+        __builtin_amdgcn_wave_barrier();
+#pragma unroll
+        for (int t2 = 0; t2 < 2; ++t2) {
+          if (64 * c + 32 * t2 < KP) {
+            const float *ts = tw + t2 * (32 * XT_LD);
+#pragma unroll
+            for (int qq = 0; qq < 4; ++qq) {
+              f32x4 o;
+#pragma unroll
+              for (int e = 0; e < 4; ++e) o[e] = ts[(8 * qq + 4 * h + e) * XT_LD + i];
+              op[(4 * (2 * c + t2) + qq) * WAVE] = o;
+            }
+          }
+        }
+        asm volatile("s_waitcnt lgkmcnt(0)" ::: "memory");
+        __builtin_amdgcn_wave_barrier();
+      }
+    }
+  }
+}
+
+template <int NC>
 __global__ __launch_bounds__(WG_THREADS, NC <= 3 ? 2 : 1) void k_x0n_wide(const float *__restrict__ X, long ldx,
                                                                            const int64_t *__restrict__ idx, long M, int D,
                                                                            int use_ln0, float *__restrict__ x0n,
@@ -39,105 +132,18 @@
                                                                            float *__restrict__ rstd0_out, long n_slabs, int KP) {
   __shared__ __attribute__((aligned(16))) float tiles[WAVES_PER_WG][2][32 * XT_LD];
   const int lane = threadIdx.x & 63, wave = wave_id();
+  float *tw = &tiles[wave][0][0];
+  for (long slab = (long)blockIdx.x * WAVES_PER_WG + wave; slab < n_slabs; slab += (long)gridDim.x * WAVES_PER_WG)
+    x0n_wide_slab<NC>(tw, X, ldx, idx, M, D, use_ln0, x0n, mu0_out, rstd0_out, slab, KP, lane);
+}
+
+template <int KPV>
+__device__ __forceinline__ void x0n_contig_slab(float *rw, const float *__restrict__ X, long M, int D, int use_ln0,
+                                                float *__restrict__ x0n, float *__restrict__ mu0_out,
+                                                float *__restrict__ rstd0_out, long slab, int lane) {
   const int i = lane & 31, h = lane >> 5;
-  float *tw = &tiles[wave][0][0];
-  for (long slab = (long)blockIdx.x * WAVES_PER_WG + wave; slab < n_slabs; slab += (long)gridDim.x * WAVES_PER_WG) {
-    long rows[32];
-    if (idx) {
-#pragma unroll
-      for (int r = 0; r < 32; ++r) {
-        const long j = slab * SLAB + r;
-        rows[r] = idx[j < M ? j : M - 1];
-      }
-    } else {
-#pragma unroll
-      for (int r = 0; r < 32; ++r) {
-        const long j = slab * SLAB + r;
-        rows[r] = j < M ? j : M - 1;
-      }
-    }
-    int kc[NC];
-#pragma unroll
-    for (int c = 0; c < NC; ++c) kc[c] = 64 * c + lane < D ? 64 * c + lane : 0;
-    float v[32][NC];
-#pragma unroll
-    for (int r = 0; r < 32; ++r) {
-      const float *xr = X + rows[r] * ldx;
-#pragma unroll
-      for (int c = 0; c < NC; ++c) v[r][c] = xr[kc[c]];
-    }
-    const float invD = 1.0f / (float)D;
-    float my_mean = 0.f, my_rstd = 1.f;
-#pragma unroll
-    for (int r = 0; r < 32; ++r) {
-      float mean = 0.f, rstd = 1.f;
-      if (use_ln0) {
-        float s = 0.f;
-#pragma unroll
-        for (int c = 0; c < NC; ++c) s += (64 * c + lane < D) ? v[r][c] : 0.f;
-        mean = wave_sum_dpp(s) * invD;
-        float q = 0.f;
-#pragma unroll
-        for (int c = 0; c < NC; ++c) {
-          const float d = v[r][c] - mean;
-          q += (64 * c + lane < D) ? d * d : 0.f;
-        }
-        rstd = 1.0f / sqrtf(wave_sum_dpp(q) * invD + 1e-5f);
-      }
-#pragma unroll
-      for (int c = 0; c < NC; ++c) {
-        const int k = 64 * c + lane;
-        v[r][c] = k < D ? (v[r][c] - mean) * rstd : ((k == KP - 1 && D < KP) ? 1.0f : 0.f);
-      }
-      if (lane == r) {
-        my_mean = mean;
-        my_rstd = rstd;
-      }
-    }
-    if (lane < 32) {
-      mu0_out[slab * SLAB + lane] = my_mean;
-      rstd0_out[slab * SLAB + lane] = my_rstd;
-    }
-    f32x4 *op = reinterpret_cast<f32x4 *>(x0n + slab * (long)KP * SLAB) + lane;
-#pragma unroll
-    for (int c = 0; c < NC; ++c) {
-      if (64 * c < KP) {
-        float *tl = tw + h * (32 * XT_LD) + i * XT_LD;
-#pragma unroll
-        for (int r4 = 0; r4 < 8; ++r4)
-          *reinterpret_cast<f32x4 *>(tl + 4 * r4) = f32x4{v[4 * r4][c], v[4 * r4 + 1][c], v[4 * r4 + 2][c], v[4 * r4 + 3][c]};
-        asm volatile("s_waitcnt lgkmcnt(0)" ::: "memory");
-        __builtin_amdgcn_wave_barrier();
-#pragma unroll
-        for (int t2 = 0; t2 < 2; ++t2) {
-          if (64 * c + 32 * t2 < KP) {
-            const float *ts = tw + t2 * (32 * XT_LD);
-#pragma unroll
-            for (int qq = 0; qq < 4; ++qq) {
-              f32x4 o;
-#pragma unroll
-              for (int e = 0; e < 4; ++e) o[e] = ts[(8 * qq + 4 * h + e) * XT_LD + i];
-              op[(4 * (2 * c + t2) + qq) * WAVE] = o;
-            }
-          }
-        }
-        asm volatile("s_waitcnt lgkmcnt(0)" ::: "memory");
-        __builtin_amdgcn_wave_barrier();
-      }
-    }
-  }
-}
-
-template <int KPV>
-__global__ __launch_bounds__(WG_THREADS, 4) void k_x0n_contig(const float *__restrict__ X, long M, int D, int use_ln0,
-                                                              float *__restrict__ x0n, float *__restrict__ mu0_out,
-                                                              float *__restrict__ rstd0_out, long n_slabs) {
-  __shared__ float rowsl[WAVES_PER_WG][32 * KPV + 32];
-  const int lane = threadIdx.x & 63, wave = wave_id();
-  const int i = lane & 31, h = lane >> 5;
-  float *rw = &rowsl[wave][0];
   const int per = 32 * D;
-  for (long slab = (long)blockIdx.x * WAVES_PER_WG + wave; slab < n_slabs; slab += (long)gridDim.x * WAVES_PER_WG) {
+  {
     const long base = slab * SLAB * (long)D, lim = M * (long)D;
 #pragma unroll
     for (int u = 0; u < KPV / 2; ++u) {
@@ -176,6 +182,45 @@
     }
     asm volatile("s_waitcnt lgkmcnt(0)" ::: "memory");
     __builtin_amdgcn_wave_barrier();
+  }
+}
+
+template <int KPV>
+__global__ __launch_bounds__(WG_THREADS, 4) void k_x0n_contig(const float *__restrict__ X, long M, int D, int use_ln0,
+                                                              float *__restrict__ x0n, float *__restrict__ mu0_out,
+                                                              float *__restrict__ rstd0_out, long n_slabs) {
+  __shared__ float rowsl[WAVES_PER_WG][32 * KPV + 32];
+  const int lane = threadIdx.x & 63, wave = wave_id();
+  float *rw = &rowsl[wave][0];
+  for (long slab = (long)blockIdx.x * WAVES_PER_WG + wave; slab < n_slabs; slab += (long)gridDim.x * WAVES_PER_WG)
+    x0n_contig_slab<KPV>(rw, X, M, D, use_ln0, x0n, mu0_out, rstd0_out, slab, lane);
+}
+
+constexpr int X0N_MULTI_MAX = 32;
+struct X0nMulti {
+  const float *X[X0N_MULTI_MAX];
+  float *x0n[X0N_MULTI_MAX];
+  float *mu0[X0N_MULTI_MAX];
+  float *rstd0[X0N_MULTI_MAX];
+  long ldx[X0N_MULTI_MAX];
+  long M[X0N_MULTI_MAX];
+  int D[X0N_MULTI_MAX];
+  int use_ln0[X0N_MULTI_MAX];
+};
+__global__ __launch_bounds__(WG_THREADS, 2) void k_x0n_multi(X0nMulti P) {
+  __shared__ __attribute__((aligned(16))) float tiles[WAVES_PER_WG][2 * 32 * XT_LD];
+  const int y = blockIdx.y, lane = threadIdx.x & 63, wave = wave_id();
+  float *tw = &tiles[wave][0];
+  const float *X = P.X[y];
+  float *x0n = P.x0n[y], *mu0 = P.mu0[y], *rstd0 = P.rstd0[y];
+  const long M = P.M[y], ldx = P.ldx[y], n_slabs = (M + SLAB - 1) / SLAB;
+  const int D = P.D[y], use_ln0 = P.use_ln0[y];
+  if (D <= 32) {
+    for (long slab = (long)blockIdx.x * WAVES_PER_WG + wave; slab < n_slabs; slab += (long)gridDim.x * WAVES_PER_WG)
+      x0n_contig_slab<32>(tw, X, M, D, use_ln0, x0n, mu0, rstd0, slab, lane);
+  } else {
+    for (long slab = (long)blockIdx.x * WAVES_PER_WG + wave; slab < n_slabs; slab += (long)gridDim.x * WAVES_PER_WG)
+      x0n_wide_slab<1>(tw, X, ldx, nullptr, M, D, use_ln0, x0n, mu0, rstd0, slab, 64, lane);
   }
 }
 
@@ -745,6 +790,35 @@
   return check_launch("harl_mlp_x0n_wide");
 }
 
+extern "C" int harl_x0n_multi(int n, const float *const *X, const long *ldx, const int *D, const int *kp0, const long *M,
+                              const int *use_ln0, float *const *x0n, float *const *mu0, float *const *rstd0, void *stream) {
+  if (n <= 0) return 0;
+  if (n > X0N_MULTI_MAX) return bad("harl_x0n_multi: at most 32 problems per launch");
+  X0nMulti P;
+  long grid = 1;
+  for (int k = 0; k < X0N_MULTI_MAX; ++k) {
+    const int j = k < n ? k : 0;
+    if (k < n) {
+      if (D[j] < 1 || D[j] > 64 || kp0[j] != ((D[j] + 31) / 32) * 32 || M[j] < 0 || (D[j] <= 32 && ldx[j] != D[j]) || ldx[j] < D[j])
+        return bad("harl_x0n_multi: 1 <= D <= 64, kp0 = D rounded up to 32, dense rows (ldx == D) for D <= 32");
+      if (!X[j] || !x0n[j] || !mu0[j] || !rstd0[j]) return bad("harl_x0n_multi: null pointer in the problem table");
+      const long wgs = (n_slabs_of(M[j]) + WAVES_PER_WG - 1) / WAVES_PER_WG, cap = D[j] <= 32 ? 1024 : 512;
+      const long g = wgs < cap ? wgs : cap;
+      if (g > grid) grid = g;
+    }
+    P.X[k] = X[j];
+    P.x0n[k] = x0n[j];
+    P.mu0[k] = mu0[j];
+    P.rstd0[k] = rstd0[j];
+    P.ldx[k] = ldx[j];
+    P.M[k] = M[j];
+    P.D[k] = D[j];
+    P.use_ln0[k] = use_ln0[j];
+  }
+  hipLaunchKernelGGL(k_x0n_multi, dim3((unsigned)grid, n), dim3(WG_THREADS), 0, (hipStream_t)stream, P);
+  return check_launch("harl_x0n_multi");
+}
+
 extern "C" int harl_mlp_fwd_wide(const float *x0n, long M, int KP, const float *Wp, int D, const float *bp, int H,
                                  void *w_img, float *xout, uint32_t *relu_mask, float *rstd, void *stream) {
   return launch_wide<0>(x0n, M, KP, Wp, D, bp, H, w_img, xout, relu_mask, rstd, nullptr, nullptr, nullptr,
diff --git a/harl_amd/dropin.py b/harl_amd/dropin.py
--- a/harl_amd/dropin.py
+++ b/harl_amd/dropin.py
@@ -58,6 +58,7 @@
         _init_update_state = ours._init_update_state
         _ensure_update_state = ours._ensure_update_state
         _critic_first_ok = getattr(ours, "_critic_first_ok", None)
+        _prebuild_images = ours._prebuild_images
         _fp_normalised_advantages = ours._fp_normalised_advantages
         _check_comms = ours._check_comms
         warmup = ours.warmup
diff --git a/harl_amd/nets.py b/harl_amd/nets.py
--- a/harl_amd/nets.py
+++ b/harl_amd/nets.py
@@ -97,7 +97,7 @@
             raise NotImplementedError("activation functions other than relu: feed-forward MLPs of width 64 / 128 with inputs <= 512")
         self.in_dim = in_dim
         self.wide = 32 < in_dim <= 512
-        self._x0n_key = None
+        self._x0n_key = self._x0n_ready = None
         self.md = False
         self._md_sp: List[int] = []
         self._cpu_params: List[Tuple[str, torch.Tensor]] = []
@@ -302,7 +302,7 @@
         self.rstd0 = torch.empty(mp, dtype=f32, device=dev)
         self.kp0 = ((self.in_dim + 31) // 32) * 32
         self.wide = 32 < self.in_dim <= 512
-        self._x0n_key = None
+        self._x0n_key = self._x0n_ready = None
         self.x0n = torch.empty(mp * self.kp0, dtype=f32, device=dev) if (self.in_dim <= 64 or self.wide) else None
         self.w1img = (torch.empty(3 * self.hidden_sizes[0] * self.kp0 // 2, dtype=f32, device=dev)
                       if (self.wide or self.act_id) else None)
@@ -386,16 +386,38 @@
         return hit
 
     def _x0n_image(self, X: torch.Tensor, M: int, s, idx: Optional[torch.Tensor] = None) -> None:
-        key = ((X.data_ptr(), X._version, tuple(X.shape), M) if idx is None
-               else (X.data_ptr(), X._version, tuple(X.shape), M, idx.data_ptr(), idx._version, idx.numel()))
+        key = self._x0n_key_of(X, M, idx)
         if key != self._x0n_key:
             call("harl_mlp_x0n_wide", ptr(X), X.shape[1], ptr(idx), M, self.in_dim, int(self.use_feature_normalization),
                  ptr(self.x0n), ptr(self.mu0), ptr(self.rstd0), s, tag="x0n_wide")
-            self._x0n_key, self._x0n_src = key, (X, idx)
+            self._x0n_key, self._x0n_src, self._x0n_ready = key, (X, idx), None
+        elif self._x0n_ready is not None:
+            ev, waited = self._x0n_ready
+            if s not in waited:
+                torch.cuda.current_stream(self.device_).wait_event(ev)
+                waited.add(s)
+
+    @staticmethod
+    def _x0n_key_of(X: torch.Tensor, M: int, idx: Optional[torch.Tensor] = None) -> tuple:
+        return ((X.data_ptr(), X._version, tuple(X.shape), M) if idx is None
+                else (X.data_ptr(), X._version, tuple(X.shape), M, idx.data_ptr(), idx._version, idx.numel()))
+
+    def _x0n_overwritten(self) -> None:
+        if self._x0n_ready is not None:
+            torch.cuda.current_stream(self.device_).wait_event(self._x0n_ready[0])
+        self._x0n_key = self._x0n_ready = None
+
+    def x0n_multi_ok(self) -> bool:
+        hs = self.hidden_sizes
+        return bool(self.in_dim <= 64 and not self.recurrent
+                    and (self.act_id or self.panel or self.wide or self.trunk_fused() or (len(hs) >= 2 and hs[0] == hs[1])))
 
     def invalidate_caches(self) -> None:
+        if getattr(self, "_x0n_ready", None) is not None:
+            torch.cuda.current_stream(self.device_).wait_event(self._x0n_ready[0])
         self._x0n_key = None
         self._x0n_src = None
+        self._x0n_ready = None
         self._fold_version = None
 
     def forward_trunk(self, X: torch.Tensor, idx: Optional[torch.Tensor], M: int, for_backward: bool = True,
@@ -450,7 +472,7 @@
             first_hidden = 2
         elif len(hs) >= 2 and hs[0] == hs[1] and self.in_dim <= 32:
             (W1, b1), (W2, b2) = self._packs[0], self._packs[1]
-            self._x0n_key = None
+            self._x0n_overwritten()
             call("harl_mlp_fwd_fused2", ptr(X), X.shape[1], ptr(idx), M, self.in_dim, ptr(W1), ptr(b1),
                  int(self.use_feature_normalization), ptr(W2), ptr(b2), hs[0], int(for_backward), ptr(self.xh[0]),
                  ptr(self.rmask[0]), ptr(self.rstd[0]), ptr(self.mu0), ptr(self.rstd0), ptr(self.xh[1]),
@@ -463,7 +485,7 @@
                  ptr(self.xh[0]), ptr(self.rmask[0]), ptr(self.rstd[0]), s, tag="fwd_wide")
         else:
             Wp, bp = self._packs[0]
-            self._x0n_key = None
+            self._x0n_overwritten()
             call("harl_mlp_fwd_input", ptr(X), X.shape[1], ptr(idx), M, self.in_dim, ptr(Wp), ptr(bp),
                  int(self.use_feature_normalization), hs[0], ptr(self.xh[0]), ptr(self.rmask[0]), ptr(self.rstd[0]),
                  ptr(self.mu0), ptr(self.rstd0), ptr(self.x0n) if for_backward else None, s, tag="fwd_input")
@@ -779,6 +801,32 @@
         return out
 
 
+_x0n_tables: dict = {}
+
+
+def build_x0n_images(problems, side: "torch.cuda.Stream") -> None:
+    import ctypes as C
+    n = len(problems)
+    for net, X, M in problems:
+        assert net.x0n_multi_ok() and X.dim() == 2 and X.shape[1] == net.in_dim and X.is_contiguous() and M <= X.shape[0]
+        net._ensure_ws(M)
+    rows = tuple((ptr(X), X.shape[1], net.in_dim, net.kp0, M, int(net.use_feature_normalization), ptr(net.x0n), ptr(net.mu0),
+                  ptr(net.rstd0)) for net, X, M in problems)
+    tab = _x0n_tables.get(rows)
+    if tab is None:
+        if len(_x0n_tables) >= 16:
+            _x0n_tables.clear()
+        cols = list(zip(*rows))
+        types = (C.c_void_p, C.c_long, C.c_int, C.c_int, C.c_long, C.c_int, C.c_void_p, C.c_void_p, C.c_void_p)
+        tab = _x0n_tables[rows] = tuple((t * n)(*c) for t, c in zip(types, cols))
+    with torch.cuda.stream(side):
+        call("harl_x0n_multi", n, *tab, side.cuda_stream, tag="x0n_multi")
+        ev = torch.cuda.Event()
+        ev.record(side)
+    for net, X, M in problems:
+        net._x0n_key, net._x0n_src, net._x0n_ready = net._x0n_key_of(X, M), (X, None), (ev, set())
+
+
 class StochasticPolicy(_FlatNet):
 
     def __init__(self, args: dict, obs_space, action_space, device: torch.device):
diff --git a/harl_amd/runner.py b/harl_amd/runner.py
--- a/harl_amd/runner.py
+++ b/harl_amd/runner.py
@@ -126,6 +126,7 @@
         actor_train_infos = []
         for x in self.actor:
             x.actor.invalidate_caches()
+        ckw = dict(_image_ready=True) if self._prebuild_images(B) else {}
         factor = torch.ones(T, N, 1, dtype=torch.float32, device=dev)
         advantages = self.critic_buffer.advantages
         if self.state_type == "FP":
@@ -157,11 +158,11 @@
                 main_s = torch.cuda.current_stream(dev)
                 self._critic_stream.wait_stream(main_s)
                 with torch.cuda.stream(self._critic_stream):
-                    cinfo = self.critic.train(self.critic_buffer, self.value_normalizer, _defer=True)
+                    cinfo = self.critic.train(self.critic_buffer, self.value_normalizer, _defer=True, **ckw)
                     critic_done = torch.cuda.Event()
                     critic_done.record(self._critic_stream)
             else:
-                cinfo = self.critic.train(self.critic_buffer, self.value_normalizer, _defer=True)
+                cinfo = self.critic.train(self.critic_buffer, self.value_normalizer, _defer=True, **ckw)
         ev.synchronize()
         counts = self._counts_host.tolist()
         rng_after = None
@@ -179,7 +180,7 @@
             if getattr(self, "_critic_stream", None) is None:
                 self._critic_stream = torch.cuda.Stream(device=dev)
             self._critic_stream.wait_stream(torch.cuda.current_stream(dev))
-            staggered = dict(gen=self.critic._train_epochs(self.critic_buffer, self.value_normalizer), state=torch.get_rng_state(),
+            staggered = dict(gen=self.critic._train_epochs(self.critic_buffer, self.value_normalizer, **ckw), state=torch.get_rng_state(),
                              left=self.critic.critic_epoch)
             torch.set_rng_state(rng_start)
 
@@ -298,7 +299,7 @@
                 critic_done = torch.cuda.Event()
                 critic_done.record(self._critic_stream)
         if cinfo is None:
-            cinfo = self.critic.train(self.critic_buffer, self.value_normalizer, _defer=True)
+            cinfo = self.critic.train(self.critic_buffer, self.value_normalizer, _defer=True, **ckw)
         if critic_done is not None:
             torch.cuda.current_stream(dev).wait_event(critic_done)
         rng_sync()
@@ -315,6 +316,30 @@
                 off += len(keys)
         critic_train_info = {"value_loss": flat[off], "critic_grad_norm": flat[off + 1]}
         return actor_train_infos, critic_train_info
+
+    def _prebuild_images(self, B: int) -> bool:
+        from .nets import build_x0n_images
+        dev = self.device
+        if dev.type != "cuda" or os.environ.get("HARL_X0N_MULTI", "1") == "0":
+            return False
+        probs = []
+        for a, buf in zip(self.actor, self.actor_buffer):
+            if hasattr(a, "masked_moments") and hasattr(a, "fuses_old_logp") and a.fuses_old_logp() and a.actor.x0n_multi_ok():
+                probs.append((a.actor, buf.flat("obs"), B))
+        c = self.critic
+        with_critic = (c.critic_num_mini_batch == 1 and not (c.use_recurrent_policy or c.use_naive_recurrent_policy)
+                       and c.critic.x0n_multi_ok())
+        if with_critic:
+            c.critic.invalidate_caches()
+            X = self.critic_buffer.flat("share_obs")
+            probs.append((c.critic, X, X.shape[0]))
+        if not probs or len(probs) > 32:
+            return False
+        if getattr(self, "_image_stream", None) is None:
+            self._image_stream = torch.cuda.Stream(device=dev)
+        self._image_stream.wait_stream(torch.cuda.current_stream(dev))
+        build_x0n_images(probs, self._image_stream)
+        return with_critic
 
     def _critic_first_ok(self, fast) -> bool:
         if not all(fast) or os.environ.get("HARL_CRITIC_FIRST", "1") == "0":
diff --git a/harl_amd/traffic.py b/harl_amd/traffic.py
--- a/harl_amd/traffic.py
+++ b/harl_amd/traffic.py
@@ -35,6 +35,10 @@
 
 def _x0n_wide(a: Sequence) -> float:
     return a[3] * (4.0 * a[4] + (8.0 if a[2] else 0.0) + 4.0 * _kp(a[4]) + 8.0)
+
+
+def _x0n_multi(a: Sequence) -> float:
+    return sum(a[5][k] * (4.0 * a[3][k] + 4.0 * a[4][k] + 8.0) for k in range(a[0]))
 
 
 def _tangent_wide(a: Sequence) -> float:
@@ -178,6 +182,7 @@
     "harl_mlp_fwd_wide": _fwd_wide,
     "harl_mlp_fwd_input": _fwd_input,
     "harl_mlp_x0n_wide": _x0n_wide,
+    "harl_x0n_multi": _x0n_multi,
     "harl_mlp_tangent_wide": _tangent_wide,
     "harl_mlp_bwd_dx": _bwd_dx,
     "harl_mlp_bwd_dx_dw": _bwd_dx_dw,
diff --git a/harl_amd/v_critic.py b/harl_amd/v_critic.py
--- a/harl_amd/v_critic.py
+++ b/harl_amd/v_critic.py
@@ -157,8 +157,9 @@
         d = self._info - before
         return d[0], d[1]
 
-    def train(self, critic_buffer: OnPolicyCriticBufferEP, value_normalizer: Optional[ValueNorm] = None, _defer=False):
-        for _ in self._train_epochs(critic_buffer, value_normalizer):
+    def train(self, critic_buffer: OnPolicyCriticBufferEP, value_normalizer: Optional[ValueNorm] = None, _defer=False,
+              _image_ready=False):
+        for _ in self._train_epochs(critic_buffer, value_normalizer, _image_ready):
             pass
         return self._train_result(_defer)
 
@@ -170,14 +171,16 @@
         vals = (self._info / n_upd).cpu().tolist()
         return {"value_loss": vals[0], "critic_grad_norm": vals[1]}
 
-    def _train_epochs(self, critic_buffer: OnPolicyCriticBufferEP, value_normalizer: Optional[ValueNorm] = None):
+    def _train_epochs(self, critic_buffer: OnPolicyCriticBufferEP, value_normalizer: Optional[ValueNorm] = None,
+                      _image_ready=False):
         buf = critic_buffer
         T, N = buf.rewards.shape[:2]
         A = getattr(buf, "num_agents", None)
         B = T * N * (A or 1)
         dev = self.device
         self._info.zero_()
-        self.critic.invalidate_caches()
+        if not _image_ready:
+            self.critic.invalidate_caches()
         buf.__dict__.pop("_seq_cache", None)
         self.critic.fold()
         share_obs = buf.flat("share_obs")
diff --git a/include/harl_hip.h b/include/harl_hip.h
--- a/include/harl_hip.h
+++ b/include/harl_hip.h
@@ -57,6 +57,8 @@
                       float *rstd0, void *stream);
 int harl_mlp_fwd_wide(const float *x0n, long M, int KP, const float *Wp, int D, const float *bp, int H, void *w_img,
                       float *xout, uint32_t *relu_mask, float *rstd, void *stream);
+int harl_x0n_multi(int n, const float *const *X, const long *ldx, const int *D, const int *kp0, const long *M,
+                   const int *use_ln0, float *const *x0n, float *const *mu0, float *const *rstd0, void *stream);
 int harl_mlp_panel_fwd(const float *xin, long M, int KP, const float *Wp, int D, const float *bp, int HO, float *xout,
                        uint32_t *relu_mask, float *rstd, void *stream);
 int harl_head_dw_rows256(const float *dhead, long M, int act_dim, const float *xhat, float *part, int n_wg, void *stream);
```

Result: no change. 52.99 million (-0.2%).
